# kujason/monopsr

Measured on AMD Instinct MI355X. Metric: instance-crops/sec (fwd+Chamfer), higher is better.
Workload: dtype f32; 1 GPU; BASELINE cfg3: batch=256/GPU synthetic 48x48 crops -> ResNet-101 trunk(block3, os4) + squash/map-decoder/xyz + heads fwd, + 1024-pt nn_distance Chamfer fwd/bwd; batch_per_gpu=256, global_batch=256, points=1024, streams_per_gpu=1

## Files before the change

### include/monopsr_hip.h

```cpp
#ifndef MONOPSR_HIP_H
#define MONOPSR_HIP_H

#include <stddef.h>
#include <stdint.h>

#ifdef __cplusplus
extern "C" {
#endif

typedef void *mpsr_stream_t;
typedef void *mpsr_event_t;

enum {
    MPSR_OK = 0,
    MPSR_ERR_INVALID_ARG = 1,
    MPSR_ERR_HIP = 2,
    MPSR_ERR_WORKSPACE = 3,
    MPSR_ERR_UNSUPPORTED = 4
};

const char *mpsr_last_error(void);
int mpsr_abi_version(void);
uint32_t mpsr_crc32c(uint32_t crc, const void *data, size_t n);


int mpsr_nn_distance_fwd(int b, int n, const float *xyz1, int m, const float *xyz2,
                         float *dist1, int *idx1, float *dist2, int *idx2, mpsr_stream_t stream);

int mpsr_nn_distance_bwd(int b, int n, const float *xyz1, int m, const float *xyz2,
                         const float *grad_dist1, const int *idx1, const float *grad_dist2, const int *idx2,
                         float *grad_xyz1, float *grad_xyz2, mpsr_stream_t stream);


enum { MPSR_EMD_DEVICE = 0, MPSR_EMD_HOST = 1 };

size_t mpsr_emd_temp_floats(int b, int n, int m, int semantics);
size_t mpsr_approx_match_temp_floats(int b, int n, int m);

int mpsr_approx_match(int b, int n, int m, const float *xyz1, const float *xyz2, float *match, float *temp,
                      size_t temp_floats, mpsr_stream_t stream);

int mpsr_approx_match_ex(int b, int n, int m, const float *xyz1, const float *xyz2, float *match, float *temp,
                         size_t temp_floats, int semantics, mpsr_stream_t stream);

size_t mpsr_emd_loss_temp_floats(int b, int n, int m, int semantics);
int mpsr_emd_loss(int b, int n, int m, const float *xyz1, const float *xyz2, float *cost, float *grad1, float *grad2,
                  float *temp, size_t temp_floats, int semantics, mpsr_stream_t stream);

int mpsr_match_cost(int b, int n, int m, const float *xyz1, const float *xyz2, const float *match, float *out,
                    mpsr_stream_t stream);

int mpsr_match_cost_grad(int b, int n, int m, const float *xyz1, const float *xyz2, const float *match,
                         float *grad1, float *grad2, mpsr_stream_t stream);


int mpsr_crop_and_resize(const float *image, int nimg, int H, int W, int C, const float *boxes,
                         const int *box_ind, int nb, int ch, int cw, float extrapolation_value, float *out,
                         mpsr_stream_t stream);

int mpsr_resize_bilinear(const float *in, int B, int H, int W, int C, int OH, int OW, int align_corners,
                         float *out, mpsr_stream_t stream);

int mpsr_max_pool(const float *in, int B, int H, int W, int C, int k, int s, int pad_same, float *out,
                  mpsr_stream_t stream);


size_t mpsr_conv2d_scratch_floats(int B, int H, int W, int N);
int mpsr_conv2d_plan(int B, int H, int W, int C, int N, int KH, int KW, int dilation, int *kind,
                     double *executed_flops);
int mpsr_conv2d_nhwc_f32(const float *x, int B, int H, int W, int C, const float *w, const float *bias,
                         const float *residual, float *y, int N, int KH, int KW, int dilation, int relu,
                         int split_k, float *ws, size_t ws_floats, mpsr_stream_t stream);

enum { MPSR_CALL_MATH_INHERIT = 0, MPSR_CALL_MATH_FP32 = 1, MPSR_CALL_MATH_BF16X3 = 2 };
enum { MPSR_CALL_WINOGRAD_INHERIT = 0, MPSR_CALL_WINOGRAD_AUTO = 1, MPSR_CALL_WINOGRAD_OFF = 2,
       MPSR_CALL_WINOGRAD_ACCURATE = 3  };
typedef struct mpsr_conv_opts {
    int32_t math;
    int32_t winograd_policy;
} mpsr_conv_opts;
int mpsr_conv2d_nhwc_f32_ex(const float *x, int B, int H, int W, int C, const float *w, const float *bias,
                            const float *residual, float *y, int N, int KH, int KW, int dilation, int relu,
                            int split_k, float *ws, size_t ws_floats, const mpsr_conv_opts *opts, mpsr_stream_t stream);

enum { MPSR_MATH_FP32 = 0, MPSR_MATH_BF16X3 = 1 };
int mpsr_set_conv_math(int mode);
int mpsr_get_conv_math(void);

enum { MPSR_WINOGRAD_AUTO = 0, MPSR_WINOGRAD_OFF = 1, MPSR_WINOGRAD_ACCURATE = 2 };
int mpsr_set_winograd_policy(int policy);
int mpsr_get_winograd_policy(void);

size_t mpsr_conv3x3_upsampled_scratch_floats(int B, int h, int w, int C, int N);
int mpsr_conv3x3_upsampled_f32(const float *x, int B, int h, int w, int C, int OH, int OW, int align_corners,
                               const float *weights, const float *bias, int relu, float *y, int N, float *ws,
                               size_t ws_floats, mpsr_stream_t stream);
int mpsr_conv3x3_upsampled_applies(int B, int h, int w, int C, int OH, int OW, int N, int align_corners);
size_t mpsr_conv3x3_upsampled_bwd_scratch_floats(int B, int h, int w, int C, int N);
int mpsr_conv3x3_upsampled_bwd_f32(const float *x, const float *dy, int B, int h, int w, int C, int OH, int OW,
                                   int align_corners, const float *weights, int N, float *dw, float *dx, float *ws,
                                   size_t ws_floats, mpsr_stream_t stream);

int mpsr_im2col_root(const float *x, int B, int H, int W, float *cols, int kpad, mpsr_stream_t stream);


int mpsr_conv2d_wgrad_f32(const float *x, const float *dy, int B, int H, int W, int C, int N, int KH, int KW,
                          int dilation, float *dw, float *db, mpsr_stream_t stream);
size_t mpsr_conv2d_wgrad_scratch_floats(int B, int H, int W, int C, int N, int KH, int KW, int dilation);
int mpsr_conv2d_wgrad_ws_f32(const float *x, const float *dy, int B, int H, int W, int C, int N, int KH, int KW,
                             int dilation, float *dw, float *db, float *ws, size_t ws_floats, mpsr_stream_t stream);
int mpsr_conv2d_wgrad_plan(int B, int H, int W, int C, int N, int KH, int KW, int dilation, size_t ws_floats, int *kind,
                           int *tiles, int *steps, int *nslices);

int mpsr_conv2d_dgrad_pack(const float *w, int N, int KH, int KW, int C, float *wd, mpsr_stream_t stream);

typedef struct mpsr_pack_job {
    const float *w;
    float *wd;
    int32_t N, Nd, T, C;
    int64_t chunk0;
} mpsr_pack_job;
size_t mpsr_dgrad_pack_table_bytes(const mpsr_pack_job *jobs, int n_jobs);
int mpsr_dgrad_pack_table_build(const mpsr_pack_job *jobs, int n_jobs, void *table_host, long long *n_chunks);
int mpsr_conv2d_dgrad_pack_batch(const void *table_dev, long long n_chunks, mpsr_stream_t stream);

int mpsr_act_bias_grad(const float *dy, const float *y, float *dx, float *db, long long M, int N,
                       mpsr_stream_t stream);

int mpsr_bias_grad(const float *dy, long long M, int N, float *db, mpsr_stream_t stream);

int mpsr_relu_grad(const float *dy, const float *y, float *dx, long long total, mpsr_stream_t stream);

int mpsr_conv2d_relu_masked_f32(const float *x, int B, int H, int W, int C, const float *w, const float *mask, float *y,
                                int N, int KH, int KW, int dilation, float *ws, size_t ws_floats, mpsr_stream_t stream);
long long mpsr_relu_bitmask_words(long long M, int N);
int mpsr_relu_bitmask(const float *y, long long M, int N, unsigned *bits, mpsr_stream_t stream);
int mpsr_conv1x1_masked_applies(long long M, int K, int N);
int mpsr_conv1x1_relu_bitmask_f32(const float *x, long long M, int K, const float *w, const float *bias,
                                  const float *residual, int relu, float *y, unsigned *bits, int N, mpsr_stream_t stream);
int mpsr_conv1x1_masked_f32(const float *x, long long M, int K, const float *w, const float *bias,
                            const float *residual, const unsigned *mask, float *y, int N, mpsr_stream_t stream);

int mpsr_max_pool_grad(const float *x, const float *dy, int B, int H, int W, int C, int k, int s, int pad_same,
                       float *dx, mpsr_stream_t stream);

int mpsr_resize_bilinear_grad(const float *dy, int B, int H, int W, int C, int OH, int OW, int align_corners,
                              float *dx, mpsr_stream_t stream);

int mpsr_adam_step(float *param, const float *grad, float *m, float *v, long long n, float lr, float beta1,
                   float beta2, float eps, int step, float grad_scale, mpsr_stream_t stream);
int mpsr_adam_step_lr_dev(float *param, const float *grad, float *m, float *v, long long n, const float *lr_t_dev,
                          float beta1, float beta2, float eps, float grad_scale, mpsr_stream_t stream);

int mpsr_crop_and_resize_grad(const float *grad_out, int nimg, int H, int W, int C, const float *boxes,
                              const int *box_ind, int nb, int ch, int cw, float *grad_image, mpsr_stream_t stream);

int mpsr_batch_norm_stats(const float *z, long long M, int C, double *sum, double *sumsq_shifted,
                          mpsr_stream_t stream);
int mpsr_batch_norm_finalize(const double *sum, const double *sumsq_shifted, const float *z_row0, long long M, int C,
                             float eps, float decay, float *moving_mean, float *moving_variance, float *mean,
                             float *inv_std, mpsr_stream_t stream);
int mpsr_batch_norm_grad_finalize(const double *sum_g, const double *sum_gz, double count, int C, float *dbeta,
                                  float *mean_g, float *mean_gz, mpsr_stream_t stream);
int mpsr_batch_norm_apply(const float *z, long long M, int C, const float *mean, const float *inv_std,
                          const float *beta, int relu, float *y, mpsr_stream_t stream);
int mpsr_batch_norm_grad_sums(const float *dy, const float *y, const float *z, long long M, int C, const float *mean,
                              const float *inv_std, double *sum_g, double *sum_gz, mpsr_stream_t stream);
int mpsr_batch_norm_grad(const float *dy, const float *y, const float *z, long long M, int C, const float *mean,
                         const float *inv_std, const float *mean_g, const float *mean_gz, float *dz,
                         mpsr_stream_t stream);

int mpsr_batch_norm_grad_sums_z(const float *dy, const float *z, long long M, int C, const float *mean,
                                const float *inv_std, const float *beta, double *sum_g, double *sum_gz,
                                mpsr_stream_t stream);
int mpsr_batch_norm_grad_z(const float *dy, const float *z, long long M, int C, const float *mean, const float *inv_std,
                           const float *beta, const float *mean_g, const float *mean_gz, float *dz, mpsr_stream_t stream);

int mpsr_clip_by_norm_segments(float *grads, const int *chunk_seg, const long long *chunk_begin,
                               const int *chunk_len, int n_chunks, float *sumsq, size_t sumsq_floats, int n_segments,
                               float clip_norm, mpsr_stream_t stream);

int mpsr_clip_adam_ema_step(float *param, const float *grad, float *m, float *v, float *shadow, const int *chunk_seg,
                            const long long *chunk_begin, const int *chunk_len, int n_chunks, float *sumsq,
                            size_t sumsq_floats, int n_segments, float clip_norm, float lr, float beta1, float beta2,
                            float eps, int step, float ema_decay, mpsr_stream_t stream);


int mpsr_xyz_map_local_to_global(const float *xyz_local, const float *view_angs, const float *centroids,
                                 float *xyz_global, int b, int p, mpsr_stream_t stream);

int mpsr_xyz_map_local_to_global_grad(const float *grad_global, const float *view_angs, float *grad_local,
                                      float *grad_centroids, int b, int p, mpsr_stream_t stream);

int mpsr_proj_err_norm(const float *xyz_global, const float *boxes_2d, const float *cam_p, const float *valid_mask,
                       float *proj_err_maps, float *proj_err_norm, int b, int h, int w, mpsr_stream_t stream);

int mpsr_proj_err_norm_grad(const float *grad_proj_err_norm, const float *xyz_global, const float *boxes_2d,
                            const float *cam_p, const float *valid_mask, float *grad_xyz_global, int b, int h, int w,
                            mpsr_stream_t stream);

int mpsr_proj_err_norm_cams(const float *xyz_global, const float *boxes_2d, const float *cam_p, int n_cams,
                            const int *cam_index, const float *valid_mask, float *proj_err_maps, float *proj_err_norm,
                            int b, int h, int w, mpsr_stream_t stream);
int mpsr_proj_err_norm_grad_cams(const float *grad_proj_err_norm, const float *xyz_global, const float *boxes_2d,
                                 const float *cam_p, int n_cams, const int *cam_index, const float *valid_mask,
                                 float *grad_xyz_global, int b, int h, int w, mpsr_stream_t stream);

int mpsr_depth_map_local_to_global(const float *depth_local, int depth_stride, const float *cen_z,
                                   const float *boxes_2d, const float *view_angs, const float *cam_p,
                                   float *depth_global, int b, int h, int w, int rotate_view, mpsr_stream_t stream);

int mpsr_depth_map_local_to_global_grad(const float *grad_global, const float *boxes_2d, const float *view_angs,
                                        const float *cam_p, float *grad_cen_z, int b, int h, int w, int rotate_view,
                                        mpsr_stream_t stream);

int mpsr_depth_map_local_to_global_cams(const float *depth_local, int depth_stride, const float *cen_z,
                                        const float *boxes_2d, const float *view_angs, const float *cam_p, int n_cams,
                                        const int *cam_index, float *depth_global, int b, int h, int w,
                                        int rotate_view, mpsr_stream_t stream);
int mpsr_depth_map_local_to_global_grad_cams(const float *grad_global, const float *boxes_2d, const float *view_angs,
                                             const float *cam_p, int n_cams, const int *cam_index, float *grad_cen_z,
                                             int b, int h, int w, int rotate_view, mpsr_stream_t stream);

int mpsr_huber_loss_sums(const float *pred, const float *target, const float *weights, int b, int p, int c,
                         float delta, float *sums, float *counts, mpsr_stream_t stream);

int mpsr_huber_loss_grad(const float *pred, const float *target, const float *weights, const float *scale, int b,
                         int p, int c, float delta, float *grad, mpsr_stream_t stream);

int mpsr_huber_loss_grad_scales(const float *pred, const float *target, const float *weights, const float *scale,
                                int b, int p, int c, float delta, float *grad, mpsr_stream_t stream);

int mpsr_format_boxes(const float *lwh, const float *view_angs, const float *alpha_bins, const float *alpha_regs,
                      const float *centroids, const float *boxes_2d, const float *scores, const int *class_idx,
                      const float *cam_p, int b, int num_alpha_bins, int img_h, int img_w, int centroid_middle,
                      int post_process_cen_x, float max_depth, float *box_3d, float *box_2d, mpsr_stream_t stream);


typedef struct mpsr_layer {
    int32_t cin, cout, kh, kw, dilation, relu;
    int64_t w_off;
    int64_t b_off;
} mpsr_layer;

typedef struct mpsr_net_opts {
    float *filter_cache;
    size_t filter_cache_floats;
    int32_t filter_cache_valid;
    mpsr_event_t ready_event;
    int32_t *filter_cache_tags;
    int32_t math;
    int32_t winograd_policy;
} mpsr_net_opts;

size_t mpsr_filter_cache_floats(const mpsr_layer *layers, int n_layers);

#define MPSR_TRUNK_LAYERS 94

size_t mpsr_trunk_workspace_bytes(int B, int H, int W);

int mpsr_trunk_fwd(const float *img, int B, int H, int W, const float *blob, const mpsr_layer *layers,
                   int n_layers, float *out, void *workspace, size_t workspace_bytes, mpsr_stream_t stream);
int mpsr_trunk_fwd_ex(const float *img, int B, int H, int W, const float *blob, const mpsr_layer *layers,
                      int n_layers, float *out, void *workspace, size_t workspace_bytes, const mpsr_net_opts *opts,
                      mpsr_stream_t stream);

#define MPSR_DECODER_LAYERS 7

size_t mpsr_decoder_workspace_bytes(int B, int fh, int fw, int mh, int mw);

int mpsr_squash_decoder_fwd(const float *crop_feat, const float *full_feat, int B, int fh, int fw, int mh, int mw,
                            const float *blob, const mpsr_layer *layers, int n_layers, float *feat_box3d,
                            float *feat_map, float *xyz_map, void *workspace, size_t workspace_bytes,
                            mpsr_stream_t stream);
int mpsr_squash_decoder_plan(int B, int fh, int fw, int mh, int mw, const mpsr_layer *layers, int n_layers, int *kinds,
                             double *executed_flops);
int mpsr_squash_decoder_fwd_ex(const float *crop_feat, const float *full_feat, int B, int fh, int fw, int mh, int mw,
                               const float *blob, const mpsr_layer *layers, int n_layers, float *feat_box3d,
                               float *feat_map, float *xyz_map, void *workspace, size_t workspace_bytes,
                               const mpsr_net_opts *opts, mpsr_stream_t stream);

#define MPSR_HEAD_LAYERS 7

typedef struct mpsr_head_consts {
    float image_h, image_w;
    float max_depth;
    float cen_y_norm;
    float cen_y_class_offset;
    int32_t num_classes;
    int32_t num_alpha_bins;
} mpsr_head_consts;

size_t mpsr_heads_workspace_bytes(int B, int feat_elems);

typedef struct mpsr_head_outputs {
    float *lwh, *lwh_offs, *alpha_bins, *alpha_regs, *prop_cen_z, *cen_y, *cen_y_offs, *cen_z, *cen_z_offs,
        *cen_x, *centroids;
} mpsr_head_outputs;

int mpsr_heads_fwd(const float *feat_box3d, int B, int feat_elems, const float *boxes_2d, const float *cam_p,
                   const float *view_angs, const int *class_idx, const float *mean_lwh, const float *cen_z_offset,
                   const mpsr_head_consts *consts, const float *blob, const mpsr_layer *layers, int n_layers,
                   const mpsr_head_outputs *outs, void *workspace, size_t workspace_bytes, mpsr_stream_t stream);
int mpsr_heads_fwd_cams(const float *feat_box3d, int B, int feat_elems, const float *boxes_2d, const float *cam_p,
                        int n_cams, const int *cam_index, const float *view_angs, const int *class_idx,
                        const float *mean_lwh, const float *cen_z_offset, const mpsr_head_consts *consts,
                        const float *blob, const mpsr_layer *layers, int n_layers, const mpsr_head_outputs *outs,
                        void *workspace, size_t workspace_bytes, mpsr_stream_t stream);


#define MPSR_KITTI_FIELDS 14
#define MPSR_KITTI_X1 0
#define MPSR_KITTI_Y1 1
#define MPSR_KITTI_X2 2
#define MPSR_KITTI_Y2 3
#define MPSR_KITTI_ALPHA 4
#define MPSR_KITTI_H 5
#define MPSR_KITTI_W 6
#define MPSR_KITTI_L 7
#define MPSR_KITTI_TX 8
#define MPSR_KITTI_TY 9
#define MPSR_KITTI_TZ 10
#define MPSR_KITTI_RY 11
#define MPSR_KITTI_SCORE 12
#define MPSR_KITTI_TRUNCATION 12
#define MPSR_KITTI_OCCLUSION 13
enum { MPSR_KITTI_CAR = 0, MPSR_KITTI_PEDESTRIAN = 1, MPSR_KITTI_CYCLIST = 2, MPSR_KITTI_VAN = 3,
       MPSR_KITTI_PERSON_SITTING = 4, MPSR_KITTI_DONTCARE = 5, MPSR_KITTI_OTHER = 6 };
#define MPSR_KITTI_CONFIGS 27
#define MPSR_KITTI_POINTS 41
#define MPSR_KITTI_MAX_FRAME_DETECTIONS 8192

typedef struct mpsr_kitti_batch {
    const double *det;
    const int *det_cls;
    const double *gt;
    const int *gt_cls;
    const int *det_off;
    const int *gt_off;
    const long long *pair_off;
    const int *det_off_host;
    const int *gt_off_host;
    const long long *pair_off_host;
    int n_det, n_gt, n_frames;
} mpsr_kitti_batch;

int mpsr_kitti_overlaps(const mpsr_kitti_batch *batch, double *overlaps, mpsr_stream_t stream);

int mpsr_kitti_match(const mpsr_kitti_batch *batch, const double *overlaps, const double *min_overlap,
                     double *tp_scores, int *n_care, mpsr_stream_t stream);

size_t mpsr_kitti_stats_workspace_bytes(int n_frames, int n_configs);

int mpsr_kitti_stats(const mpsr_kitti_batch *batch, const double *overlaps, const double *min_overlap,
                     const double *thresholds, const int *n_thresholds, int compute_aos, int *counts,
                     double *similarity, void *workspace, size_t workspace_bytes, mpsr_stream_t stream);


size_t mpsr_lidar_project_workspace_bytes(int n_frames, int h, int w);

int mpsr_lidar_project_depths(const float *points, const long long *frame_offsets, const long long *frame_offsets_host,
                              int n_frames, const double *velo_to_cam0, const double *p2, int h, int w,
                              double max_depth, float *out, void *workspace, size_t workspace_bytes,
                              mpsr_stream_t stream);

#define MPSR_DEPTH_MAX_KERNEL 15
enum { MPSR_DEPTH_BLUR_BILATERAL = 0, MPSR_DEPTH_BLUR_GAUSSIAN = 1 };
enum { MPSR_DEPTH_KERNEL_FAR = 0, MPSR_DEPTH_KERNEL_MED = 1, MPSR_DEPTH_KERNEL_NEAR = 2 };

typedef struct mpsr_depth_fill_opts {
    float max_depth;
    int extrapolate;
    int blur_type;
    int kernel_h[3];
    int kernel_w[3];
    unsigned char kernels[3][MPSR_DEPTH_MAX_KERNEL * MPSR_DEPTH_MAX_KERNEL];
} mpsr_depth_fill_opts;

size_t mpsr_depth_fill_workspace_bytes(int n_frames, int h, int w);

int mpsr_depth_fill_multiscale(const float *depths, int n_frames, int h, int w, const mpsr_depth_fill_opts *opts,
                               float *out, float *stages, void *workspace, size_t workspace_bytes,
                               mpsr_stream_t stream);


#define MPSR_INSTANCE_MAX_BOXES 255
#define MPSR_INSTANCE_BOX_STRIDE 20
enum { MPSR_CENTROID_BOTTOM = 0, MPSR_CENTROID_MIDDLE = 1 };

int mpsr_instance_images(const float *depth, int n_frames, int h, int w, const double *p2, const double *boxes,
                         const long long *box_offsets, const long long *box_offsets_host, unsigned char *out,
                         mpsr_stream_t stream);

int mpsr_instance_xyz_crops(const float *depth, const unsigned char *inst, const float *p2, int n_frames, int h, int w,
                            const int *frame_index, const int *instance_id, const float *boxes_2d,
                            const float *boxes_3d, const float *view_angs, const int *frame_index_host,
                            const int *instance_id_host, const float *boxes_2d_host, int n_boxes, int roi_h,
                            int roi_w, int centroid_type, int rotate_view, float *xyz_local, float *xyz_global,
                            float *valid, mpsr_stream_t stream);


enum { MPSR_JITTER_NONE = 0, MPSR_JITTER_OVERSAMPLE = 1, MPSR_JITTER_ALL = 2 };

int mpsr_sample_slots(const int *slot_frame, const int *slot_s, int n, const int *num_objs,
                      const long long *label_offset, const int *split_index, const int *frame_local,
                      const int *image_hw, const double *p00_p02, const double *label_boxes, int n_frames,
                      unsigned long long seed, int epoch, int jitter_mode, long long *label_row, int *oversample_index,
                      int *jitter_flag, double *boxes_xyxy, int *slot_hw, double *slot_p, int *slot_split_index,
                      int *slot_frame_local, mpsr_stream_t stream);

int mpsr_jitter_boxes_2d(const double *boxes_xyxy, const int *jitter_flag, const int *image_hw, const double *p00_p02,
                         const int *frame_index, const int *slot, int n, unsigned long long seed, int epoch,
                         double iou_threshold_min, int max_trials, int write_unjittered, double *out_xyxy,
                         float *out_boxes_2d, float *out_boxes_2d_norm, float *out_view_angs, int *out_trials,
                         mpsr_stream_t stream);

enum { MPSR_CROP_BAD_FRAME = 1, MPSR_CROP_BAD_ID = 2, MPSR_CROP_BAD_NOT_FINITE = 4, MPSR_CROP_BAD_BOX = 8 };
int mpsr_instance_xyz_crops_status(const float *depth, const unsigned char *inst, const float *p2, int n_frames, int h,
                                   int w, const int *frame_index, const int *instance_id, const float *boxes_2d,
                                   const float *boxes_3d, const float *view_angs, int n_boxes, int roi_h, int roi_w,
                                   int centroid_type, int rotate_view, float *xyz_local, float *xyz_global,
                                   float *valid, int *status, mpsr_stream_t stream);

enum { MPSR_IMAGE_NOISE_REFERENCE = 1, MPSR_IMAGE_NOISE_COMPOSED = 2 };
int mpsr_image_noise(const unsigned char *frames, int n_frames, int h, int w, const int *gather,
                     const int *frame_index, int nb, unsigned long long seed, int epoch, int mode, float *out,
                     int *stages, double *params, mpsr_stream_t stream);


enum { MPSR_MERGE_SCORE_DISTANCE = 0, MPSR_MERGE_SCORE_MAX = 1, MPSR_MERGE_SCORE_MIN = 2 };

int mpsr_merge_detections(const float *label_boxes, const float *label_z, const long long *label_off,
                          long long n_labels, const float *det_boxes, const double *det_scores,
                          const long long *det_off, long long n_dets, int n_frames, double min_iou, int score_type,
                          float *out_boxes, double *out_scores, int *out_match, mpsr_stream_t stream);

int mpsr_kitti_detection_rows(const float *box_3d, const float *box_2d, const int *frame, const double *p2,
                              const int *image_wh, int n, int n_frames, double score_threshold, int project,
                              double *rows, int *cls, int *keep, mpsr_stream_t stream);

enum { MPSR_NAN_RULE_ENTRY = 0, MPSR_NAN_RULE_FRAME = 1 };
#define MPSR_METRIC_STATS_MAX_COLS 32
int mpsr_metric_stats(const float *values, const int *frame, int n_rows, int n_cols, const int *column_metric,
                      int n_metrics, int n_frames, int nan_rule, int *frame_flags, double *stats,
                      mpsr_stream_t stream);

#define MPSR_TRAIN_LOG_MAX_TERMS 16
#define MPSR_TRAIN_LOG_STAT_COLS 5
typedef struct { const float *p[MPSR_TRAIN_LOG_MAX_TERMS]; } mpsr_train_log_terms;
int mpsr_train_log_append(mpsr_train_log_terms terms, int n_terms, const float *sumsq, int n_segments, float clip_norm,
                          float lr, long long step, float *rows, long long *steps, int n_rows, int n_cols, int row,
                          mpsr_stream_t stream);


size_t mpsr_scene_workspace_bytes(int n_frames, long long total_pixels, int n_boxes, int points_per_box);

int mpsr_scene_project(const float *xyz_global, const float *valid_mask, const int *box_frame,
                       const int *box_frame_host, const int *box_keep, const double *cam_p, const int *frame_hw,
                       const int *frame_hw_host, const long long *pixel_offset, const long long *pixel_offset_host,
                       int n_frames, int n_boxes, int points_per_box, void *workspace, size_t workspace_bytes,
                       mpsr_stream_t stream);

int mpsr_scene_resolve(const int *box_frame, const int *box_frame_host, int n_frames, long long total_pixels,
                       int n_boxes, int points_per_box, const void *workspace, size_t workspace_bytes, float *depth,
                       unsigned char *instance, mpsr_stream_t stream);

int mpsr_scene_compact(const float *xyz_global, const int *box_frame, const float *const *images,
                       const long long *pixel_offset, int n_frames, long long total_pixels, int n_boxes,
                       int points_per_box, int visible_only, void *workspace, size_t workspace_bytes, float *xyz,
                       float *rgb, int *box, int *pixel, long long *frame_offset, int *kept_per_box,
                       int *visible_per_box, mpsr_stream_t stream);

size_t mpsr_scene_score_scratch_bytes(int n_frames);
int mpsr_scene_score(const float *xyz_global, const int *box_frame, const int *box_frame_host, const int *box_gt_id,
                     const float *const *gt_depth, const unsigned char *const *gt_instance,
                     const long long *pixel_offset, int n_frames, long long total_pixels, int n_boxes,
                     int points_per_box, const void *workspace, size_t workspace_bytes, void *scratch,
                     size_t scratch_bytes, int *counts, double *sums, mpsr_stream_t stream);


size_t mpsr_scene_surface_workspace_bytes(int n_frames, long long total_pixels, int n_boxes, int map_h, int map_w);

int mpsr_scene_surface_render(const float *xyz_global, const float *valid_mask, const int *box_frame,
                              const int *box_frame_host, const int *box_keep, const double *cam_p, const int *frame_hw,
                              const int *frame_hw_host, const long long *pixel_offset,
                              const long long *pixel_offset_host, int n_frames, int n_boxes, int map_h, int map_w,
                              float max_edge_dz, int max_span_px, void *workspace, size_t workspace_bytes,
                              mpsr_stream_t stream);

int mpsr_scene_surface_resolve(const int *box_frame, const int *box_frame_host, int n_frames, long long total_pixels,
                               int n_boxes, int map_h, int map_w, const void *workspace, size_t workspace_bytes,
                               float *depth, unsigned char *instance, int *tri, mpsr_stream_t stream);

int mpsr_scene_surface_score(const int *box_frame, const int *box_frame_host, const int *box_gt_id,
                             const float *const *gt_depth, const unsigned char *const *gt_instance,
                             const int *frame_hw, const long long *pixel_offset, int n_frames, long long total_pixels,
                             int n_boxes, int map_h, int map_w, const void *workspace, size_t workspace_bytes,
                             void *scratch, size_t scratch_bytes, int *counts, double *sums, mpsr_stream_t stream);


int mpsr_proj_points(const float *local, const float *x, const float *boxes_2d, const float *cam_p, int n_cams,
                     const int *cam_index, const float *mask, float *uv, unsigned char *valid, double *err, int b,
                     int h, int w, int rotate_view, int cam0_shift, int round_box_2d, int use_pixel_centres,
                     mpsr_stream_t stream);

int mpsr_proj_fit(const float *local, const float *x0, const float *boxes_2d, const float *cam_p, int n_cams,
                  const int *cam_index, const float *mask, int b, int h, int w, int n_fit, int rotate_view,
                  int cam0_shift, int round_box_2d, int use_pixel_centres, double xatol, double fatol, int max_iter,
                  float *x, double *err, double *err0, int *iters, int *evals, int *status, mpsr_stream_t stream);

#ifdef __cplusplus
}
#endif
#endif
```

### monopsr_amd/_lib.py

```python
import ctypes
import os

_HERE = os.path.dirname(os.path.abspath(__file__))
LIB_PATH = os.environ.get("MPSR_LIB_PATH") or os.path.join(_HERE, "libmonopsr_hip.so")
ABI_VERSION = 13

_lib = None


class MpsrError(RuntimeError):
    """A libmonopsr_hip.so call returned a non-zero status."""


class InvalidArgumentError(MpsrError, ValueError):
    """Shape/argument check failed -- the analogue of the tf.errors.InvalidArgumentError the reference's
    OP_REQUIRES checks raise (tf_nndistance.cpp:51-58, tf_approxmatch.cpp:152-165)."""


c_f = ctypes.c_void_p
c_i = ctypes.c_int
c_sz = ctypes.c_size_t


class Layer(ctypes.Structure):
    _fields_ = [("cin", ctypes.c_int32), ("cout", ctypes.c_int32), ("kh", ctypes.c_int32), ("kw", ctypes.c_int32),
                ("dilation", ctypes.c_int32), ("relu", ctypes.c_int32), ("w_off", ctypes.c_int64),
                ("b_off", ctypes.c_int64)]


class HeadConsts(ctypes.Structure):
    _fields_ = [("image_h", ctypes.c_float), ("image_w", ctypes.c_float), ("max_depth", ctypes.c_float),
                ("cen_y_norm", ctypes.c_float), ("cen_y_class_offset", ctypes.c_float),
                ("num_classes", ctypes.c_int32), ("num_alpha_bins", ctypes.c_int32)]


class HeadOutputs(ctypes.Structure):
    _fields_ = [(k, ctypes.c_void_p) for k in
                ("lwh", "lwh_offs", "alpha_bins", "alpha_regs", "prop_cen_z", "cen_y", "cen_y_offs", "cen_z",
                 "cen_z_offs", "cen_x", "centroids")]


class NetOpts(ctypes.Structure):
    _fields_ = [("filter_cache", ctypes.c_void_p), ("filter_cache_floats", ctypes.c_size_t),
                ("filter_cache_valid", ctypes.c_int32), ("ready_event", ctypes.c_void_p),
                ("filter_cache_tags", ctypes.POINTER(ctypes.c_int32)), ("math", ctypes.c_int32),
                ("winograd_policy", ctypes.c_int32)]


class ConvOpts(ctypes.Structure):
    _fields_ = [("math", ctypes.c_int32), ("winograd_policy", ctypes.c_int32)]


class PackJob(ctypes.Structure):
    _fields_ = [("w", ctypes.c_void_p), ("wd", ctypes.c_void_p), ("N", ctypes.c_int32), ("Nd", ctypes.c_int32),
                ("T", ctypes.c_int32), ("C", ctypes.c_int32), ("chunk0", ctypes.c_int64)]


class KittiBatch(ctypes.Structure):
    _fields_ = [(k, ctypes.c_void_p) for k in
                ("det", "det_cls", "gt", "gt_cls", "det_off", "gt_off", "pair_off", "det_off_host", "gt_off_host",
                 "pair_off_host")] + [("n_det", ctypes.c_int32), ("n_gt", ctypes.c_int32), ("n_frames", ctypes.c_int32)]


class DepthFillOpts(ctypes.Structure):
    _fields_ = [("max_depth", ctypes.c_float), ("extrapolate", ctypes.c_int32), ("blur_type", ctypes.c_int32),
                ("kernel_h", ctypes.c_int32 * 3), ("kernel_w", ctypes.c_int32 * 3),
                ("kernels", (ctypes.c_uint8 * (15 * 15)) * 3)]


class TrainLogTerms(ctypes.Structure):
    _fields_ = [("p", ctypes.c_void_p * 16)]


CALL_MATH = {None: 0, "inherit": 0, "fp32": 1, "bf16x3": 2}
CALL_WINOGRAD = {None: 0, "inherit": 0, "auto": 1, "off": 2, "accurate": 3}


SIGNATURES = {
    "mpsr_last_error": (ctypes.c_char_p, []),
    "mpsr_abi_version": (c_i, []),
    "mpsr_set_conv_math": (c_i, [c_i]),
    "mpsr_get_conv_math": (c_i, []),
    "mpsr_set_winograd_policy": (c_i, [c_i]),
    "mpsr_get_winograd_policy": (c_i, []),
    "mpsr_crc32c": (ctypes.c_uint32, [ctypes.c_uint32, ctypes.c_void_p, c_sz]),
    "mpsr_nn_distance_fwd": (c_i, [c_i, c_i, c_f, c_i, c_f, c_f, c_f, c_f, c_f, c_f]),
    "mpsr_nn_distance_bwd": (c_i, [c_i, c_i, c_f, c_i, c_f, c_f, c_f, c_f, c_f, c_f, c_f, c_f]),
    "mpsr_approx_match_temp_floats": (c_sz, [c_i, c_i, c_i]),
    "mpsr_emd_temp_floats": (c_sz, [c_i, c_i, c_i, c_i]),
    "mpsr_emd_loss_temp_floats": (c_sz, [c_i, c_i, c_i, c_i]),
    "mpsr_approx_match": (c_i, [c_i, c_i, c_i, c_f, c_f, c_f, c_f, c_sz, c_f]),
    "mpsr_approx_match_ex": (c_i, [c_i, c_i, c_i, c_f, c_f, c_f, c_f, c_sz, c_i, c_f]),
    "mpsr_emd_loss": (c_i, [c_i, c_i, c_i, c_f, c_f, c_f, c_f, c_f, c_f, c_sz, c_i, c_f]),
    "mpsr_match_cost": (c_i, [c_i, c_i, c_i, c_f, c_f, c_f, c_f, c_f]),
    "mpsr_match_cost_grad": (c_i, [c_i, c_i, c_i, c_f, c_f, c_f, c_f, c_f, c_f]),
    "mpsr_crop_and_resize": (c_i, [c_f, c_i, c_i, c_i, c_i, c_f, c_f, c_i, c_i, c_i, ctypes.c_float, c_f, c_f]),
    "mpsr_resize_bilinear": (c_i, [c_f, c_i, c_i, c_i, c_i, c_i, c_i, c_i, c_f, c_f]),
    "mpsr_max_pool": (c_i, [c_f, c_i, c_i, c_i, c_i, c_i, c_i, c_i, c_f, c_f]),
    "mpsr_conv2d_nhwc_f32": (c_i, [c_f, c_i, c_i, c_i, c_i, c_f, c_f, c_f, c_f, c_i, c_i, c_i, c_i, c_i, c_i, c_f,
                                   c_sz, c_f]),
    "mpsr_conv2d_nhwc_f32_ex": (c_i, [c_f, c_i, c_i, c_i, c_i, c_f, c_f, c_f, c_f, c_i, c_i, c_i, c_i, c_i, c_i, c_f,
                                      c_sz, ctypes.POINTER(ConvOpts), c_f]),
    "mpsr_conv2d_scratch_floats": (c_sz, [c_i, c_i, c_i, c_i]),
    "mpsr_conv2d_plan": (c_i, [c_i] * 8 + [ctypes.POINTER(c_i), ctypes.POINTER(ctypes.c_double)]),
    "mpsr_im2col_root": (c_i, [c_f, c_i, c_i, c_i, c_f, c_i, c_f]),
    "mpsr_conv2d_wgrad_f32": (c_i, [c_f, c_f, c_i, c_i, c_i, c_i, c_i, c_i, c_i, c_i, c_f, c_f, c_f]),
    "mpsr_conv2d_wgrad_scratch_floats": (c_sz, [c_i] * 8),
    "mpsr_conv2d_wgrad_ws_f32": (c_i, [c_f, c_f, c_i, c_i, c_i, c_i, c_i, c_i, c_i, c_i, c_f, c_f, c_f, c_sz, c_f]),
    "mpsr_conv2d_wgrad_plan": (c_i, [c_i] * 8 + [c_sz] + [ctypes.POINTER(c_i)] * 4),
    "mpsr_conv2d_dgrad_pack": (c_i, [c_f, c_i, c_i, c_i, c_i, c_f, c_f]),
    "mpsr_dgrad_pack_table_bytes": (c_sz, [ctypes.POINTER(PackJob), c_i]),
    "mpsr_dgrad_pack_table_build": (c_i, [ctypes.POINTER(PackJob), c_i, ctypes.c_void_p,
                                          ctypes.POINTER(ctypes.c_longlong)]),
    "mpsr_conv2d_dgrad_pack_batch": (c_i, [c_f, ctypes.c_longlong, c_f]),
    "mpsr_act_bias_grad": (c_i, [c_f, c_f, c_f, c_f, ctypes.c_longlong, c_i, c_f]),
    "mpsr_bias_grad": (c_i, [c_f, ctypes.c_longlong, c_i, c_f, c_f]),
    "mpsr_relu_grad": (c_i, [c_f, c_f, c_f, ctypes.c_longlong, c_f]),
    "mpsr_conv2d_relu_masked_f32": (c_i, [c_f, c_i, c_i, c_i, c_i, c_f, c_f, c_f, c_i, c_i, c_i, c_i, c_f, c_sz, c_f]),
    "mpsr_relu_bitmask_words": (ctypes.c_longlong, [ctypes.c_longlong, c_i]),
    "mpsr_relu_bitmask": (c_i, [c_f, ctypes.c_longlong, c_i, c_f, c_f]),
    "mpsr_conv1x1_masked_applies": (c_i, [ctypes.c_longlong, c_i, c_i]),
    "mpsr_conv1x1_masked_f32": (c_i, [c_f, ctypes.c_longlong, c_i, c_f, c_f, c_f, c_f, c_f, c_i, c_f]),
    "mpsr_conv1x1_relu_bitmask_f32": (c_i, [c_f, ctypes.c_longlong, c_i, c_f, c_f, c_f, c_i, c_f, c_f, c_i, c_f]),
    "mpsr_max_pool_grad": (c_i, [c_f, c_f, c_i, c_i, c_i, c_i, c_i, c_i, c_i, c_f, c_f]),
    "mpsr_resize_bilinear_grad": (c_i, [c_f, c_i, c_i, c_i, c_i, c_i, c_i, c_i, c_f, c_f]),
    "mpsr_adam_step": (c_i, [c_f, c_f, c_f, c_f, ctypes.c_longlong, ctypes.c_float, ctypes.c_float, ctypes.c_float,
                             ctypes.c_float, c_i, ctypes.c_float, c_f]),
    "mpsr_adam_step_lr_dev": (c_i, [c_f, c_f, c_f, c_f, ctypes.c_longlong, c_f, ctypes.c_float, ctypes.c_float,
                                    ctypes.c_float, ctypes.c_float, c_f]),
    "mpsr_crop_and_resize_grad": (c_i, [c_f, c_i, c_i, c_i, c_i, c_f, c_f, c_i, c_i, c_i, c_f, c_f]),
    "mpsr_batch_norm_stats": (c_i, [c_f, ctypes.c_longlong, c_i, c_f, c_f, c_f]),
    "mpsr_batch_norm_finalize": (c_i, [c_f, c_f, c_f, ctypes.c_longlong, c_i, ctypes.c_float, ctypes.c_float, c_f, c_f,
                                       c_f, c_f, c_f]),
    "mpsr_batch_norm_grad_finalize": (c_i, [c_f, c_f, ctypes.c_double, c_i, c_f, c_f, c_f, c_f]),
    "mpsr_batch_norm_apply": (c_i, [c_f, ctypes.c_longlong, c_i, c_f, c_f, c_f, c_i, c_f, c_f]),
    "mpsr_batch_norm_grad_sums": (c_i, [c_f, c_f, c_f, ctypes.c_longlong, c_i, c_f, c_f, c_f, c_f, c_f]),
    "mpsr_batch_norm_grad_sums_z": (c_i, [c_f, c_f, ctypes.c_longlong, c_i, c_f, c_f, c_f, c_f, c_f, c_f]),
    "mpsr_batch_norm_grad_z": (c_i, [c_f, c_f, ctypes.c_longlong, c_i, c_f, c_f, c_f, c_f, c_f, c_f, c_f]),
    "mpsr_batch_norm_grad": (c_i, [c_f, c_f, c_f, ctypes.c_longlong, c_i, c_f, c_f, c_f, c_f, c_f, c_f]),
    "mpsr_clip_by_norm_segments": (c_i, [c_f, c_f, c_f, c_f, c_i, c_f, ctypes.c_size_t, c_i, ctypes.c_float, c_f]),
    "mpsr_clip_adam_ema_step": (c_i, [c_f, c_f, c_f, c_f, c_f, c_f, c_f, c_f, c_i, c_f, ctypes.c_size_t, c_i, ctypes.c_float,
                                      ctypes.c_float, ctypes.c_float, ctypes.c_float, ctypes.c_float, c_i, ctypes.c_float,
                                      c_f]),
    "mpsr_xyz_map_local_to_global": (c_i, [c_f, c_f, c_f, c_f, c_i, c_i, c_f]),
    "mpsr_xyz_map_local_to_global_grad": (c_i, [c_f, c_f, c_f, c_f, c_i, c_i, c_f]),
    "mpsr_proj_err_norm": (c_i, [c_f, c_f, c_f, c_f, c_f, c_f, c_i, c_i, c_i, c_f]),
    "mpsr_proj_err_norm_grad": (c_i, [c_f, c_f, c_f, c_f, c_f, c_f, c_i, c_i, c_i, c_f]),
    "mpsr_proj_err_norm_cams": (c_i, [c_f, c_f, c_f, c_i, c_f, c_f, c_f, c_f, c_i, c_i, c_i, c_f]),
    "mpsr_proj_err_norm_grad_cams": (c_i, [c_f, c_f, c_f, c_f, c_i, c_f, c_f, c_f, c_i, c_i, c_i, c_f]),
    "mpsr_depth_map_local_to_global": (c_i, [c_f, c_i, c_f, c_f, c_f, c_f, c_f, c_i, c_i, c_i, c_i, c_f]),
    "mpsr_depth_map_local_to_global_grad": (c_i, [c_f, c_f, c_f, c_f, c_f, c_i, c_i, c_i, c_i, c_f]),
    "mpsr_depth_map_local_to_global_cams": (c_i, [c_f, c_i, c_f, c_f, c_f, c_f, c_i, c_f, c_f, c_i, c_i, c_i, c_i, c_f]),
    "mpsr_depth_map_local_to_global_grad_cams": (c_i, [c_f, c_f, c_f, c_f, c_i, c_f, c_f, c_i, c_i, c_i, c_i, c_f]),
    "mpsr_huber_loss_sums": (c_i, [c_f, c_f, c_f, c_i, c_i, c_i, ctypes.c_float, c_f, c_f, c_f]),
    "mpsr_huber_loss_grad": (c_i, [c_f, c_f, c_f, c_f, c_i, c_i, c_i, ctypes.c_float, c_f, c_f]),
    "mpsr_huber_loss_grad_scales": (c_i, [c_f, c_f, c_f, c_f, c_i, c_i, c_i, ctypes.c_float, c_f, c_f]),
    "mpsr_format_boxes": (c_i, [c_f, c_f, c_f, c_f, c_f, c_f, c_f, c_f, c_f, c_i, c_i, c_i, c_i, c_i, c_i,
                                ctypes.c_float, c_f, c_f, c_f]),
    "mpsr_trunk_workspace_bytes": (c_sz, [c_i, c_i, c_i]),
    "mpsr_trunk_fwd": (c_i, [c_f, c_i, c_i, c_i, c_f, ctypes.POINTER(Layer), c_i, c_f, c_f, c_sz, c_f]),
    "mpsr_conv3x3_upsampled_scratch_floats": (c_sz, [c_i, c_i, c_i, c_i, c_i]),
    "mpsr_conv3x3_upsampled_f32": (c_i, [c_f, c_i, c_i, c_i, c_i, c_i, c_i, c_i, c_f, c_f, c_i, c_f, c_i, c_f, c_sz, c_f]),
    "mpsr_conv3x3_upsampled_applies": (c_i, [c_i, c_i, c_i, c_i, c_i, c_i, c_i, c_i]),
    "mpsr_conv3x3_upsampled_bwd_scratch_floats": (c_sz, [c_i, c_i, c_i, c_i, c_i]),
    "mpsr_conv3x3_upsampled_bwd_f32": (c_i, [c_f, c_f, c_i, c_i, c_i, c_i, c_i, c_i, c_i, c_f, c_i, c_f, c_f, c_f, c_sz,
                                            c_f]),
    "mpsr_filter_cache_floats": (c_sz, [ctypes.POINTER(Layer), c_i]),
    "mpsr_trunk_fwd_ex": (c_i, [c_f, c_i, c_i, c_i, c_f, ctypes.POINTER(Layer), c_i, c_f, c_f, c_sz,
                                ctypes.POINTER(NetOpts), c_f]),
    "mpsr_squash_decoder_fwd_ex": (c_i, [c_f, c_f, c_i, c_i, c_i, c_i, c_i, c_f, ctypes.POINTER(Layer), c_i, c_f, c_f,
                                         c_f, c_f, c_sz, ctypes.POINTER(NetOpts), c_f]),
    "mpsr_decoder_workspace_bytes": (c_sz, [c_i, c_i, c_i, c_i, c_i]),
    "mpsr_squash_decoder_plan": (c_i, [c_i, c_i, c_i, c_i, c_i, ctypes.POINTER(Layer), c_i, ctypes.POINTER(c_i),
                                       ctypes.POINTER(ctypes.c_double)]),
    "mpsr_squash_decoder_fwd": (c_i, [c_f, c_f, c_i, c_i, c_i, c_i, c_i, c_f, ctypes.POINTER(Layer), c_i, c_f, c_f,
                                      c_f, c_f, c_sz, c_f]),
    "mpsr_heads_workspace_bytes": (c_sz, [c_i, c_i]),
    "mpsr_heads_fwd": (c_i, [c_f, c_i, c_i, c_f, c_f, c_f, c_f, c_f, c_f, ctypes.POINTER(HeadConsts), c_f,
                             ctypes.POINTER(Layer), c_i, ctypes.POINTER(HeadOutputs), c_f, c_sz, c_f]),
    "mpsr_heads_fwd_cams": (c_i, [c_f, c_i, c_i, c_f, c_f, c_i, c_f, c_f, c_f, c_f, c_f, ctypes.POINTER(HeadConsts), c_f,
                                  ctypes.POINTER(Layer), c_i, ctypes.POINTER(HeadOutputs), c_f, c_sz, c_f]),
    "mpsr_kitti_overlaps": (c_i, [ctypes.POINTER(KittiBatch), c_f, c_f]),
    "mpsr_kitti_match": (c_i, [ctypes.POINTER(KittiBatch), c_f, ctypes.POINTER(ctypes.c_double), c_f, c_f, c_f]),
    "mpsr_kitti_stats_workspace_bytes": (c_sz, [c_i, c_i]),
    "mpsr_kitti_stats": (c_i, [ctypes.POINTER(KittiBatch), c_f, ctypes.POINTER(ctypes.c_double), c_f,
                               ctypes.POINTER(c_i), c_i, c_f, c_f, c_f, c_sz, c_f]),
    "mpsr_lidar_project_workspace_bytes": (c_sz, [c_i, c_i, c_i]),
    "mpsr_lidar_project_depths": (c_i, [c_f, c_f, ctypes.c_void_p, c_i, c_f, c_f, c_i, c_i, ctypes.c_double, c_f, c_f,
                                        c_sz, c_f]),
    "mpsr_depth_fill_workspace_bytes": (c_sz, [c_i, c_i, c_i]),
    "mpsr_depth_fill_multiscale": (c_i, [c_f, c_i, c_i, c_i, ctypes.POINTER(DepthFillOpts), c_f, c_f, c_f, c_sz, c_f]),
    "mpsr_instance_images": (c_i, [c_f, c_i, c_i, c_i, c_f, c_f, c_f, ctypes.c_void_p, c_f, c_f]),
    "mpsr_instance_xyz_crops": (c_i, [c_f, c_f, c_f, c_i, c_i, c_i, c_f, c_f, c_f, c_f, c_f, ctypes.c_void_p,
                                      ctypes.c_void_p, ctypes.c_void_p, c_i, c_i, c_i, c_i, c_i, c_f, c_f, c_f, c_f]),
    "mpsr_sample_slots": (c_i, [c_f, c_f, c_i, c_f, c_f, c_f, c_f, c_f, c_f, c_f, c_i, ctypes.c_uint64, c_i, c_i, c_f,
                                c_f, c_f, c_f, c_f, c_f, c_f, c_f, c_f]),
    "mpsr_jitter_boxes_2d": (c_i, [c_f, c_f, c_f, c_f, c_f, c_f, c_i, ctypes.c_uint64, c_i, ctypes.c_double, c_i, c_i,
                                   c_f, c_f, c_f, c_f, c_f, c_f]),
    "mpsr_image_noise": (c_i, [c_f, c_i, c_i, c_i, c_f, c_f, c_i, ctypes.c_uint64, c_i, c_i, c_f, c_f, c_f, c_f]),
    "mpsr_instance_xyz_crops_status": (c_i, [c_f, c_f, c_f, c_i, c_i, c_i, c_f, c_f, c_f, c_f, c_f, c_i, c_i, c_i, c_i,
                                             c_i, c_f, c_f, c_f, c_f, c_f]),
    "mpsr_merge_detections": (c_i, [c_f, c_f, c_f, ctypes.c_longlong, c_f, c_f, c_f, ctypes.c_longlong, c_i,
                                    ctypes.c_double, c_i, c_f, c_f, c_f, c_f]),
    "mpsr_kitti_detection_rows": (c_i, [c_f, c_f, c_f, c_f, c_f, c_i, c_i, ctypes.c_double, c_i, c_f, c_f, c_f, c_f]),
    "mpsr_metric_stats": (c_i, [c_f, c_f, c_i, c_i, ctypes.POINTER(c_i), c_i, c_i, c_i, c_f, c_f, c_f]),
    "mpsr_train_log_append": (c_i, [TrainLogTerms, c_i, c_f, c_i, ctypes.c_float, ctypes.c_float, ctypes.c_longlong, c_f,
                                    c_f, c_i, c_i, c_i, c_f]),
    "mpsr_scene_workspace_bytes": (c_sz, [c_i, ctypes.c_longlong, c_i, c_i]),
    "mpsr_scene_project": (c_i, [c_f, c_f, c_f, ctypes.c_void_p, c_f, c_f, c_f, ctypes.c_void_p, c_f, ctypes.c_void_p,
                                 c_i, c_i, c_i, c_f, c_sz, c_f]),
    "mpsr_scene_resolve": (c_i, [c_f, ctypes.c_void_p, c_i, ctypes.c_longlong, c_i, c_i, c_f, c_sz, c_f, c_f, c_f]),
    "mpsr_scene_compact": (c_i, [c_f, c_f, c_f, c_f, c_i, ctypes.c_longlong, c_i, c_i, c_i, c_f, c_sz, c_f, c_f, c_f,
                                 c_f, c_f, c_f, c_f, c_f]),
    "mpsr_scene_score_scratch_bytes": (c_sz, [c_i]),
    "mpsr_scene_score": (c_i, [c_f, c_f, ctypes.c_void_p, c_f, c_f, c_f, c_f, c_i, ctypes.c_longlong, c_i, c_i, c_f,
                               c_sz, c_f, c_sz, c_f, c_f, c_f]),
    "mpsr_scene_surface_workspace_bytes": (c_sz, [c_i, ctypes.c_longlong, c_i, c_i, c_i]),
    "mpsr_scene_surface_render": (c_i, [c_f, c_f, c_f, ctypes.c_void_p, c_f, c_f, c_f, ctypes.c_void_p, c_f,
                                        ctypes.c_void_p, c_i, c_i, c_i, c_i, ctypes.c_float, c_i, c_f, c_sz, c_f]),
    "mpsr_scene_surface_resolve": (c_i, [c_f, ctypes.c_void_p, c_i, ctypes.c_longlong, c_i, c_i, c_i, c_f, c_sz, c_f,
                                         c_f, c_f, c_f]),
    "mpsr_scene_surface_score": (c_i, [c_f, ctypes.c_void_p, c_f, c_f, c_f, c_f, c_f, c_i, ctypes.c_longlong, c_i, c_i,
                                       c_i, c_f, c_sz, c_f, c_sz, c_f, c_f, c_f]),
    "mpsr_proj_points": (c_i, [c_f, c_f, c_f, c_f, c_i, c_f, c_f, c_f, c_f, c_f, c_i, c_i, c_i, c_i, c_i, c_i, c_i,
                               c_f]),
    "mpsr_proj_fit": (c_i, [c_f, c_f, c_f, c_f, c_i, c_f, c_f, c_i, c_i, c_i, c_i, c_i, c_i, c_i, c_i, ctypes.c_double,
                            ctypes.c_double, c_i, c_f, c_f, c_f, c_f, c_f, c_f, c_f]),
}


def lib():
    global _lib
    if _lib is None:
        import torch
        if not os.path.exists(LIB_PATH):
            raise MpsrError(
                "libmonopsr_hip.so is not built (%s). Build it with `python -c 'import __graft_entry__ as g; "
                "g.build()'` or `make -C monopsr_amd/csrc`. There is no CPU fallback." % LIB_PATH)
        handle = ctypes.CDLL(LIB_PATH)
        missing = [name for name in SIGNATURES if not hasattr(handle, name)]
        if missing and not os.environ.get("MPSR_PARTIAL_LIB"):
            raise MpsrError("libmonopsr_hip.so lacks declared symbols %s; rebuild (make -C monopsr_amd/csrc)"
                            % missing)
        for name, (res, args) in SIGNATURES.items():
            if name in missing:
                continue
            fn = getattr(handle, name)
            fn.restype = res
            fn.argtypes = args
        got = handle.mpsr_abi_version()
        if got != ABI_VERSION:
            raise MpsrError("libmonopsr_hip.so ABI %d != expected %d; rebuild" % (got, ABI_VERSION))
        _lib = handle
    return _lib


MATH_MODES = {"fp32": 0, "bf16x3": 1}


def get_conv_math():
    return {v: k for k, v in MATH_MODES.items()}[lib().mpsr_get_conv_math()]


def set_conv_math(mode):
    names = {v: k for k, v in MATH_MODES.items()}
    prev = names[lib().mpsr_get_conv_math()]
    if mode not in MATH_MODES:
        raise InvalidArgumentError("unknown conv math mode %r (choose from %s)" % (mode, sorted(MATH_MODES)))
    check(lib().mpsr_set_conv_math(MATH_MODES[mode]))
    return prev


WINOGRAD_POLICIES = {"auto": 0, "off": 1, "accurate": 2}


def set_winograd_policy(policy):
    names = {v: k for k, v in WINOGRAD_POLICIES.items()}
    prev = names[lib().mpsr_get_winograd_policy()]
    if policy not in WINOGRAD_POLICIES:
        raise InvalidArgumentError("unknown Winograd policy %r (choose from %s)" % (policy, sorted(WINOGRAD_POLICIES)))
    check(lib().mpsr_set_winograd_policy(WINOGRAD_POLICIES[policy]))
    return prev


def check(status):
    if status == 0:
        return
    msg = lib().mpsr_last_error().decode("utf-8", "replace")
    if status == 1:
        raise InvalidArgumentError(msg)
    raise MpsrError("status %d: %s" % (status, msg))


def ptr(t):
    if t is None:
        return None
    if not t.is_cuda:
        raise MpsrError("expected a tensor on the GPU; monopsr_amd has no CPU path")
    if not t.is_contiguous():
        raise MpsrError("expected a contiguous tensor")
    return t.data_ptr()


def stream(device_index=None):
    import torch
    raw = getattr(torch._C, "_cuda_getCurrentRawStream", None)
    if raw is None:
        return torch.cuda.current_stream(device_index).cuda_stream
    return raw(torch._C._cuda_getDevice() if device_index is None else device_index)
```

### monopsr_amd/csrc/conv_mfma.hip

```cpp
#include <atomic>
#include <mutex>
#include <type_traits>

#include "common.h"

namespace {

using f32x16 = __attribute__((ext_vector_type(16))) float;
using f32x4 = __attribute__((ext_vector_type(4))) float;
using bf16x4 = __attribute__((ext_vector_type(4))) __bf16;
using bf16x8 = __attribute__((ext_vector_type(8))) __bf16;

constexpr int MATH_FP32 = 0, MATH_BF16X3 = 1;

constexpr int BK = 32;
constexpr int LDS_STRIDE = BK + 4;
constexpr int MAX_CLS = 9;

using mpsr::FastDiv;
using mpsr::fdiv;
using mpsr::make_fastdiv;

struct PixelClass {
    int y0, h, x0, w;
    int ky0, ky1, kx0, kx1;
    int tiles;
    int rows;
    FastDiv fd_ppi, fd_w;
};

struct ConvParams {
    const float *x;
    const float *w;
    const float *bias;
    const float *residual;
    float *y;
    float *ws;
    int M, H, W, C, N, KH, KW, dil, relu;
    int ksteps_total, ksteps_per_split, cblocks;
    int mtiles_xcd, ntiles, splits;
    FastDiv fd_ntiles, fd_mtiles;
    unsigned xbytes, wbytes;
    size_t ws_floats;
    int ncls;
    PixelClass cls[MAX_CLS];
};


template <bool PLAIN>
__device__ __forceinline__ int decode_row(const ConvParams &p, const PixelClass &pc, int row, int &yy, int &xx)
{
    if constexpr (PLAIN) {
        yy = xx = 0;
        return row < pc.rows ? row : -1;
    }
    if (row >= pc.rows) {
        yy = -(1 << 20);
        xx = 0;
        return -1;
    }
    const int img = fdiv(row, pc.fd_ppi), pp = row - img * (pc.h * pc.w);
    const int py = fdiv(pp, pc.fd_w);
    yy = pc.y0 + py;
    xx = pc.x0 + (pp - py * pc.w);
    return (img * p.H + yy) * p.W + xx;
}

template <bool PLAIN, int AV, int BV>
__device__ __forceinline__ void tile_rows(const ConvParams &p, const PixelClass &pc, int r0, int n0, int lrow,
                                          unsigned col, unsigned apast, int (&ay)[AV], int (&ax)[AV],
                                          unsigned (&abase)[AV], unsigned (&bbase)[BV])
{
#pragma unroll
    for (int j = 0; j < AV; ++j) {
        const int pix = decode_row<PLAIN>(p, pc, r0 + lrow + 32 * j, ay[j], ax[j]);
        abase[j] = pix < 0 ? apast : (unsigned)pix * (unsigned)p.C * 4u + col;
    }
    const int Ktot = p.KH * p.KW * p.C;
#pragma unroll
    for (int j = 0; j < BV; ++j) {
        const int n = n0 + lrow + 32 * j;
        bbase[j] = n < p.N ? (unsigned)n * (unsigned)Ktot * 4u + col : p.wbytes;
    }
}

struct KCursor {
    int cb, kx, ky;
    __device__ __forceinline__ void seek(const PixelClass &pc, int ks)
    {
        const int ntx = pc.kx1 - pc.kx0 + 1;
        const int ntaps = (pc.ky1 - pc.ky0 + 1) * ntx;
        cb = ks / ntaps;
        const int tap = ks - cb * ntaps;
        const int ty = tap / ntx;
        ky = pc.ky0 + ty;
        kx = pc.kx0 + (tap - ty * ntx);
    }
    __device__ __forceinline__ void advance(const PixelClass &pc)
    {
        if (++kx > pc.kx1) {
            kx = pc.kx0;
            if (++ky > pc.ky1) {
                ky = pc.ky0;
                ++cb;
            }
        }
    }
};

template <int AV, int BV>
__device__ __forceinline__ void load_tile_checked(const ConvParams &p, __amdgpu_buffer_rsrc_t rx,
                                                  __amdgpu_buffer_rsrc_t rw, const KCursor &st, int lcol, bool live,
                                                  const int (&ay)[AV], const int (&ax)[AV],
                                                  const unsigned (&abase)[AV], const unsigned (&bbase)[BV],
                                                  float4 (&ra)[AV], float4 (&rb)[BV])
{
    const int dy = (st.ky - (p.KH >> 1)) * p.dil, dx = (st.kx - (p.KW >> 1)) * p.dil;
    const int c = st.cb * BK + lcol;
    const bool cok = (c < p.C) & live;
    const int aoff = ((dy * p.W + dx) * p.C + c) * 4;
#pragma unroll
    for (int j = 0; j < AV; ++j) {
        const int yy = ay[j] + dy, xx = ax[j] + dx;
        const bool ok = cok & (yy >= 0) & (yy < p.H) & (xx >= 0) & (xx < p.W);
        const unsigned off = ok ? abase[j] + (unsigned)aoff : p.xbytes;
        ra[j] = __builtin_bit_cast(float4, __builtin_amdgcn_raw_buffer_load_b128(rx, off, 0, 0));
    }
    const unsigned boff = (unsigned)(((st.ky * p.KW + st.kx) * p.C + c) * 4);
#pragma unroll
    for (int j = 0; j < BV; ++j) {
        const unsigned off = cok ? bbase[j] + boff : p.wbytes;
        rb[j] = __builtin_bit_cast(float4, __builtin_amdgcn_raw_buffer_load_b128(rw, off, 0, 0));
    }
}

template <int MATH, int AV, int BV>
__device__ __forceinline__ void fill_lds(float *As, float *Bs, int lrow, int lcol, const float4 (&ra)[AV],
                                         const float4 (&rb)[BV])
{
    auto put = [&](float *row, const float4 &v4) {
        if constexpr (MATH == MATH_BF16X3) {
            const f32x4 v = {v4.x, v4.y, v4.z, v4.w};
            const bf16x4 hi = __builtin_convertvector(v, bf16x4);
            const bf16x4 lo = __builtin_convertvector(v - __builtin_convertvector(hi, f32x4), bf16x4);
            __bf16 *r = reinterpret_cast<__bf16 *>(row);
            *reinterpret_cast<bf16x4 *>(r + lcol) = hi;
            *reinterpret_cast<bf16x4 *>(r + BK + lcol) = lo;
        } else {
            *reinterpret_cast<float4 *>(row + lcol) = v4;
        }
    };
#pragma unroll
    for (int j = 0; j < AV; ++j) put(&As[(lrow + 32 * j) * LDS_STRIDE], ra[j]);
#pragma unroll
    for (int j = 0; j < BV; ++j) put(&Bs[(lrow + 32 * j) * LDS_STRIDE], rb[j]);
}

__device__ __forceinline__ int lds_fragment(int lane) { return (lane & 31) * LDS_STRIDE + (lane >> 5) * 4; }

template <int TM, int TN, int MATH>
__device__ __forceinline__ void mma_tile(f32x16 (&acc)[TM][TN], const float *Aw, const float *Bw)
{
    if constexpr (MATH == MATH_BF16X3) {
        const __bf16 *Ah = reinterpret_cast<const __bf16 *>(Aw), *Bh = reinterpret_cast<const __bf16 *>(Bw);
#pragma unroll
        for (int sl = 0; sl < BK / 16; ++sl) {
            bf16x8 ah[TM], al[TM], bh[TN], bl[TN];
#pragma unroll
            for (int i = 0; i < TM; ++i) {
                ah[i] = *reinterpret_cast<const bf16x8 *>(Ah + i * 32 * LDS_STRIDE * 2 + sl * 16);
                al[i] = *reinterpret_cast<const bf16x8 *>(Ah + i * 32 * LDS_STRIDE * 2 + BK + sl * 16);
            }
#pragma unroll
            for (int j = 0; j < TN; ++j) {
                bh[j] = *reinterpret_cast<const bf16x8 *>(Bh + j * 32 * LDS_STRIDE * 2 + sl * 16);
                bl[j] = *reinterpret_cast<const bf16x8 *>(Bh + j * 32 * LDS_STRIDE * 2 + BK + sl * 16);
            }
#pragma unroll
            for (int i = 0; i < TM; ++i)
#pragma unroll
                for (int j = 0; j < TN; ++j) {
                    acc[i][j] = __builtin_amdgcn_mfma_f32_32x32x16_bf16(al[i], bh[j], acc[i][j], 0, 0, 0);
                    acc[i][j] = __builtin_amdgcn_mfma_f32_32x32x16_bf16(ah[i], bl[j], acc[i][j], 0, 0, 0);
                    acc[i][j] = __builtin_amdgcn_mfma_f32_32x32x16_bf16(ah[i], bh[j], acc[i][j], 0, 0, 0);
                }
        }
    } else {
#pragma unroll
        for (int kb = 0; kb < BK / 8; ++kb) {
            float4 a[TM], b[TN];
#pragma unroll
            for (int i = 0; i < TM; ++i) a[i] = *reinterpret_cast<const float4 *>(Aw + i * 32 * LDS_STRIDE + kb * 8);
#pragma unroll
            for (int j = 0; j < TN; ++j) b[j] = *reinterpret_cast<const float4 *>(Bw + j * 32 * LDS_STRIDE + kb * 8);
#pragma unroll
            for (int i = 0; i < TM; ++i)
#pragma unroll
                for (int j = 0; j < TN; ++j) {
                    acc[i][j] = __builtin_amdgcn_mfma_f32_32x32x2f32(a[i].x, b[j].x, acc[i][j], 0, 0, 0);
                    acc[i][j] = __builtin_amdgcn_mfma_f32_32x32x2f32(a[i].y, b[j].y, acc[i][j], 0, 0, 0);
                    acc[i][j] = __builtin_amdgcn_mfma_f32_32x32x2f32(a[i].z, b[j].z, acc[i][j], 0, 0, 0);
                    acc[i][j] = __builtin_amdgcn_mfma_f32_32x32x2f32(a[i].w, b[j].w, acc[i][j], 0, 0, 0);
                }
        }
    }
}

template <int TM, int TN>
__device__ __forceinline__ void clear_acc(f32x16 (&acc)[TM][TN])
{
#pragma unroll
    for (int i = 0; i < TM; ++i)
#pragma unroll
        for (int j = 0; j < TN; ++j)
#pragma unroll
            for (int e = 0; e < 16; ++e) acc[i][j][e] = 0.f;
}

template <int TM, int TN>
__device__ __forceinline__ void settle_acc(f32x16 (&acc)[TM][TN])
{
#pragma unroll
    for (int i = 0; i < TM; ++i)
#pragma unroll
        for (int j = 0; j < TN; ++j) asm volatile("s_nop 15\n\ts_nop 7" : "+a"(acc[i][j]));
}

template <int TM, int TN, bool PLAIN, class TileFn>
__device__ __forceinline__ void store_output(const ConvParams &p, const PixelClass &pc, float *lds, int r0, int n0,
                                             int wm, int wn, int wave, int lane, bool fused, float *dst, TileFn tile)
{
    const int col = lane & 31, rsub = (lane >> 5) * 4;
    int dy_, dx_;
    if ((p.N & 3) == 0) {
        __syncthreads();
        float *ep = lds + wave * (32 * LDS_STRIDE);
        const int erow = lane >> 3, ecol = (lane & 7) * 4;
#pragma unroll
        for (int i = 0; i < TM; ++i) {
            int pix[4];
#pragma unroll
            for (int it = 0; it < 4; ++it)
                pix[it] = decode_row<PLAIN>(p, pc, r0 + (wm * TM + i) * 32 + erow + 8 * it, dy_, dx_);
#pragma unroll
            for (int j = 0; j < TN; ++j) {
                const int n = n0 + (wn * TN + j) * 32 + ecol;
                float4 bias = make_float4(0.f, 0.f, 0.f, 0.f);
                if (fused && p.bias && n < p.N) bias = *reinterpret_cast<const float4 *>(p.bias + n);
                const f32x16 tv = tile(i, j);
#pragma unroll
                for (int e = 0; e < 16; ++e) ep[((e & 3) + 8 * (e >> 2) + rsub) * LDS_STRIDE + col] = tv[e];
                __builtin_amdgcn_wave_barrier();
#pragma unroll
                for (int it = 0; it < 4; ++it) {
                    float4 v = *reinterpret_cast<const float4 *>(&ep[(erow + 8 * it) * LDS_STRIDE + ecol]);
                    if (pix[it] >= 0 && n < p.N) {
                        const size_t o = (size_t)pix[it] * p.N + n;
                        if (fused) {
                            v.x += bias.x; v.y += bias.y; v.z += bias.z; v.w += bias.w;
                            if (p.residual) {
                                const float4 rr = *reinterpret_cast<const float4 *>(p.residual + o);
                                v.x += rr.x; v.y += rr.y; v.z += rr.z; v.w += rr.w;
                            }
                            if (p.relu) {
                                v.x = fmaxf(v.x, 0.f); v.y = fmaxf(v.y, 0.f); v.z = fmaxf(v.z, 0.f); v.w = fmaxf(v.w, 0.f);
                            }
                        }
                        *reinterpret_cast<float4 *>(dst + o) = v;
                    }
                }
                __builtin_amdgcn_wave_barrier();
            }
        }
        return;
    }
#pragma unroll
    for (int i = 0; i < TM; ++i) {
#pragma unroll
        for (int j = 0; j < TN; ++j) {
            const int n = n0 + (wn * TN + j) * 32 + col;
            const f32x16 tv = tile(i, j);
            if (n >= p.N) continue;
#pragma unroll
            for (int e = 0; e < 16; ++e) {
                const int pix = decode_row<PLAIN>(p, pc, r0 + (wm * TM + i) * 32 + rsub + (e & 3) + 8 * (e >> 2), dy_, dx_);
                if (pix < 0) continue;
                const size_t o = (size_t)pix * p.N + n;
                float v = tv[e];
                if (fused) {
                    if (p.bias) v += p.bias[n];
                    if (p.residual) v += p.residual[o];
                    if (p.relu) v = fmaxf(v, 0.f);
                }
                dst[o] = v;
            }
        }
    }
}

template <int BM, int BN, int WM, int WN, int MATH = MATH_FP32, int DEPTH = 1, int KIND = 0>
__global__ __launch_bounds__(256) void conv_igemm_kernel(const ConvParams p)
{
    constexpr bool PLAIN = KIND == 1, CLS = KIND == 2;
    static_assert(WM * WN == 4, "4 waves per workgroup");
    constexpr int TM = BM / WM / 32, TN = BN / WN / 32;
    constexpr int AV = BM / 32, BV = BN / 32;
    __shared__ __attribute__((aligned(16))) float lds[(BM + BN) * LDS_STRIDE];
    float *As = lds, *Bs = lds + BM * LDS_STRIDE;

    const int xcd = blockIdx.x & 7, l = blockIdx.x >> 3;
    const int lq = fdiv(l, p.fd_ntiles);
    const int ni = l - lq * p.ntiles;
    const int si = fdiv(lq, p.fd_mtiles);
    int lm = lq - si * p.mtiles_xcd;
    const int n0 = ni * BN;
    int ci = -1;
    if constexpr (PLAIN) {
        if (xcd + 8 * lm < p.cls[0].tiles) ci = 0;
    } else {
        for (int c = 0; c < p.ncls; ++c) {
            const int cnt = p.cls[c].tiles > xcd ? (p.cls[c].tiles - xcd + 7) >> 3 : 0;
            if (lm < cnt) {
                ci = c;
                break;
            }
            lm -= cnt;
        }
    }
    if (ci < 0) return;
    const PixelClass pc = p.cls[ci];
    const int r0 = (xcd + 8 * lm) * BM;
    const int ksteps_cls = (pc.ky1 - pc.ky0 + 1) * (pc.kx1 - pc.kx0 + 1) * p.cblocks;
    const int ks_per = p.splits > 1 ? (ksteps_cls + p.splits - 1) / p.splits : ksteps_cls;
    const int ks_begin = si * ks_per;
    const int ks_end = min(ksteps_cls, ks_begin + ks_per);

    const int tid = threadIdx.x, lane = tid & 63, wave = tid >> 6;
    const int wm = wave / WN, wn = wave % WN;
    const int lrow = tid >> 3, lcol = (tid & 7) * 4;

    const __amdgpu_buffer_rsrc_t rx =
        __builtin_amdgcn_make_buffer_rsrc(const_cast<float *>(p.x), 0, (int)p.xbytes, 0x00020000);
    const __amdgpu_buffer_rsrc_t rw =
        __builtin_amdgcn_make_buffer_rsrc(const_cast<float *>(p.w), 0, (int)p.wbytes, 0x00020000);

    int ay[AV], ax[AV];
    unsigned abase[AV], bbase[BV];
    tile_rows<PLAIN>(p, pc, r0, n0, lrow, PLAIN || CLS ? (unsigned)lcol * 4u : 0u,
                     PLAIN ? p.xbytes : CLS ? p.xbytes + (unsigned)(p.dil * (p.W + 1) * p.C * 4) : 0u, ay, ax, abase,
                     bbase);

    KCursor st;
    if (PLAIN || ks_begin == 0) {
        st.cb = ks_begin;
        st.ky = pc.ky0;
        st.kx = pc.kx0;
    } else {
        st.seek(pc, ks_begin);
    }
    float4 ra[DEPTH][AV], rb[DEPTH][BV];
    auto load_tile = [&](auto set_c, bool live) {
        constexpr int set = decltype(set_c)::value;
        if constexpr (PLAIN) {
            const int soff = st.cb * (BK * 4);
            const __amdgpu_buffer_rsrc_t rxl =
                __builtin_amdgcn_make_buffer_rsrc(const_cast<float *>(p.x), 0, live ? (int)p.xbytes : 0, 0x00020000);
            const __amdgpu_buffer_rsrc_t rwl =
                __builtin_amdgcn_make_buffer_rsrc(const_cast<float *>(p.w), 0, live ? (int)p.wbytes : 0, 0x00020000);
#pragma unroll
            for (int j = 0; j < AV; ++j)
                ra[set][j] = __builtin_bit_cast(float4, __builtin_amdgcn_raw_buffer_load_b128(rxl, abase[j], soff, 0));
#pragma unroll
            for (int j = 0; j < BV; ++j)
                rb[set][j] = __builtin_bit_cast(float4, __builtin_amdgcn_raw_buffer_load_b128(rwl, bbase[j], soff, 0));
            ++st.cb;
        } else if constexpr (CLS) {
            const int dy = (st.ky - (p.KH >> 1)) * p.dil, dx = (st.kx - (p.KW >> 1)) * p.dil;
            const int bias = p.dil * (p.W + 1) * p.C * 4;
            const int soffa = ((dy * p.W + dx) * p.C + st.cb * BK) * 4 + bias;
            const int soffb = ((st.ky * p.KW + st.kx) * p.C + st.cb * BK) * 4;
            const __amdgpu_buffer_rsrc_t rxl = __builtin_amdgcn_make_buffer_rsrc(
                const_cast<char *>(reinterpret_cast<const char *>(p.x)) - bias, 0, live ? (int)p.xbytes + bias : 0,
                0x00020000);
            const __amdgpu_buffer_rsrc_t rwl =
                __builtin_amdgcn_make_buffer_rsrc(const_cast<float *>(p.w), 0, live ? (int)p.wbytes : 0, 0x00020000);
#pragma unroll
            for (int j = 0; j < AV; ++j)
                ra[set][j] = __builtin_bit_cast(float4, __builtin_amdgcn_raw_buffer_load_b128(rxl, abase[j], soffa, 0));
#pragma unroll
            for (int j = 0; j < BV; ++j)
                rb[set][j] = __builtin_bit_cast(float4, __builtin_amdgcn_raw_buffer_load_b128(rwl, bbase[j], soffb, 0));
            st.advance(pc);
        } else {
            load_tile_checked(p, rx, rw, st, lcol, live, ay, ax, abase, bbase, ra[set], rb[set]);
            st.advance(pc);
        }
    };
    using Set0 = std::integral_constant<int, 0>;
    using Set1 = std::integral_constant<int, DEPTH - 1>;
    auto store_tile = [&](auto set_c) {
        constexpr int set = decltype(set_c)::value;
        fill_lds<MATH>(As, Bs, lrow, lcol, ra[set], rb[set]);
    };

    f32x16 acc[TM][TN];
    clear_acc(acc);
    const float *Aw = As + (wm * TM * 32) * LDS_STRIDE + lds_fragment(lane);
    const float *Bw = Bs + (wn * TN * 32) * LDS_STRIDE + lds_fragment(lane);
    auto compute_tile = [&]() { mma_tile<TM, TN, MATH>(acc, Aw, Bw); };

    if (ks_begin < ks_end) {
        load_tile(Set0{}, true);
        store_tile(Set0{});
        __syncthreads();
        if constexpr (DEPTH == 1) {
            for (int ks = ks_begin; ks < ks_end - 1; ++ks) {
                load_tile(Set0{}, true);
                compute_tile();
                __syncthreads();
                store_tile(Set0{});
                __syncthreads();
            }
            compute_tile();
        } else {
            const int n = ks_end - ks_begin;
            load_tile(Set0{}, n > 1);
            int k = 0;
            for (; k + 2 < n; k += 2) {
                load_tile(Set1{}, true);
                compute_tile();
                __syncthreads();
                store_tile(Set0{});
                __syncthreads();
                load_tile(Set0{}, k + 3 < n);
                compute_tile();
                __syncthreads();
                store_tile(Set1{});
                __syncthreads();
            }
            compute_tile();
            if (n - k == 2) {
                __syncthreads();
                store_tile(Set0{});
                __syncthreads();
                compute_tile();
            }
        }
    }
    settle_acc(acc);

    const bool fused = p.splits == 1;
    store_output<TM, TN, PLAIN>(p, pc, lds, r0, n0, wm, wn, wave, lane, fused,
                                fused ? p.y : p.ws + (size_t)si * p.M * p.N,
                                [&](int i, int j) -> f32x16 { return acc[i][j]; });
}

__global__ __launch_bounds__(256) void splitk_reduce_kernel(const float *__restrict__ ws, int splits, long long MN,
                                                            int N, const float *__restrict__ bias,
                                                            const float *__restrict__ residual, int relu,
                                                            float *__restrict__ y)
{
    for (long long i = (long long)blockIdx.x * blockDim.x + threadIdx.x; i < MN;
         i += (long long)gridDim.x * blockDim.x) {
        float v = 0.f;
        for (int s = 0; s < splits; ++s) v += ws[(size_t)s * MN + i];
        if (bias) v += bias[i % N];
        if (residual) v += residual[i];
        if (relu) v = fmaxf(v, 0.f);
        y[i] = v;
    }
}

struct SkParams {
    int G;
    unsigned U;
    unsigned q, r;
    float *slabs;
    int *counters;
    unsigned ubase[MAX_CLS + 1];
    unsigned tbase[MAX_CLS + 1];
    int ks[MAX_CLS];
};

__device__ __forceinline__ unsigned sk_bound(const SkParams &s, unsigned v) { return v * s.q + min(v, s.r); }

__device__ __forceinline__ unsigned sk_owner(const SkParams &s, unsigned u)
{
    const unsigned thr = s.r * (s.q + 1);
    return u < thr ? u / (s.q + 1) : s.r + (u - thr) / s.q;
}

template <int BM, int BN, int WM, int WN, int MATH = MATH_FP32>
__global__ __launch_bounds__(256) void conv_sk_kernel(const ConvParams p, const SkParams sk)
{
    static_assert(WM * WN == 4, "4 waves per workgroup");
    constexpr int TM = BM / WM / 32, TN = BN / WN / 32;
    constexpr int AV = BM / 32, BV = BN / 32;
    __shared__ __attribute__((aligned(16))) float lds[(BM + BN) * LDS_STRIDE + 4];
    float *As = lds, *Bs = lds + BM * LDS_STRIDE;
    int *flag = reinterpret_cast<int *>(lds + (BM + BN) * LDS_STRIDE);

    const unsigned v = (blockIdx.x & 7) * ((unsigned)sk.G >> 3) + (blockIdx.x >> 3);
    const unsigned ustart = sk_bound(sk, v), uend = sk_bound(sk, v + 1);
    unsigned u = ustart;

    const __amdgpu_buffer_rsrc_t rx =
        __builtin_amdgcn_make_buffer_rsrc(const_cast<float *>(p.x), 0, (int)p.xbytes, 0x00020000);
    const __amdgpu_buffer_rsrc_t rw =
        __builtin_amdgcn_make_buffer_rsrc(const_cast<float *>(p.w), 0, (int)p.wbytes, 0x00020000);

    while (u < uend) {
        int tid = threadIdx.x;
        asm volatile("" : "+v"(tid));
        const int lane = tid & 63, wave = tid >> 6;
        const int wm = wave / WN, wn = wave % WN;
        const int lrow = tid >> 3, lcol = (tid & 7) * 4;
        int ci = 0;
        while (u >= sk.ubase[ci + 1]) ++ci;
        const PixelClass pc = p.cls[ci];
        const int ksc = sk.ks[ci];
        const unsigned local = u - sk.ubase[ci];
        const unsigned tic = local / (unsigned)ksc;
        const int ks_begin = (int)(local - tic * (unsigned)ksc);
        const int ks_end = min(ksc, ks_begin + (int)(uend - u));
        const int mt = (int)(tic / (unsigned)p.ntiles), ni = (int)(tic - (unsigned)mt * (unsigned)p.ntiles);
        const int r0 = mt * BM, n0 = ni * BN;

        int ay[AV], ax[AV];
        unsigned abase[AV], bbase[BV];
        tile_rows<false>(p, pc, r0, n0, lrow, 0u, 0u, ay, ax, abase, bbase);
        KCursor st;
        st.seek(pc, ks_begin);
        float4 ra[AV], rb[BV];
        auto load_tile = [&]() {
            load_tile_checked(p, rx, rw, st, lcol, true, ay, ax, abase, bbase, ra, rb);
            st.advance(pc);
        };
        auto store_tile = [&]() { fill_lds<MATH>(As, Bs, lrow, lcol, ra, rb); };
        f32x16 acc[TM][TN];
        clear_acc(acc);
        auto compute_tile = [&]() {
            mma_tile<TM, TN, MATH>(acc, As + (wm * TM * 32) * LDS_STRIDE + lds_fragment(lane),
                                   Bs + (wn * TN * 32) * LDS_STRIDE + lds_fragment(lane));
        };

        load_tile();
        store_tile();
        __syncthreads();
        for (int ks = ks_begin; ks < ks_end - 1; ++ks) {
            load_tile();
            compute_tile();
            __syncthreads();
            store_tile();
            __syncthreads();
        }
        compute_tile();
        settle_acc(acc);

        const unsigned seg_first = u;
        u += (unsigned)(ks_end - ks_begin);
        bool finish = true;
        int pieces = 1;
        unsigned t0 = 0, vfirst = 0;
        if (ks_begin != 0 || ks_end != ksc) {
            t0 = sk.ubase[ci] + tic * (unsigned)ksc;
            vfirst = sk_owner(sk, t0);
            pieces = (int)(sk_owner(sk, t0 + (unsigned)ksc - 1) - vfirst) + 1;
            int *cnt = sk.counters + (sk.tbase[ci] + tic);
            float *slab = sk.slabs + (size_t)(2 * v + (seg_first == ustart ? 0 : 1)) * (BM * BN);
#pragma unroll
            for (int i = 0; i < TM; ++i)
#pragma unroll
                for (int j = 0; j < TN; ++j)
#pragma unroll
                    for (int e4 = 0; e4 < 4; ++e4) {
                        const float4 val = make_float4(acc[i][j][4 * e4], acc[i][j][4 * e4 + 1], acc[i][j][4 * e4 + 2],
                                                       acc[i][j][4 * e4 + 3]);
                        *reinterpret_cast<float4 *>(slab + ((((wave * TM + i) * TN + j) * 4 + e4) * 64 + lane) * 4) = val;
                    }
            asm volatile("s_waitcnt vmcnt(0)" ::: "memory");
            __syncthreads();
            if (tid == 0) {
                __builtin_amdgcn_fence(__ATOMIC_RELEASE, "agent");
                asm volatile("s_waitcnt vmcnt(0)" ::: "memory");
                *flag = __hip_atomic_fetch_add(cnt, 1, __ATOMIC_RELAXED, __HIP_MEMORY_SCOPE_AGENT);
            }
            __syncthreads();
            finish = *flag == pieces - 1;
            if (finish) {
                if (tid == 0) {
                    __builtin_amdgcn_fence(__ATOMIC_ACQUIRE, "agent");
                    __hip_atomic_store(cnt, 0, __ATOMIC_RELAXED, __HIP_MEMORY_SCOPE_AGENT);
                }
                __syncthreads();
            }
        }
        auto tile_values = [&](int i, int j) -> f32x16 {
            if (pieces == 1) return acc[i][j];
            f32x16 t;
            for (int qq = 0; qq < pieces; ++qq) {
                const unsigned vq = vfirst + (unsigned)qq;
                const float *src = sk.slabs + (size_t)(2 * vq + (sk_bound(sk, vq) < t0 ? 1 : 0)) * (BM * BN) +
                                   (((wave * TM + i) * TN + j) * 4 * 64 + lane) * 4;
#pragma unroll
                for (int e4 = 0; e4 < 4; ++e4) {
                    const float4 val = *reinterpret_cast<const float4 *>(src + e4 * 256);
                    if (qq == 0) {
                        t[4 * e4] = val.x; t[4 * e4 + 1] = val.y; t[4 * e4 + 2] = val.z; t[4 * e4 + 3] = val.w;
                    } else {
                        t[4 * e4] += val.x; t[4 * e4 + 1] += val.y; t[4 * e4 + 2] += val.z; t[4 * e4 + 3] += val.w;
                    }
                }
            }
            return t;
        };
        if (finish) store_output<TM, TN, false>(p, pc, lds, r0, n0, wm, wn, wave, lane, true, p.y, tile_values);
        __syncthreads();
    }
}

void build_classes(ConvParams &p, int B, int BM, bool use_classes)
{
    struct Span {
        int o, len, k0, k1;
    };
    Span ys[3], xs[3];
    int ny = 0, nx = 0;
    const int d = p.dil, hk = p.KH >> 1, wk = p.KW >> 1;
    if (use_classes && p.KH == 3 && p.H >= 2 * d) {
        if (p.H - 2 * d > 0) ys[ny++] = {d, p.H - 2 * d, 0, 2};
        ys[ny++] = {0, d, hk, 2};
        ys[ny++] = {p.H - d, d, 0, hk};
    } else {
        ys[ny++] = {0, p.H, 0, p.KH - 1};
    }
    if (use_classes && p.KW == 3 && p.W >= 2 * d) {
        if (p.W - 2 * d > 0) xs[nx++] = {d, p.W - 2 * d, 0, 2};
        xs[nx++] = {0, d, wk, 2};
        xs[nx++] = {p.W - d, d, 0, wk};
    } else {
        xs[nx++] = {0, p.W, 0, p.KW - 1};
    }
    p.ncls = 0;
    for (int a = 0; a < ny; ++a)
        for (int b = 0; b < nx; ++b) {
            PixelClass &c = p.cls[p.ncls++];
            c.y0 = ys[a].o; c.h = ys[a].len; c.ky0 = ys[a].k0; c.ky1 = ys[a].k1;
            c.x0 = xs[b].o; c.w = xs[b].len; c.kx0 = xs[b].k0; c.kx1 = xs[b].k1;
            c.rows = B * c.h * c.w;
            c.fd_ppi = make_fastdiv(c.h * c.w);
            c.fd_w = make_fastdiv(c.w);
            c.tiles = mpsr::ceil_div(c.rows, BM);
        }
    auto taps = [](const PixelClass &c) { return (c.ky1 - c.ky0 + 1) * (c.kx1 - c.kx0 + 1); };
    for (int i = 0; i < p.ncls; ++i)
        for (int j = i + 1; j < p.ncls; ++j)
            if (taps(p.cls[j]) > taps(p.cls[i])) {
                const PixelClass tmp = p.cls[i];
                p.cls[i] = p.cls[j];
                p.cls[j] = tmp;
            }
    p.mtiles_xcd = 0;
    for (int i = 0; i < p.ncls; ++i) p.mtiles_xcd += mpsr::ceil_div(p.cls[i].tiles, 8);
}

inline void plan_tiles(ConvParams &p, int B, int BM, int BN, bool use_classes)
{
    build_classes(p, B, BM, use_classes);
    p.ntiles = mpsr::ceil_div(p.N, BN);
}

template <int BM_, int BN_, int WM_, int WN_>
struct TileShape {
    static constexpr int BM = BM_, BN = BN_, WM = WM_, WN = WN_;
};

template <class F>
int with_tile(int sel, F &&f)
{
    switch (sel) {
        case 0: return f(TileShape<128, 128, 2, 2>{});
        case 1: return f(TileShape<128, 64, 2, 2>{});
        case 2: return f(TileShape<64, 128, 2, 2>{});
        case 3: return f(TileShape<64, 64, 2, 2>{});
        case 5: return f(TileShape<96, 128, 1, 4>{});
        default: return f(TileShape<128, 32, 4, 1>{});
    }
}

std::atomic<int> g_plain_override{-1};

template <int BM, int BN, int WM, int WN, int MATH = MATH_FP32, int DEPTH = 1>
int launch(ConvParams &p, int B, bool use_classes, hipStream_t s)
{
    plan_tiles(p, B, BM, BN, use_classes);
    p.fd_ntiles = make_fastdiv(p.ntiles);
    p.fd_mtiles = make_fastdiv(p.mtiles_xcd);
    const long long blocks = 8LL * p.mtiles_xcd * p.ntiles * p.splits;
    if (blocks > 0x7fffffffLL) return mpsr::fail(MPSR_ERR_UNSUPPORTED, "conv2d: grid too large");
    const bool plain = p.KH == 1 && p.KW == 1 && p.C % BK == 0 && p.ncls == 1 && g_plain_override.load() != 0;
    const bool cls = use_classes && p.KH == 3 && p.KW == 3 && p.C % BK == 0 &&
                     p.H >= 2 * p.dil && p.W >= 2 * p.dil && g_plain_override.load() != 0 &&
                     (long long)p.xbytes + (long long)p.dil * (p.W + 1) * p.C * 4 < 0x7ffffff0LL;
    {
        if (plain) {
            hipLaunchKernelGGL((conv_igemm_kernel<BM, BN, WM, WN, MATH, DEPTH, 1>), dim3((unsigned)blocks), dim3(256),
                               0, s, p);
            MPSR_CHECK_LAUNCH("conv_igemm_kernel");
            return MPSR_OK;
        }
        if (cls) {
            hipLaunchKernelGGL((conv_igemm_kernel<BM, BN, WM, WN, MATH, DEPTH, 2>), dim3((unsigned)blocks), dim3(256),
                               0, s, p);
            MPSR_CHECK_LAUNCH("conv_igemm_kernel");
            return MPSR_OK;
        }
    }
    hipLaunchKernelGGL((conv_igemm_kernel<BM, BN, WM, WN, MATH, DEPTH>), dim3((unsigned)blocks), dim3(256), 0, s, p);
    MPSR_CHECK_LAUNCH("conv_igemm_kernel");
    return MPSR_OK;
}

struct SkSlots {
    std::once_flag once[16];
    int slots[16] = {0};
};

template <int BM, int BN, int WM, int WN, int MATH>
int sk_slots(int &out)
{
    static SkSlots cache;
    int dev = 0;
    MPSR_CHECK_HIP(hipGetDevice(&dev));
    if (dev < 0 || dev >= 16) dev = 0;
    hipError_t err = hipSuccess;
    std::call_once(cache.once[dev], [&]() {
        int per_cu = 0, cus = 0;
        err = hipOccupancyMaxActiveBlocksPerMultiprocessor(
            &per_cu, reinterpret_cast<const void *>(conv_sk_kernel<BM, BN, WM, WN, MATH>), 256, 0);
        if (err == hipSuccess) err = hipDeviceGetAttribute(&cus, hipDeviceAttributeMultiprocessorCount, dev);
        if (err == hipSuccess && per_cu > 0 && cus > 0) cache.slots[dev] = per_cu * cus;
    });
    if (err != hipSuccess) return mpsr::fail(MPSR_ERR_HIP, "stream-K occupancy query: %s", hipGetErrorString(err));
    out = cache.slots[dev] > 0 ? cache.slots[dev] : 256 * 4;
    return MPSR_OK;
}

std::atomic<int> g_tile_override{-1};
std::atomic<int> g_class_override{-1};
std::atomic<int> g_sched_override{-1};
std::atomic<int> g_sk_per_cu{0};
std::atomic<int> g_wino_policy{0};
std::atomic<int> g_wino_override{-1};
std::atomic<int> g_depth_override{-1};
std::atomic<int> g_math{MATH_FP32};
inline int cur_math() { return mpsr::t_call_math >= 0 ? mpsr::t_call_math : g_math.load(); }
inline int cur_wino_policy() { return mpsr::t_call_wino_policy >= 0 ? mpsr::t_call_wino_policy : g_wino_policy.load(); }
std::atomic<int> g_atrous_wino2{1};
std::atomic<int> g_atrous_wino2_min_pixels{12000};
std::atomic<int> g_wino3_halo{1};

inline size_t sk_scratch_floats(int G, int BM, int BN, long long tiles)
{
    return (size_t)G * 2 * BM * BN + (size_t)tiles;
}

template <int BM, int BN, int WM, int WN, int MATH = MATH_FP32>
int launch_sk(ConvParams &p, int B, bool use_classes, int mode, bool counters_clean, hipStream_t s, bool &done)
{
    done = false;
    plan_tiles(p, B, BM, BN, use_classes);
    p.splits = 1;
    SkParams sk;
    unsigned long long U = 0, T = 0;
    for (int c = 0; c < p.ncls; ++c) {
        const PixelClass &pc = p.cls[c];
        sk.ks[c] = (pc.ky1 - pc.ky0 + 1) * (pc.kx1 - pc.kx0 + 1) * p.cblocks;
        sk.ubase[c] = (unsigned)U;
        sk.tbase[c] = (unsigned)T;
        const unsigned long long tiles = (unsigned long long)pc.tiles * p.ntiles;
        T += tiles;
        U += tiles * sk.ks[c];
    }
    for (int c = p.ncls; c <= MAX_CLS; ++c) {
        sk.ubase[c] = (unsigned)U;
        sk.tbase[c] = (unsigned)T;
        if (c < MAX_CLS) sk.ks[c] = 1;
    }
    if (U == 0 || U > 0x7fffffffULL || T > 0x7fffffffULL) return MPSR_OK;
    int slots = 0;
    if (int rc = sk_slots<BM, BN, WM, WN, MATH>(slots)) return rc;
    const int per_cu = g_sk_per_cu.load();
    if (per_cu > 0) {
        int dev = 0, cus = 256;
        MPSR_CHECK_HIP(hipGetDevice(&dev));
        MPSR_CHECK_HIP(hipDeviceGetAttribute(&cus, hipDeviceAttributeMultiprocessorCount, dev));
        slots = per_cu * cus;
    } else if (per_cu < 0) {
        slots = -per_cu;
    }
    long long G = slots;
    if (G > (long long)(U / 4)) G = (long long)(U / 4);
    G = G / 8 * 8;
    if (G < 8) G = 8;
    while (G > 8 && sk_scratch_floats((int)G, BM, BN, (long long)T) > (p.ws ? p.ws_floats : 0)) G -= 8;
    if (!p.ws || sk_scratch_floats((int)G, BM, BN, (long long)T) > p.ws_floats) return MPSR_OK;
    sk.G = (int)G;
    sk.U = (unsigned)U;
    sk.q = (unsigned)(U / G);
    sk.r = (unsigned)(U % G);
    sk.slabs = p.ws;
    sk.counters = reinterpret_cast<int *>(p.ws + (size_t)G * 2 * BM * BN);
    if (!counters_clean) MPSR_CHECK_HIP(hipMemsetAsync(sk.counters, 0, sizeof(int) * (size_t)T, s));
    hipLaunchKernelGGL((conv_sk_kernel<BM, BN, WM, WN, MATH>), dim3((unsigned)G), dim3(256), 0, s, p, sk);
    MPSR_CHECK_LAUNCH("conv_sk_kernel");
    done = true;
    return MPSR_OK;
}

}

namespace mpsr {

bool conv2d_takes_fc_rows(int H, int W, long long M, int C, int N, int KH, int KW, int split_k)
{
    const int pw = pointwise_override();
    return H == 1 && W == 1 && KH == 1 && KW == 1 && split_k <= 1 && pw != 0 && cur_math() == MATH_FP32 &&
           g_tile_override.load() < 0 && g_sched_override.load() < 0 && fc_rows_applies(M, C, N);
}

bool conv2d_takes_pointwise(long long M, int C, int N, int KH, int KW, int split_k)
{
    const int pw = pointwise_override();
    if (KH != 1 || KW != 1 || split_k > 1 || pw == 0 || cur_math() != MATH_FP32 || g_tile_override.load() >= 0 ||
        !pointwise_applies(M, C, N))
        return false;
    if (pw > 0) return true;
    if (g_sched_override.load() >= 0 || g_class_override.load() >= 0) return false;
    const long long tiles = ((M + 95) / 96) * ((N + 127) / 128);
    return split_k == 0 && N % 128 == 0 && tiles >= 512;
}

size_t conv_auto_split_floats() { return (size_t)1536 * 64 * 64; }
size_t conv_scratch_floats(long long M, int N)
{
    const size_t slabs = (size_t)1024 * 2 * 96 * 128;
    const size_t counters = (size_t)((M + 63) / 64 + 9) * (size_t)((N + 31) / 32);
    return slabs + counters;
}

int g_auto_split_target = 768;
constexpr int g_auto_split_enough = 768;
constexpr int g_auto_split_min_ksteps = 4;

int auto_split_k(int M, int N, int ksteps, const float *ws, size_t ws_floats)
{
    if (!ws) return 1;
    const long long tiles = (long long)ceil_div(M, 64) * ceil_div(N, 64);
    if (tiles >= g_auto_split_enough || tiles >= g_auto_split_target || N <= 32) return 1;
    long long s = (g_auto_split_target + tiles - 1) / tiles;
    if (s > 8) s = 8;
    if (s > ksteps / g_auto_split_min_ksteps) s = ksteps / g_auto_split_min_ksteps;
    while (s > 1 && (size_t)s * M * N > ws_floats) --s;
    return s < 1 ? 1 : (int)s;
}

static int winograd_mode()
{
    const int wino = g_wino_override.load();
    return (wino < 0 && cur_wino_policy() == MPSR_WINOGRAD_OFF) ? 0 : wino;
}
static bool accurate_only() { return g_wino_override.load() < 0 && cur_wino_policy() == MPSR_WINOGRAD_ACCURATE; }

bool conv2d_takes_winograd4(int B, int H, int W, int C, int N, const float *ws, size_t ws_floats)
{
    const long long M64 = (long long)B * H * W;
    const int wino = winograd_mode();
    if (accurate_only()) return false;
    return ws && (wino < 0 || wino == 2) && g_tile_override.load() < 0 && M64 >= 65536 && C >= 64 && N >= 64 &&
           winograd4_applies(H, W, C, N) && ws_floats >= winograd4_scratch_floats(C, N) && M64 * C * 4 < 0x7f000000LL;
}

bool conv2d_takes_winograd3(int B, int H, int W, int C, int N, int KH, int KW, int dilation, int split_k, const float *ws,
                            size_t ws_floats)
{
    const int wino = winograd_mode();
    const long long M64 = (long long)B * H * W;
    const bool can3 = KH == 3 && KW == 3 && split_k == 0 && ws && cur_math() == MATH_FP32 &&
                      winograd3_applies(H, W, C, dilation) && ws_floats >= winograd3_scratch_floats(C, N) &&
                      M64 * C * 4 < 0x7f000000LL;
    const int th = can3 ? H / (3 * dilation) : 1;
    const long long min_tiles = (can3 && th == 1 && winograd3_form(B, H, W, C, N, dilation) == 2) ? 1 : 1024;
    const int th_max = !g_wino3_halo.load() ? 1 : dilation > 1 ? 2 : conv2d_takes_winograd4(B, H, W, C, N, ws, ws_floats) ? 4 : 16;
    const bool want3 = wino == 3 || (wino < 0 && g_tile_override.load() < 0 && g_class_override.load() < 0 &&
                                     th <= th_max && (dilation > 1 || th > 1) &&
                                     (long long)B * dilation * dilation * th * th >= min_tiles && C >= 64 && N >= 64);
    if (accurate_only() && !(th == 1 && winograd3_form(B, H, W, C, N, dilation) == 2)) return false;
    return can3 && want3;
}

int conv2d_winograd_choice(int B, int H, int W, int C, int N, int KH, int KW, int dilation, bool residual, int split_k,
                           const float *ws, size_t ws_floats)
{
    const long long M64 = (long long)B * H * W;
    int wino = winograd_mode();
    const bool base = KH == 3 && KW == 3 && dilation == 1 && !residual && split_k <= 1 && ws;
    const bool atrous2 = KH == 3 && KW == 3 && dilation > 1 && !residual && split_k <= 1 && ws &&
                         winograd_applies_dilated(H, W, C, N, dilation) && M64 * C * 4 < 0x7f000000LL;
    const bool can2 = (base || atrous2) && cur_math() == MATH_FP32 && winograd_applies_dilated(H, W, C, N, dilation) &&
                      ws_floats >= winograd_scratch_floats(C, N);
    const bool can4 = base && winograd4_applies(H, W, C, N) && ws_floats >= winograd4_scratch_floats(C, N) &&
                      M64 * C * 4 < 0x7f000000LL;
    const long long atrous2_min = C >= 256 ? std::min(6000, g_atrous_wino2_min_pixels.load()) : g_atrous_wino2_min_pixels.load();
    if (wino < 0) wino = split_k != 0 ? 0 : (base && conv2d_takes_winograd4(B, H, W, C, N, ws, ws_floats)) ? 2
                         : (base && M64 >= 65536 && C >= 64 && N >= 64 && g_tile_override.load() < 0) ? 1
                         : (atrous2 && g_atrous_wino2.load() && M64 >= atrous2_min && C >= 64 && N >= 64 &&
                            g_tile_override.load() < 0 && g_class_override.load() < 0) ? 1 : 0;
    if (wino == 2 && can4) return 2;
    if ((wino == 1 || wino == 2) && can2) return 1;
    return 0;
}

int conv2d(const float *x, int B, int H, int W, int C, const float *w, const float *bias, const float *residual,
           float *y, int N, int KH, int KW, int dilation, int relu, int split_k, float *ws, size_t ws_floats,
           hipStream_t stream)
{
    MPSR_REQUIRE(B >= 0 && H > 0 && W > 0 && C > 0 && N > 0, "conv2d: bad shape (B=%d H=%d W=%d C=%d N=%d)", B, H, W,
                 C, N);
    MPSR_REQUIRE(KH >= 1 && KW >= 1 && (KH & 1) && (KW & 1) && dilation >= 1,
                 "conv2d: kernel %dx%d (odd sizes only) dilation %d", KH, KW, dilation);
    MPSR_REQUIRE(C % 4 == 0, "conv2d: C=%d must be a multiple of 4 (pad the channels)", C);
    if (B == 0) return MPSR_OK;
    MPSR_REQUIRE(x && w && y, "conv2d: null pointer");
    MPSR_REQUIRE(((uintptr_t)x & 15) == 0 && ((uintptr_t)w & 15) == 0, "conv2d: x and w must be 16-byte aligned");
    const long long M64 = (long long)B * H * W;
    MPSR_REQUIRE(M64 * C * 4 < 0xfffffff0LL && (long long)N * KH * KW * C * 4 < 0xfffffff0LL && M64 < 0x7fffffffLL,
                 "conv2d: tensor exceeds the 4 GiB addressable by one launch; split the batch");
    if (KH == 3 && KW == 3 && dilation == 1 && N <= 4 && C % 32 == 0 && !residual && split_k <= 1 &&
        g_tile_override.load() < 0 && ((uintptr_t)w & 3) == 0)
        return conv3x3_narrow(x, B, H, W, C, w, bias, relu, y, N, stream, 0);
    if (!residual && split_k <= 1 && g_tile_override.load() < 0 && cur_math() == MATH_FP32 &&
        thin_input_conv_applies(B, H, W, C, N, KH, KW, dilation))
        return thin_input_conv(x, B, H, W, w, bias, relu, y, N, stream);
    if (!residual && conv2d_takes_winograd3(B, H, W, C, N, KH, KW, dilation, split_k, ws, ws_floats))
        return conv3x3_winograd3(x, B, H, W, C, w, bias, relu, y, N, dilation, ws, ws_floats, stream);
    {
        const int wc = conv2d_winograd_choice(B, H, W, C, N, KH, KW, dilation, residual != nullptr, split_k, ws, ws_floats);
        if (wc == 2) return conv3x3_winograd4(x, B, H, W, C, w, bias, relu, y, N, ws, ws_floats, stream, 0, 0, nullptr, 0);
        if (wc == 1) return conv3x3_winograd(x, B, H, W, C, w, bias, relu, y, N, ws, ws_floats, stream, dilation);
    }
    if (conv2d_takes_pointwise(M64, C, N, KH, KW, split_k))
        return conv1x1_pointwise(x, M64, C, w, bias, residual, relu, y, N, stream);
    if (conv2d_takes_fc_rows(H, W, M64, C, N, KH, KW, split_k))
        return fc_rows(x, M64, C, w, bias, residual, relu, y, N, stream);
    if (H == 1 && W == 1 && KH == 1 && KW == 1 && !residual && split_k == 0 && pointwise_override() != 0 &&
        cur_math() == MATH_FP32 && g_tile_override.load() < 0 && g_sched_override.load() < 0 &&
        fc_rows_split_applies(M64, C, N, bias, y, ws, ws_floats))
        return fc_rows_split(x, M64, C, w, bias, relu, y, N, ws, stream);
    ConvParams p;
    p.x = x; p.w = w; p.bias = bias; p.residual = residual; p.y = y; p.ws = ws; p.ws_floats = ws ? ws_floats : 0;
    p.M = (int)M64; p.H = H; p.W = W; p.C = C; p.N = N; p.KH = KH; p.KW = KW; p.dil = dilation; p.relu = relu;
    p.xbytes = (unsigned)(M64 * C * 4);
    p.wbytes = (unsigned)((long long)N * KH * KW * C * 4);
    p.cblocks = ceil_div(C, BK);
    p.ksteps_total = KH * KW * p.cblocks;
    bool use_classes = KH == 3 && KW == 3 && dilation > 1;
    const int class_override = g_class_override.load(), tile_override = g_tile_override.load();
    const int math = cur_math();
    if (class_override == 0) use_classes = false;
    if (class_override == 1) use_classes = KH == 3 && KW == 3;
    int sel = tile_override;
    if (sel < 0) {
        if (N <= 32) sel = 4;
        else if (p.M >= 131072) sel = N <= 64 ? 1 : 0;
        else if (KH == 1 && KW == 1 && C >= 512 && N >= 256 && N % 128 == 0 && p.M >= 24576 && math == MATH_FP32) sel = 5;
        else sel = 3;
        if (math == MATH_BF16X3) sel = N <= 32 ? 4 : (p.M < 16384 ? 3 : ((N <= 64 || p.M < 131072) ? 1 : 0));
    }
    int sched = g_sched_override.load();
    if (sched < 0) sched = (split_k == 0 && ws && p.M <= 2048 && p.ksteps_total >= 128) ? 1 : 0;
    if (sched == 1 && split_k <= 1 && ws) {
        bool done = false;
        const int rc = with_tile(sel, [&](auto t) {
            using T = decltype(t);
            return math == MATH_BF16X3
                       ? launch_sk<T::BM, T::BN, T::WM, T::WN, MATH_BF16X3>(p, B, use_classes, sched, false, stream, done)
                       : launch_sk<T::BM, T::BN, T::WM, T::WN, MATH_FP32>(p, B, use_classes, sched, false, stream, done);
        });
        if (rc) return rc;
        if (done) return MPSR_OK;
    }
    if (split_k == 0) split_k = auto_split_k(p.M, N, p.ksteps_total, ws, ws_floats);
    if (split_k < 1) split_k = 1;
    if (split_k > p.ksteps_total) split_k = p.ksteps_total;
    p.ksteps_per_split = ceil_div(p.ksteps_total, split_k);
    p.splits = ceil_div(p.ksteps_total, p.ksteps_per_split);
    if (p.splits > 1) {
        if (!ws || ws_floats < (size_t)p.splits * p.M * N)
            return fail(MPSR_ERR_WORKSPACE, "conv2d: split_k=%d needs %zu workspace floats, got %zu", p.splits,
                        (size_t)p.splits * p.M * N, ws_floats);
    }
    int depth = g_depth_override.load();
    const bool plain64 = sel == 3 && KH == 1 && KW == 1 && C % BK == 0 && p.ksteps_total >= 8 && math == MATH_FP32;
    if (depth < 0) depth = ((sel == 3 && use_classes) || (sel == 5 && N <= 256) || plain64) ? 2 : 1;
    const int rc = with_tile(sel, [&](auto t) {
        using T = decltype(t);
        return math == MATH_BF16X3 ? launch<T::BM, T::BN, T::WM, T::WN, MATH_BF16X3>(p, B, use_classes, stream)
               : depth == 2        ? launch<T::BM, T::BN, T::WM, T::WN, MATH_FP32, 2>(p, B, use_classes, stream)
                                   : launch<T::BM, T::BN, T::WM, T::WN, MATH_FP32, 1>(p, B, use_classes, stream);
    });
    if (rc) return rc;
    if (p.splits > 1) {
        const long long MN = (long long)p.M * N;
        const int grid = (int)((MN + 255) / 256 < 65536 ? (MN + 255) / 256 : 65536);
        hipLaunchKernelGGL(splitk_reduce_kernel, dim3(grid), dim3(256), 0, stream, ws, p.splits, MN, N, bias, residual,
                           relu, y);
        MPSR_CHECK_LAUNCH("splitk_reduce_kernel");
    }
    return MPSR_OK;
}

}

extern "C" void mpsr_debug_set_auto_split_target(int workgroups) { mpsr::g_auto_split_target = workgroups; }
extern "C" void mpsr_debug_set_conv_tile(int sel) { g_tile_override = sel; }
extern "C" void mpsr_debug_set_conv_classes(int mode) { g_class_override = mode; }
extern "C" void mpsr_debug_set_conv_depth(int depth) { g_depth_override = depth; }
extern "C" void mpsr_debug_set_conv_plain(int mode) { g_plain_override = mode; }
extern "C" void mpsr_debug_set_conv_winograd(int mode) { g_wino_override = mode; }
extern "C" int mpsr_set_winograd_policy(int policy)
{
    MPSR_REQUIRE(policy == MPSR_WINOGRAD_AUTO || policy == MPSR_WINOGRAD_OFF || policy == MPSR_WINOGRAD_ACCURATE,
                 "set_winograd_policy: unknown policy %d", policy);
    g_wino_policy = policy;
    return MPSR_OK;
}
extern "C" int mpsr_get_winograd_policy(void) { return g_wino_policy; }
extern "C" void mpsr_debug_set_conv_sched(int mode, int per_cu)
{
    g_sched_override = mode;
    g_sk_per_cu = per_cu;
}

extern "C" int mpsr_set_conv_math(int mode)
{
    MPSR_REQUIRE(mode == MATH_FP32 || mode == MATH_BF16X3, "set_conv_math: unknown mode %d", mode);
    g_math = mode;
    return MPSR_OK;
}
extern "C" int mpsr_get_conv_math(void) { return g_math; }
extern "C" void mpsr_debug_set_wino3_halo(int on) { g_wino3_halo = on; }
extern "C" void mpsr_debug_set_atrous_wino2(int on, int min_pixels)
{
    g_atrous_wino2 = on;
    if (min_pixels > 0) g_atrous_wino2_min_pixels = min_pixels;
}

extern "C" int mpsr_conv2d_plan(int B, int H, int W, int C, int N, int KH, int KW, int dilation, int *kind,
                                double *executed_flops)
{
    MPSR_REQUIRE(B > 0 && H > 0 && W > 0 && C > 0 && N > 0 && kind && executed_flops, "conv2d_plan: bad arguments");
    const double M = (double)B * H * W;
    if (mpsr::conv2d_takes_winograd3(B, H, W, C, N, KH, KW, dilation, 0, reinterpret_cast<const float *>(16), ~(size_t)0)) {
        *kind = 4;
        *executed_flops = mpsr::winograd3_executed_flops(B, H, C, N, dilation);
        return MPSR_OK;
    }
    const int wc = mpsr::conv2d_winograd_choice(B, H, W, C, N, KH, KW, dilation, false, 0,
                                                reinterpret_cast<const float *>(16), ~(size_t)0);
    if (wc == 2) {
        *kind = 3;
        *executed_flops = 2.0 * (double)B * (H / 4) * (W / 4) * 36.0 * C * N;
        return MPSR_OK;
    }
    if (wc == 1) {
        *kind = 1;
        *executed_flops = 2.0 * (double)B * (H / 2) * (W / 2) * 16.0 * C * N;
        return MPSR_OK;
    }
    if (KH == 3 && KW == 3 && dilation == 1 && N <= 4 && C % 32 == 0) {
        *kind = 2;
        *executed_flops = 2.0 * M * 9.0 * C * N;
        return MPSR_OK;
    }
    if (mpsr::thin_input_conv_applies(B, H, W, C, N, KH, KW, dilation)) {
        *kind = 2;
        *executed_flops = 2.0 * M * 9.0 * C * N;
        return MPSR_OK;
    }
    if (mpsr::conv2d_takes_pointwise((long long)B * H * W, C, N, KH, KW, 0)) {
        *kind = 5;
        *executed_flops = 2.0 * M * C * N;
        return MPSR_OK;
    }
    if (mpsr::conv2d_takes_fc_rows(H, W, (long long)B * H * W, C, N, KH, KW, 0)) {
        *kind = 6;
        *executed_flops = 2.0 * M * C * N;
        return MPSR_OK;
    }
    *kind = 0;
    double taps = (double)KH * KW * H * W;
    if (KH == 3 && KW == 3 && dilation > 1 && H >= 2 * dilation && W >= 2 * dilation) {
        const double ty = 3.0 * H - 2.0 * dilation, tx = 3.0 * W - 2.0 * dilation;
        taps = ty * tx;
    }
    *executed_flops = 2.0 * (double)B * taps * C * N;
    return MPSR_OK;
}

extern "C" size_t mpsr_conv2d_scratch_floats(int B, int H, int W, int N)
{
    if (B <= 0 || H <= 0 || W <= 0 || N <= 0) return 0;
    size_t n = mpsr::conv_scratch_floats((long long)B * H * W, N);
    if (mpsr::g_wino4_split.load() != 0 && (long long)B * H * W >= 65536 && N % 128 == 0 && H % 4 == 0 && W % 4 == 0)
        n += mpsr::winograd4_split_floats(B, H, W, N) + 64;
    return n;
}

extern "C" int mpsr_conv2d_nhwc_f32(const float *x, int B, int H, int W, int C, const float *w, const float *bias,
                                    const float *residual, float *y, int N, int KH, int KW, int dilation, int relu,
                                    int split_k, float *ws, size_t ws_floats, mpsr_stream_t stream)
{
    return mpsr::conv2d(x, B, H, W, C, w, bias, residual, y, N, KH, KW, dilation, relu, split_k, ws, ws_floats,
                        mpsr::as_stream(stream));
}

extern "C" int mpsr_conv2d_nhwc_f32_ex(const float *x, int B, int H, int W, int C, const float *w, const float *bias,
                                       const float *residual, float *y, int N, int KH, int KW, int dilation, int relu,
                                       int split_k, float *ws, size_t ws_floats, const mpsr_conv_opts *opts,
                                       mpsr_stream_t stream)
{
    if (opts) {
        MPSR_REQUIRE(opts->math >= 0 && opts->math <= MPSR_CALL_MATH_BF16X3, "conv2d: unknown opts.math %d", opts->math);
        MPSR_REQUIRE(opts->winograd_policy >= 0 && opts->winograd_policy <= MPSR_CALL_WINOGRAD_ACCURATE,
                     "conv2d: unknown opts.winograd_policy %d", opts->winograd_policy);
    }
    mpsr::CallOptsGuard guard(opts ? opts->math : 0, opts ? opts->winograd_policy : 0);
    return mpsr::conv2d(x, B, H, W, C, w, bias, residual, y, N, KH, KW, dilation, relu, split_k, ws, ws_floats,
                        mpsr::as_stream(stream));
}

extern "C" int mpsr_conv2d_relu_masked_f32(const float *x, int B, int H, int W, int C, const float *w, const float *mask,
                                           float *y, int N, int KH, int KW, int dilation, float *ws, size_t ws_floats,
                                           mpsr_stream_t stream)
{
    MPSR_REQUIRE(mask, "conv2d_relu_masked: null mask");
    hipStream_t s = mpsr::as_stream(stream);
    if (B > 0 && x && w && y && mpsr::conv2d_takes_winograd3(B, H, W, C, N, KH, KW, dilation, 0, ws, ws_floats))
        return mpsr::conv3x3_winograd3(x, B, H, W, C, w, nullptr, 0, y, N, dilation, ws, ws_floats, s, mask);
    if (int rc = mpsr::conv2d(x, B, H, W, C, w, nullptr, nullptr, y, N, KH, KW, dilation, 0, 0, ws, ws_floats, s)) return rc;
    return mpsr_relu_grad(y, mask, y, (long long)B * H * W * N, stream);
}
```

### monopsr_amd/csrc/internal.h

```cpp
#pragma once
#include <hip/hip_runtime.h>

#include <atomic>
#include <cstddef>

#include "monopsr_hip.h"

namespace mpsr {

char *error_buffer();
extern thread_local int t_call_math;
extern thread_local int t_call_wino_policy;

int conv2d(const float *x, int B, int H, int W, int C, const float *w, const float *bias, const float *residual,
           float *y, int N, int KH, int KW, int dilation, int relu, int split_k, float *ws, size_t ws_floats,
           hipStream_t stream);
size_t conv_scratch_floats(long long M, int N);
bool conv2d_takes_winograd4(int B, int H, int W, int C, int N, const float *ws, size_t ws_floats);
bool conv2d_takes_winograd3(int B, int H, int W, int C, int N, int KH, int KW, int dilation, int split_k, const float *ws,
                            size_t ws_floats);
bool conv2d_takes_pointwise(long long M, int C, int N, int KH, int KW, int split_k);
int conv2d_winograd_choice(int B, int H, int W, int C, int N, int KH, int KW, int dilation, bool residual, int split_k,
                           const float *ws, size_t ws_floats);

int conv3x3_narrow(const float *x, int B, int H, int W, int C, const float *w, const float *bias, int relu, float *y,
                   int N, hipStream_t s, int in_c8);
bool conv3x3_narrow_takes_mfma(const float *x, int B, int H, int W, int C, int N, const float *w);
int resize_bilinear_c8(const float *in, int B, int H, int W, int C, int OH, int OW, int align_corners, float *out,
                       hipStream_t s);

size_t winograd_scratch_floats(int C, int N);
bool winograd_applies(int H, int W, int C, int N);
bool winograd_applies_dilated(int H, int W, int C, int N, int dilation);
int conv3x3_winograd(const float *x, int B, int H, int W, int C, const float *w, const float *bias, int relu, float *y,
                     int N, float *ws, size_t ws_floats, hipStream_t s, int dilation);
extern std::atomic<int> g_wino_waves;

size_t winograd4_scratch_floats(int C, int N);
bool winograd4_applies(int H, int W, int C, int N);
int conv3x3_winograd4(const float *x, int B, int H, int W, int C, const float *w, const float *bias, int relu,
                      float *y, int N, float *ws, size_t ws_floats, hipStream_t s, int in_c8, int out_c8, float *part,
                      size_t part_floats);
size_t winograd4_split_floats(int B, int H, int W, int N);
extern std::atomic<int> g_wino4_split;

size_t winograd3_scratch_floats(int C, int N);
bool winograd3_applies(int H, int W, int C, int dilation);
double winograd3_executed_flops(int B, int H, int C, int N, int dilation);
int winograd3_form(int B, int H, int W, int C, int N, int dilation);
int winograd3_filter_form(int B, int H, int W, int C, int N, int dilation);
int conv3x3_winograd3(const float *x, int B, int H, int W, int C, const float *w, const float *bias, int relu,
                      float *y, int N, int dilation, float *ws, size_t ws_floats, hipStream_t s,
                      const float *mask = nullptr);
struct FilterTailJob {
    const float *w = nullptr;
    float *u = nullptr;
    int N = 0, C = 0;
    int form = 0;
};
extern thread_local FilterTailJob g_filter_tail_job;
extern thread_local FilterTailJob g_filter_tail_done;
struct FilterCacheSlot {
    const float *w = nullptr;
    float *u = nullptr;
    size_t floats = 0;
    bool ready = false;
    int *tag = nullptr;
    bool holds(int kind)
    {
        const bool ok = ready && (!tag || *tag == kind);
        if (tag) *tag = kind;
        return ok;
    }
};
enum { FILTER_FORM_WINO4 = 1, FILTER_FORM_WINO3 = 2, FILTER_FORM_UPCONV = 3, FILTER_FORM_WINO3Z = 4, FILTER_FORM_WINO2 = 5 };
extern thread_local FilterCacheSlot g_filter_cache_slot;

bool winograd3w_applies(int B, int H, int W, int C, int N, int dilation);
long long winograd3w_workgroups(int B, int N, int dilation);
int launch_winograd3w(const float *x, int B, int H, int W, int C, const float *u, const float *bias, int relu, float *y,
                      int N, int dilation, hipStream_t s, const float *mask);

int launch_winograd3z(const float *x, int B, int H, int W, int C, const float *u, const float *bias, int relu, float *y,
                      int N, int dilation, hipStream_t s, const float *mask, float *part, size_t part_floats);
int launch_winograd3z_filter(const float *w, int N, int C, float *u, hipStream_t s);
int winograd_slices(long long blocks, int want_blocks, int cblocks, int min_steps, size_t part_floats, size_t y_floats);
int winograd_finish_slices(const float *part, const float *bias, float *y, size_t y_floats, int nslices, int N, int relu,
                           hipStream_t s);

struct WgradSlices {
    int tiles, steps, nslices;
};
WgradSlices wgrad_tile_slices(int tiles, int blocks, int workgroups, int kt);

bool winograd3_wgrad_applies(int B, int H, int W, int C, int N, int KH, int KW, int dilation);
WgradSlices winograd3_wgrad_slices(int B, int dilation, int C, int N);
int conv3x3_wgrad_winograd3(const float *x, const float *dy, int B, int H, int W, int C, int N, int dilation, float *dw,
                            float *db, hipStream_t s);

bool pointwise_applies(long long M, int K, int N);
bool pointwise_masked_applies(long long M, int K, int N);
int pointwise_override();
int conv1x1_pointwise(const float *x, long long M, int K, const float *w, const float *bias, const float *residual,
                      int relu, float *y, int N, hipStream_t s);
int conv1x1_pointwise_masked(const float *x, long long M, int K, const float *w, const float *bias, const float *residual,
                             const unsigned *mask, float *y, int N, hipStream_t s);
int conv1x1_pointwise_emit(const float *x, long long M, int K, const float *w, const float *bias, const float *residual,
                           int relu, float *y, unsigned *bits, int N, hipStream_t s);
bool fc_rows_applies(long long M, int K, int N);
bool fc_rows_split_applies(long long M, int K, int N, const float *bias, const float *y, const float *ws, size_t ws_floats);
int fc_rows_split(const float *x, long long M, int K, const float *w, const float *bias, int relu, float *y, int N,
                  float *ws, hipStream_t s);
int fc_rows(const float *x, long long M, int K, const float *w, const float *bias, const float *residual, int relu,
            float *y, int N, hipStream_t s);

int conv2d_wgrad_direct_plan(int B, int H, int W, int C, int N, int KH, int KW, int dilation, bool dy_aligned, int *kind);

bool thin_input_conv_applies(int B, int H, int W, int C, int N, int KH, int KW, int dilation);
int thin_input_conv(const float *x, int B, int H, int W, const float *w, const float *bias, int relu, float *y, int N,
                    hipStream_t s);
bool thin_wgrad_applies(int B, int H, int W, int C, int N, int KH, int KW, int dilation);
int thin_wgrad(const float *x, const float *dy, int B, int H, int W, int C, float *dw, float *db, hipStream_t s);

bool upconv_applies(int B, int h, int w, int C, int OH, int OW, int N, int align_corners);
size_t upconv_z_floats(long long Msrc, int N);
size_t upconv_weight_floats(int C, int N);
int conv3x3_upsampled(const float *x, int B, int h, int w, int C, int OH, int OW, int align_corners, const float *g,
                      const float *bias, int relu, float *y, int N, int out_c8, float *z, size_t z_floats, float *ws,
                      size_t ws_floats, hipStream_t s);

}
```

### monopsr_amd/csrc/network.hip

```cpp
#include <atomic>
#include <vector>

#include "common.h"

static std::atomic<int> g_decoder_c8{1};
extern "C" void mpsr_debug_set_decoder_c8(int on) { g_decoder_c8 = on; }
static std::atomic<int> g_decoder_upconv{1};
extern "C" void mpsr_debug_set_decoder_upconv(int on) { g_decoder_upconv = on; }

namespace {

struct Arena {
    char *base;
    size_t size, used = 0;
    bool ok = true;
    Arena(void *p, size_t n) : base(static_cast<char *>(p)), size(n) {}
    float *floats(size_t n)
    {
        const size_t bytes = mpsr::align_up(n * sizeof(float), 256);
        if (used + bytes > size) {
            ok = false;
            return nullptr;
        }
        float *r = reinterpret_cast<float *>(base + used);
        used += bytes;
        return r;
    }
};

inline size_t fbytes(size_t n) { return mpsr::align_up(n * sizeof(float), 256); }

int run_layer(const float *blob, const mpsr_layer &L, const float *x, int B, int H, int W, const float *residual,
              float *y, int split_k, float *ws, size_t ws_floats, hipStream_t s)
{
    return mpsr::conv2d(x, B, H, W, L.cin, blob + L.w_off, L.b_off >= 0 ? blob + L.b_off : nullptr, residual, y, L.cout,
                        L.kh, L.kw, L.dilation, L.relu, split_k, ws, ws_floats, s);
}

constexpr int kTrunkUnits[3] = {3, 4, 23};

inline size_t cache_floats_of(const mpsr_layer &L)
{
    if (L.kh != 3 || L.kw != 3) return 0;
    return mpsr::align_up((size_t)(L.dilation > 1 ? 25 : 36) * (size_t)L.cout * (size_t)L.cin, 64);
}

struct FilterCache {
    float *base = nullptr;
    size_t floats = 0, used = 0;
    bool valid = false;
    int *tags = nullptr;
    explicit FilterCache(const mpsr_net_opts *o)
    {
        if (o && o->filter_cache && o->filter_cache_floats) {
            base = o->filter_cache;
            floats = o->filter_cache_floats;
            valid = o->filter_cache_valid != 0;
            tags = o->filter_cache_tags;
        }
    }
    float *take(const mpsr_layer &L)
    {
        const size_t need = cache_floats_of(L);
        if (!base || need == 0) return nullptr;
        float *r = used + need <= floats ? base + used : nullptr;
        used += need;
        return r;
    }
    void offer(const float *w, float *slice, const mpsr_layer &L, int layer_index) const
    {
        mpsr::g_filter_cache_slot = mpsr::FilterCacheSlot();
        if (slice) {
            mpsr::g_filter_cache_slot.w = w;
            mpsr::g_filter_cache_slot.u = slice;
            mpsr::g_filter_cache_slot.floats = cache_floats_of(L);
            mpsr::g_filter_cache_slot.ready = valid;
            mpsr::g_filter_cache_slot.tag = tags ? tags + layer_index : nullptr;
        }
    }
};

struct TrunkDims {
    int OH, OW, PH, PW;
};
inline TrunkDims trunk_dims(int H, int W)
{
    TrunkDims d;
    d.OH = (H + 6 - 7) / 2 + 1;
    d.OW = (W + 6 - 7) / 2 + 1;
    d.PH = (d.OH + 1) / 2;
    d.PW = (d.OW + 1) / 2;
    return d;
}

}


extern "C" size_t mpsr_trunk_workspace_bytes(int B, int H, int W)
{
    if (B <= 0 || H <= 0 || W <= 0) return 0;
    const TrunkDims d = trunk_dims(H, W);
    const size_t Mr = (size_t)B * d.OH * d.OW, Mp = (size_t)B * d.PH * d.PW;
    return fbytes(Mr * 160) + fbytes(Mr * 64) + fbytes(Mp * 64) + 3 * fbytes(Mp * 1024) + 2 * fbytes(Mp * 256) +
           fbytes(mpsr::conv_scratch_floats((long long)(Mr > Mp ? Mr : Mp), 1024));
}

extern "C" size_t mpsr_filter_cache_floats(const mpsr_layer *layers, int n_layers)
{
    size_t n = 0;
    if (layers)
        for (int i = 0; i < n_layers; ++i) n += cache_floats_of(layers[i]);
    return n;
}

extern "C" int mpsr_trunk_fwd(const float *img, int B, int H, int W, const float *blob, const mpsr_layer *layers,
                              int n_layers, float *out, void *workspace, size_t workspace_bytes, mpsr_stream_t stream)
{
    return mpsr_trunk_fwd_ex(img, B, H, W, blob, layers, n_layers, out, workspace, workspace_bytes, nullptr, stream);
}

extern "C" int mpsr_trunk_fwd_ex(const float *img, int B, int H, int W, const float *blob, const mpsr_layer *layers,
                                 int n_layers, float *out, void *workspace, size_t workspace_bytes,
                                 const mpsr_net_opts *opts, mpsr_stream_t stream)
{
    MPSR_REQUIRE(B >= 0 && H >= 7 && W >= 7, "trunk_fwd: bad input shape (B=%d H=%d W=%d)", B, H, W);
    if (opts) {
        MPSR_REQUIRE(opts->math >= 0 && opts->math <= MPSR_CALL_MATH_BF16X3, "%s: unknown opts.math %d", "trunk_fwd", opts->math);
        MPSR_REQUIRE(opts->winograd_policy >= 0 && opts->winograd_policy <= MPSR_CALL_WINOGRAD_ACCURATE,
                     "%s: unknown opts.winograd_policy %d", "trunk_fwd", opts->winograd_policy);
    }
    mpsr::CallOptsGuard call_opts(opts ? opts->math : 0, opts ? opts->winograd_policy : 0);
    MPSR_REQUIRE(n_layers == MPSR_TRUNK_LAYERS, "trunk_fwd: expected %d layer records, got %d", MPSR_TRUNK_LAYERS,
                 n_layers);
    if (B == 0) return MPSR_OK;
    MPSR_REQUIRE(img && blob && layers && out && workspace, "trunk_fwd: null pointer");
    hipStream_t s = mpsr::as_stream(stream);
    const TrunkDims d = trunk_dims(H, W);
    const size_t Mr = (size_t)B * d.OH * d.OW, Mp = (size_t)B * d.PH * d.PW;
    const mpsr_layer &root = layers[0];
    MPSR_REQUIRE(root.kh == 1 && root.kw == 1 && root.cin >= 147 && root.cin % 32 == 0,
                 "trunk_fwd: layer 0 must be the root as a 1x1 layer over im2col columns (cin=%d)", root.cin);
    int cmax = 0, bmax = 0;
    for (int i = 1; i < n_layers; ++i) {
        if (layers[i].kh == 3 && layers[i].cout > bmax) bmax = layers[i].cout;
        if (layers[i].cout > cmax) cmax = layers[i].cout;
    }
    Arena ar(workspace, workspace_bytes);
    float *cols = ar.floats(Mr * root.cin);
    float *rootout = ar.floats(Mr * root.cout);
    float *pooled = ar.floats(Mp * root.cout);
    float *ping = ar.floats(Mp * cmax), *pong = ar.floats(Mp * cmax), *scut = ar.floats(Mp * cmax);
    float *t1 = ar.floats(Mp * bmax), *t2 = ar.floats(Mp * bmax);
    const size_t skn = mpsr::conv_scratch_floats((long long)(Mr > Mp ? Mr : Mp), cmax > 1024 ? cmax : 1024);
    float *sk = ar.floats(skn);
    if (!ar.ok)
        return mpsr::fail(MPSR_ERR_WORKSPACE, "trunk_fwd: workspace %zu bytes too small (see mpsr_trunk_workspace_bytes)",
                          workspace_bytes);

    int rc;
    struct TailJobGuard {
        ~TailJobGuard()
        {
            mpsr::g_filter_tail_job = mpsr::FilterTailJob();
            mpsr::g_filter_tail_done = mpsr::FilterTailJob();
            mpsr::g_filter_cache_slot = mpsr::FilterCacheSlot();
        }
    } tail_job_guard;
    FilterCache cache(opts);
    if ((rc = mpsr_im2col_root(img, B, H, W, cols, root.cin, stream))) return rc;
    if ((rc = run_layer(blob, root, cols, B, d.OH, d.OW, nullptr, rootout, 0, sk, skn, s))) return rc;
    if ((rc = mpsr_max_pool(rootout, B, d.OH, d.OW, root.cout, 3, 2, 1, pooled, stream))) return rc;

    const float *cur = pooled;
    int cur_c = root.cout;
    int li = 1;
    for (int blk = 0; blk < 3; ++blk) {
        for (int u = 0; u < kTrunkUnits[blk]; ++u) {
            const bool last = (blk == 2 && u == kTrunkUnits[blk] - 1);
            const float *residual = cur;
            if (u == 0) {
                const mpsr_layer &S = layers[li++];
                MPSR_REQUIRE(S.kh == 1 && S.cin == cur_c && !S.relu, "trunk_fwd: record %d is not a shortcut", li - 1);
                if ((rc = run_layer(blob, S, cur, B, d.PH, d.PW, nullptr, scut, 0, sk, skn, s))) return rc;
                residual = scut;
            }
            const mpsr_layer &c1 = layers[li], &c2 = layers[li + 1], &c3 = layers[li + 2];
            li += 3;
            MPSR_REQUIRE(c1.kh == 1 && c1.cin == cur_c && c2.kh == 3 && c2.cin == c1.cout && c3.kh == 1 &&
                             c3.cin == c2.cout && (u == 0 || c3.cout == cur_c),
                         "trunk_fwd: records %d..%d do not form a bottleneck unit", li - 3, li - 1);
            float *dst = last ? out : (cur == ping ? pong : ping);
            float *uslice = cache.take(c2);
            const int c2i = (int)(&c2 - layers);
            const int fform = mpsr::winograd3_filter_form(B, d.PH, d.PW, c2.cin, c2.cout, c2.dilation);
            const bool cached_u = uslice && cache.valid && (!cache.tags || cache.tags[c2i] == fform);
            if (!cached_u &&
                mpsr::conv2d_takes_pointwise((long long)B * d.PH * d.PW, c1.cin, c1.cout, 1, 1, 0) &&
                mpsr::conv2d_takes_winograd3(B, d.PH, d.PW, c2.cin, c2.cout, c2.kh, c2.kw, c2.dilation, 0, sk, skn)) {
                mpsr::g_filter_tail_job.w = blob + c2.w_off;
                mpsr::g_filter_tail_job.u = uslice ? uslice : sk;
                mpsr::g_filter_tail_job.N = c2.cout;
                mpsr::g_filter_tail_job.C = c2.cin;
                mpsr::g_filter_tail_job.form = fform == mpsr::FILTER_FORM_WINO3Z ? 1 : 0;
            }
            if ((rc = run_layer(blob, c1, cur, B, d.PH, d.PW, nullptr, t1, 0, sk, skn, s))) return rc;
            mpsr::g_filter_tail_job = mpsr::FilterTailJob();
            cache.offer(blob + c2.w_off, uslice, c2, c2i);
            rc = run_layer(blob, c2, t1, B, d.PH, d.PW, nullptr, t2, 0, sk, skn, s);
            mpsr::g_filter_cache_slot = mpsr::FilterCacheSlot();
            if (rc) return rc;
            if ((rc = run_layer(blob, c3, t2, B, d.PH, d.PW, residual, dst, 0, sk, skn, s))) return rc;
            cur = dst;
            cur_c = c3.cout;
        }
    }
    return MPSR_OK;
}


namespace {
struct DecoderChoice {
    bool c8, up1, up2, xyz_c8;
};
DecoderChoice decoder_choice(int B, int fh, int fw, int mh, int mw, const mpsr_layer *L, const float *blob, bool feat_map,
                             bool xyz_map, const float *sk, size_t skn)
{
    const int hh = mh / 2, hw = mw / 2;
    const int csq = L[1].cout, c2 = L[2].cout, c3 = L[4].cout;
    DecoderChoice ch;
    ch.xyz_c8 = !feat_map && xyz_map && L[6].kh == 3 && L[6].kw == 3 && L[6].dilation == 1 &&
                mpsr::conv3x3_narrow_takes_mfma(nullptr, B, mh, mw, L[6].cin, L[6].cout, blob ? blob + L[6].w_off : nullptr);
    const bool k3 = L[2].kh == 3 && L[3].kh == 3 && L[4].kh == 3 && L[5].kh == 3 && L[2].kw == 3 && L[3].kw == 3 &&
                    L[4].kw == 3 && L[5].kw == 3 && L[2].dilation == 1 && L[3].dilation == 1 && L[4].dilation == 1 &&
                    L[5].dilation == 1;
    const bool upok = g_decoder_upconv.load() != 0 && k3 && mpsr_get_conv_math() == MPSR_MATH_FP32;
    ch.up1 = upok && mpsr::upconv_applies(B, fh, fw, csq, hh, hw, c2, 1) && skn >= mpsr::upconv_weight_floats(csq, c2);
    ch.up2 = upok && mpsr::upconv_applies(B, hh, hw, c2, mh, mw, c3, 1) && skn >= mpsr::upconv_weight_floats(c2, c3);
    ch.c8 = g_decoder_c8.load() != 0 && csq % 8 == 0 && c2 % 8 == 0 && c3 % 8 == 0 && k3 &&
            (ch.up1 || mpsr::conv2d_takes_winograd4(B, hh, hw, L[2].cin, L[2].cout, sk, skn)) &&
            mpsr::conv2d_takes_winograd4(B, hh, hw, L[3].cin, L[3].cout, sk, skn) &&
            (ch.up2 || mpsr::conv2d_takes_winograd4(B, mh, mw, L[4].cin, L[4].cout, sk, skn)) &&
            mpsr::conv2d_takes_winograd4(B, mh, mw, L[5].cin, L[5].cout, sk, skn);
    if (!ch.c8) ch.xyz_c8 = false;
    return ch;
}
}

extern "C" int mpsr_squash_decoder_plan(int B, int fh, int fw, int mh, int mw, const mpsr_layer *L, int n_layers,
                                        int *kinds, double *executed_flops)
{
    MPSR_REQUIRE(B > 0 && fh >= 2 && fw >= 2 && mh >= 2 && mw >= 2 && L && n_layers == MPSR_DECODER_LAYERS && kinds &&
                     executed_flops,
                 "squash_decoder_plan: bad arguments");
    const int hh = mh / 2, hw = mw / 2;
    const size_t Mm = (size_t)B * mh * mw;
    int cwide = L[1].cout;
    for (int i = 2; i < n_layers; ++i) cwide = L[i].cout > cwide ? L[i].cout : cwide;
    const size_t skn = mpsr::conv_scratch_floats((long long)Mm, cwide > 512 ? cwide : 512);
    const DecoderChoice ch = decoder_choice(B, fh, fw, mh, mw, L, nullptr, false, true, reinterpret_cast<const float *>(256), skn);
    const int hs[7] = {fh, fh, hh, hh, mh, mh, mh}, ws[7] = {fw, fw, hw, hw, mw, mw, mw};
    for (int i = 0; i < 7; ++i) {
        int rc;
        if ((i == 2 && ch.up1) || (i == 4 && ch.up2)) {
            const int sh = i == 2 ? fh : hh, sw = i == 2 ? fw : hw;
            kinds[i] = 7;
            executed_flops[i] = 2.0 * (double)B * sh * sw * (double)L[i].cin * 9.0 * (double)L[i].cout;
        } else if (ch.c8 && (i == 2 || i == 3 || i == 4 || i == 5)) {
            kinds[i] = 3;
            executed_flops[i] = 2.0 * (double)B * (hs[i] / 4) * (ws[i] / 4) * 36.0 * (double)L[i].cin * (double)L[i].cout;
        } else if ((rc = mpsr_conv2d_plan(B, hs[i], ws[i], L[i].cin, L[i].cout, L[i].kh, L[i].kw, L[i].dilation, &kinds[i],
                                          &executed_flops[i])))
            return rc;
    }
    return MPSR_OK;
}

extern "C" size_t mpsr_decoder_workspace_bytes(int B, int fh, int fw, int mh, int mw)
{
    if (B <= 0) return 0;
    const size_t Mf = (size_t)B * fh * fw, Mh = (size_t)B * (mh / 2) * (mw / 2), Mm = (size_t)B * mh * mw;
    const size_t parth = mpsr::winograd4_split_floats(B, mh / 2, mw / 2, 256), partm = mpsr::winograd4_split_floats(B, mh, mw, 128);
    const size_t part = mpsr::g_wino4_split.load() != 0 ? fbytes((parth > partm ? parth : partm) + 64) : 0;
    const size_t r1 = Mh * 512 > Mf * 9 * 256 ? Mh * 512 : Mf * 9 * 256, r2 = Mm * 256 > Mh * 9 * 128 ? Mm * 256 : Mh * 9 * 128;
    return 2 * fbytes(Mf * 512) + fbytes(r1) + 2 * fbytes(Mh * 256) + fbytes(r2) + 2 * fbytes(Mm * 128) +
           fbytes(mpsr::conv_scratch_floats((long long)Mm, 512)) + part;
}

extern "C" int mpsr_squash_decoder_fwd(const float *crop_feat, const float *full_feat, int B, int fh, int fw, int mh,
                                       int mw, const float *blob, const mpsr_layer *L, int n_layers,
                                       float *feat_box3d, float *feat_map, float *xyz_map, void *workspace,
                                       size_t workspace_bytes, mpsr_stream_t stream)
{
    return mpsr_squash_decoder_fwd_ex(crop_feat, full_feat, B, fh, fw, mh, mw, blob, L, n_layers, feat_box3d, feat_map,
                                      xyz_map, workspace, workspace_bytes, nullptr, stream);
}

extern "C" int mpsr_squash_decoder_fwd_ex(const float *crop_feat, const float *full_feat, int B, int fh, int fw, int mh,
                                          int mw, const float *blob, const mpsr_layer *L, int n_layers,
                                          float *feat_box3d, float *feat_map, float *xyz_map, void *workspace,
                                          size_t workspace_bytes, const mpsr_net_opts *opts, mpsr_stream_t stream)
{
    MPSR_REQUIRE(B >= 0 && fh >= 2 && fw >= 2 && mh >= 2 && mw >= 2 && mh % 2 == 0 && mw % 2 == 0,
                 "squash_decoder_fwd: bad shape");
    if (opts) {
        MPSR_REQUIRE(opts->math >= 0 && opts->math <= MPSR_CALL_MATH_BF16X3, "%s: unknown opts.math %d", "squash_decoder_fwd", opts->math);
        MPSR_REQUIRE(opts->winograd_policy >= 0 && opts->winograd_policy <= MPSR_CALL_WINOGRAD_ACCURATE,
                     "%s: unknown opts.winograd_policy %d", "squash_decoder_fwd", opts->winograd_policy);
    }
    mpsr::CallOptsGuard call_opts(opts ? opts->math : 0, opts ? opts->winograd_policy : 0);
    MPSR_REQUIRE(n_layers == MPSR_DECODER_LAYERS, "squash_decoder_fwd: expected %d layer records, got %d",
                 MPSR_DECODER_LAYERS, n_layers);
    if (B == 0) return MPSR_OK;
    MPSR_REQUIRE(crop_feat && full_feat && blob && L && feat_box3d && workspace,
                 "squash_decoder_fwd: null pointer");
    hipStream_t s = mpsr::as_stream(stream);
    const int hh = mh / 2, hw = mw / 2;
    const size_t Mf = (size_t)B * fh * fw, Mh = (size_t)B * hh * hw, Mm = (size_t)B * mh * mw;
    const int csq = L[1].cout, c2 = L[2].cout, c3 = L[4].cout;
    MPSR_REQUIRE(L[0].cout == csq && L[2].cin == csq && L[3].cin == c2 && L[4].cin == c2 && L[5].cin == c3 &&
                     L[6].cin == c3,
                 "squash_decoder_fwd: layer records are not squash_a, squash_b, conv2_1, conv2_2, conv3_1, conv3_2, xyz");
    Arena ar(workspace, workspace_bytes);
    float *part = ar.floats(Mf * csq), *sq = ar.floats(Mf * csq);
    const size_t r1n = Mh * csq > Mf * 9 * (size_t)c2 ? Mh * csq : Mf * 9 * (size_t)c2;
    const size_t r2n = Mm * c2 > Mh * 9 * (size_t)c3 ? Mm * c2 : Mh * 9 * (size_t)c3;
    float *r1 = ar.floats(r1n), *a = ar.floats(Mh * c2), *b = ar.floats(Mh * c2);
    float *r2 = ar.floats(r2n), *c = ar.floats(Mm * c3);
    float *fm = feat_map ? feat_map : ar.floats(Mm * c3);
    int cwide = csq;
    for (int i = 2; i < n_layers; ++i) cwide = L[i].cout > cwide ? L[i].cout : cwide;
    const size_t skn = mpsr::conv_scratch_floats((long long)Mm, cwide > 512 ? cwide : 512);
    float *sk = ar.floats(skn);
    size_t partn = 0;
    float *partb = nullptr;
    if (ar.ok && mpsr::g_wino4_split.load() != 0 && c2 % 128 == 0 && c3 % 128 == 0 && hh % 4 == 0 && hw % 4 == 0 && mh % 4 == 0 && mw % 4 == 0) {
        const size_t a1 = mpsr::winograd4_split_floats(B, hh, hw, c2), a2 = mpsr::winograd4_split_floats(B, mh, mw, c3);
        partn = (a1 > a2 ? a1 : a2) + 64;
        partb = ar.floats(partn);
        if (!ar.ok) {
            ar.ok = true;
            partb = nullptr;
            partn = 0;
        }
    }
    if (!ar.ok)
        return mpsr::fail(MPSR_ERR_WORKSPACE, "squash_decoder_fwd: workspace %zu bytes too small", workspace_bytes);
    int rc;
    if ((rc = run_layer(blob, L[0], crop_feat, B, fh, fw, nullptr, part, 0, sk, skn, s))) return rc;
    if ((rc = run_layer(blob, L[1], full_feat, B, fh, fw, part, sq, 0, sk, skn, s))) return rc;
    if ((rc = mpsr_max_pool(sq, B, fh, fw, csq, 2, 2, 0, feat_box3d, stream))) return rc;
    if (opts && opts->ready_event) MPSR_CHECK_HIP(hipEventRecord(reinterpret_cast<hipEvent_t>(opts->ready_event), s));
    struct SlotGuard {
        ~SlotGuard() { mpsr::g_filter_cache_slot = mpsr::FilterCacheSlot(); }
    } slot_guard;
    FilterCache cache(opts);
    const DecoderChoice ch = decoder_choice(B, fh, fw, mh, mw, L, blob, feat_map != nullptr, xyz_map != nullptr, sk, skn);
    const bool xyz_c8 = ch.xyz_c8, up1 = ch.up1, up2 = ch.up2, c8 = ch.c8;
    if (c8) {
        auto wino = [&](const mpsr_layer &Lr, const float *x, int H, int W, float *y, int in_c8, int out_c8) {
            cache.offer(blob + Lr.w_off, cache.take(Lr), Lr, (int)(&Lr - L));
            return mpsr::conv3x3_winograd4(x, B, H, W, Lr.cin, blob + Lr.w_off, Lr.b_off >= 0 ? blob + Lr.b_off : nullptr,
                                           Lr.relu, y, Lr.cout, sk, skn, s, in_c8, out_c8, partb, partn);
        };
        auto upconv = [&](const mpsr_layer &Lr, const float *x, int h, int w, int H, int W, float *y, float *z, size_t zn) {
            cache.offer(blob + Lr.w_off, cache.take(Lr), Lr, (int)(&Lr - L));
            return mpsr::conv3x3_upsampled(x, B, h, w, Lr.cin, H, W, 1, blob + Lr.w_off,
                                           Lr.b_off >= 0 ? blob + Lr.b_off : nullptr, Lr.relu, y, Lr.cout, 1, z, zn, sk,
                                           skn, s);
        };
        if (up1) {
            if ((rc = upconv(L[2], sq, fh, fw, hh, hw, a, r1, r1n))) return rc;
        } else {
            if ((rc = mpsr::resize_bilinear_c8(sq, B, fh, fw, csq, hh, hw, 1, r1, s))) return rc;
            if ((rc = wino(L[2], r1, hh, hw, a, 1, 1))) return rc;
        }
        if ((rc = wino(L[3], a, hh, hw, b, 1, 0))) return rc;
        if (up2) {
            if ((rc = upconv(L[4], b, hh, hw, mh, mw, c, r2, r2n))) return rc;
        } else {
            if ((rc = mpsr::resize_bilinear_c8(b, B, hh, hw, c2, mh, mw, 1, r2, s))) return rc;
            if ((rc = wino(L[4], r2, mh, mw, c, 1, 1))) return rc;
        }
        if ((rc = wino(L[5], c, mh, mw, fm, 1, xyz_c8 ? 1 : 0))) return rc;
        if (xyz_map) {
            if (xyz_c8)
                rc = mpsr::conv3x3_narrow(fm, B, mh, mw, L[6].cin, blob + L[6].w_off,
                                          L[6].b_off >= 0 ? blob + L[6].b_off : nullptr, L[6].relu, xyz_map, L[6].cout, s, 1);
            else
                rc = run_layer(blob, L[6], fm, B, mh, mw, nullptr, xyz_map, 1, nullptr, 0, s);
            if (rc) return rc;
        }
        return MPSR_OK;
    }
    auto cached = [&](const mpsr_layer &Lr, const float *x, int H, int W, float *y) {
        cache.offer(blob + Lr.w_off, cache.take(Lr), Lr, (int)(&Lr - L));
        return run_layer(blob, Lr, x, B, H, W, nullptr, y, 0, sk, skn, s);
    };
    auto upconv_nhwc = [&](const mpsr_layer &Lr, const float *x, int h, int w, int H, int W, float *y, float *z, size_t zn) {
        cache.offer(blob + Lr.w_off, cache.take(Lr), Lr, (int)(&Lr - L));
        return mpsr::conv3x3_upsampled(x, B, h, w, Lr.cin, H, W, 1, blob + Lr.w_off,
                                       Lr.b_off >= 0 ? blob + Lr.b_off : nullptr, Lr.relu, y, Lr.cout, 0, z, zn, sk, skn, s);
    };
    if (up1) {
        if ((rc = upconv_nhwc(L[2], sq, fh, fw, hh, hw, a, r1, r1n))) return rc;
    } else {
        if ((rc = mpsr_resize_bilinear(sq, B, fh, fw, csq, hh, hw, 1, r1, stream))) return rc;
        if ((rc = cached(L[2], r1, hh, hw, a))) return rc;
    }
    if ((rc = cached(L[3], a, hh, hw, b))) return rc;
    if (up2) {
        if ((rc = upconv_nhwc(L[4], b, hh, hw, mh, mw, c, r2, r2n))) return rc;
    } else {
        if ((rc = mpsr_resize_bilinear(b, B, hh, hw, c2, mh, mw, 1, r2, stream))) return rc;
        if ((rc = cached(L[4], r2, mh, mw, c))) return rc;
    }
    if ((rc = cached(L[5], c, mh, mw, fm))) return rc;
    if (xyz_map && (rc = run_layer(blob, L[6], fm, B, mh, mw, nullptr, xyz_map, 1, nullptr, 0, s))) return rc;
    return MPSR_OK;
}


namespace {

struct HeadIn {
    const float *boxes, *cam_p, *view, *mean_lwh, *z_off;
    const int *cls;
    const int *cam_idx;
    int n_cams;
    mpsr_head_consts k;
};
__device__ const float kBadCam[12] = {__builtin_nanf(""), __builtin_nanf(""), __builtin_nanf(""), __builtin_nanf(""),
                                      __builtin_nanf(""), __builtin_nanf(""), __builtin_nanf(""), __builtin_nanf(""),
                                      __builtin_nanf(""), __builtin_nanf(""), __builtin_nanf(""), __builtin_nanf("")};
__device__ __forceinline__ const float *cam_of(const HeadIn &in, int b)
{
    if (!in.cam_idx) return in.cam_p;
    const int i = in.cam_idx[b];
    return (i >= 0 && i < in.n_cams) ? in.cam_p + 12 * i : kBadCam;
}

__device__ __forceinline__ float common_feature(const HeadIn &in, int b, int j)
{
    const float *bx = in.boxes + 4 * b;
    const float *cam = cam_of(in, b);
    const float cu = cam[2], cv = cam[6];
    if (j < 4) {
        const float centre = (j & 1) ? cu : cv;
        const float half = ((j & 1) ? in.k.image_w : in.k.image_h) / 2.0f;
        return (bx[j] - centre) / half;
    }
    if (j == 4) return (bx[2] - bx[0]) / in.k.image_h;
    if (j == 5) return in.view[b];
    return (in.cls[b] == j - 6) ? 1.0f : 0.0f;
}

__constant__ float kCamNorm[12] = {1000.f, 1.f, 1000.f, 100.f, 1.f, 1000.f, 1000.f, 1.f, 1.f, 1.f, 1.f, 1.f};

__global__ __launch_bounds__(256) void head_concat_prop_kernel(HeadIn in, const float *__restrict__ imgfc,
                                                               int imgfc_stride, int nfc, int kpad, int B,
                                                               float *__restrict__ out)
{
    const int i = blockIdx.x * blockDim.x + threadIdx.x;
    if (i >= B * kpad) return;
    const int b = i / kpad, col = i - b * kpad;
    const int ncommon = 6 + in.k.num_classes;
    float v = 0.f;
    if (col < nfc) v = imgfc[(size_t)b * imgfc_stride + col];
    else if (col < nfc + ncommon) v = common_feature(in, b, col - nfc);
    else if (col < nfc + ncommon + 12) v = cam_of(in, b)[col - nfc - ncommon] / kCamNorm[col - nfc - ncommon];
    out[i] = v;
}

__global__ __launch_bounds__(256) void head_prop_outputs_kernel(HeadIn in, const float *__restrict__ pout, int B,
                                                                mpsr_head_outputs o, float *__restrict__ prop)
{
    const int b = blockIdx.x * blockDim.x + threadIdx.x;
    if (b >= B) return;
    const int nb = in.k.num_alpha_bins, stride = 3 + 2 * nb;
    const float *p = pout + (size_t)b * stride;
    float lwh[3];
    for (int j = 0; j < 3; ++j) {
        lwh[j] = in.mean_lwh[3 * b + j] + p[j];
        if (o.lwh) o.lwh[3 * b + j] = lwh[j];
        if (o.lwh_offs) o.lwh_offs[3 * b + j] = p[j];
    }
    for (int j = 0; j < nb; ++j) {
        if (o.alpha_bins) o.alpha_bins[(size_t)b * nb + j] = p[3 + j];
        if (o.alpha_regs) o.alpha_regs[(size_t)b * nb + j] = p[3 + nb + j];
    }
    const float *bx = in.boxes + 4 * b;
    const float focal = cam_of(in, b)[0], cv = cam_of(in, b)[6];
    const float z = focal * lwh[2] / (bx[2] - bx[0]) + in.z_off[b];
    const float centre_v = (bx[2] + bx[0]) / 2.0f - cv;
    const float y = centre_v * (z / focal) - in.k.cen_y_class_offset;
    if (o.prop_cen_z) o.prop_cen_z[b] = z;
    prop[2 * b] = y;
    prop[2 * b + 1] = z;
}

__global__ __launch_bounds__(256) void head_concat_reg_kernel(HeadIn in, const float *__restrict__ imgfc,
                                                              int imgfc_stride, int nfc, int kpad, int B,
                                                              const float *__restrict__ pout,
                                                              const float *__restrict__ prop, float *__restrict__ out)
{
    const int i = blockIdx.x * blockDim.x + threadIdx.x;
    if (i >= B * kpad) return;
    const int b = i / kpad, col = i - b * kpad;
    const int ncommon = 6 + in.k.num_classes, nout = 3 + 2 * in.k.num_alpha_bins;
    float v = 0.f;
    if (col < nfc) v = imgfc[(size_t)b * imgfc_stride + nfc + col];
    else if (col < nfc + ncommon) v = common_feature(in, b, col - nfc);
    else if (col < nfc + ncommon + nout) v = pout[(size_t)b * nout + (col - nfc - ncommon)];
    else if (col == nfc + ncommon + nout) v = prop[2 * b] / in.k.cen_y_norm;
    else if (col == nfc + ncommon + nout + 1) v = prop[2 * b + 1] / in.k.max_depth;
    out[i] = v;
}

__global__ __launch_bounds__(256) void head_final_kernel(HeadIn in, const float *__restrict__ rout,
                                                         const float *__restrict__ prop, int B, mpsr_head_outputs o)
{
    const int b = blockIdx.x * blockDim.x + threadIdx.x;
    if (b >= B) return;
    const float yo = rout[2 * b], zo = rout[2 * b + 1];
    const float y = prop[2 * b] + yo, z = prop[2 * b + 1] + zo;
    const float x = z * tanf(in.view[b]) + (-cam_of(in, b)[3] / cam_of(in, b)[0]);
    if (o.cen_y) o.cen_y[b] = y;
    if (o.cen_y_offs) o.cen_y_offs[b] = yo;
    if (o.cen_z) o.cen_z[b] = z;
    if (o.cen_z_offs) o.cen_z_offs[b] = zo;
    if (o.cen_x) o.cen_x[b] = x;
    if (o.centroids) {
        o.centroids[3 * b] = x;
        o.centroids[3 * b + 1] = y;
        o.centroids[3 * b + 2] = z;
    }
}

}

extern "C" size_t mpsr_heads_workspace_bytes(int B, int feat_elems)
{
    if (B <= 0 || feat_elems <= 0) return 0;
    const size_t b = (size_t)B;
    return fbytes(b * 2048) + fbytes(mpsr::conv_scratch_floats(B, 2048)) + 2 * fbytes(b * 1152) + 4 * fbytes(b * 1024) +
           fbytes(b * 64) + fbytes(b * 2) + fbytes(b * 2);
}

extern "C" int mpsr_heads_fwd(const float *feat_box3d, int B, int feat_elems, const float *boxes_2d,
                              const float *cam_p, const float *view_angs, const int *class_idx, const float *mean_lwh,
                              const float *cen_z_offset, const mpsr_head_consts *consts, const float *blob,
                              const mpsr_layer *L, int n_layers, const mpsr_head_outputs *outs, void *workspace,
                              size_t workspace_bytes, mpsr_stream_t stream)
{
    return mpsr_heads_fwd_cams(feat_box3d, B, feat_elems, boxes_2d, cam_p, 1, nullptr, view_angs, class_idx, mean_lwh,
                               cen_z_offset, consts, blob, L, n_layers, outs, workspace, workspace_bytes, stream);
}

extern "C" int mpsr_heads_fwd_cams(const float *feat_box3d, int B, int feat_elems, const float *boxes_2d,
                                   const float *cam_p, int n_cams, const int *cam_index, const float *view_angs,
                                   const int *class_idx, const float *mean_lwh, const float *cen_z_offset,
                                   const mpsr_head_consts *consts, const float *blob, const mpsr_layer *L, int n_layers,
                                   const mpsr_head_outputs *outs, void *workspace, size_t workspace_bytes,
                                   mpsr_stream_t stream)
{
    MPSR_REQUIRE(n_cams >= 1, "heads_fwd: n_cams = %d", n_cams);
    MPSR_REQUIRE(B >= 0 && feat_elems > 0 && feat_elems % 4 == 0, "heads_fwd: bad shape (B=%d feat=%d)", B, feat_elems);
    MPSR_REQUIRE(n_layers == MPSR_HEAD_LAYERS, "heads_fwd: expected %d layer records, got %d", MPSR_HEAD_LAYERS,
                 n_layers);
    if (B == 0) return MPSR_OK;
    MPSR_REQUIRE(feat_box3d && boxes_2d && cam_p && view_angs && class_idx && mean_lwh && cen_z_offset && consts &&
                     blob && L && outs && workspace,
                 "heads_fwd: null pointer");
    const int nfc = L[0].cout / 2;
    const int nb = consts->num_alpha_bins, nc = consts->num_classes;
    const int prop_in = nfc + 6 + nc + 12, reg_in = nfc + 6 + nc + 3 + 2 * nb + 2;
    MPSR_REQUIRE(L[0].cin == feat_elems && L[1].cin >= prop_in && L[1].cin % 4 == 0 && L[3].cout == 3 + 2 * nb &&
                     L[4].cin >= reg_in && L[4].cin % 4 == 0 && L[6].cout == 2 && L[1].cin <= 1152 && L[4].cin <= 1152 &&
                     L[1].cout <= 1024 && L[2].cout <= 1024 && L[4].cout <= 1024 && L[5].cout <= 1024 && nfc <= 1024 &&
                     3 + 2 * nb <= 64,
                 "heads_fwd: layer records do not match the head graph");
    hipStream_t s = mpsr::as_stream(stream);
    Arena ar(workspace, workspace_bytes);
    const size_t b = (size_t)B;
    float *imgfc = ar.floats(b * L[0].cout);
    const size_t skn = mpsr::conv_scratch_floats(B, L[0].cout > 2048 ? L[0].cout : 2048);
    float *skws = ar.floats(skn);
    float *cat_p = ar.floats(b * L[1].cin), *cat_r = ar.floats(b * L[4].cin);
    float *h1 = ar.floats(b * L[1].cout), *h2 = ar.floats(b * L[2].cout);
    float *g1 = ar.floats(b * L[4].cout), *g2 = ar.floats(b * L[5].cout);
    float *pout = ar.floats(b * L[3].cout), *rout = ar.floats(b * 2), *prop = ar.floats(b * 2);
    if (!ar.ok) return mpsr::fail(MPSR_ERR_WORKSPACE, "heads_fwd: workspace %zu bytes too small", workspace_bytes);

    HeadIn in;
    in.boxes = boxes_2d; in.cam_p = cam_p; in.view = view_angs; in.mean_lwh = mean_lwh; in.z_off = cen_z_offset;
    in.cls = class_idx; in.cam_idx = cam_index; in.n_cams = n_cams; in.k = *consts;
    int rc;
    if ((rc = run_layer(blob, L[0], feat_box3d, B, 1, 1, nullptr, imgfc, 0, skws, skn, s))) return rc;
    {
        const int total = B * L[1].cin;
        hipLaunchKernelGGL(head_concat_prop_kernel, dim3(mpsr::ceil_div(total, 256)), dim3(256), 0, s, in, imgfc,
                           L[0].cout, nfc, L[1].cin, B, cat_p);
        MPSR_CHECK_LAUNCH("head_concat_prop_kernel");
    }
    if ((rc = run_layer(blob, L[1], cat_p, B, 1, 1, nullptr, h1, 1, nullptr, 0, s))) return rc;
    if ((rc = run_layer(blob, L[2], h1, B, 1, 1, nullptr, h2, 1, nullptr, 0, s))) return rc;
    if ((rc = run_layer(blob, L[3], h2, B, 1, 1, nullptr, pout, 1, nullptr, 0, s))) return rc;
    hipLaunchKernelGGL(head_prop_outputs_kernel, dim3(mpsr::ceil_div(B, 256)), dim3(256), 0, s, in, pout, B, *outs, prop);
    MPSR_CHECK_LAUNCH("head_prop_outputs_kernel");
    {
        const int total = B * L[4].cin;
        hipLaunchKernelGGL(head_concat_reg_kernel, dim3(mpsr::ceil_div(total, 256)), dim3(256), 0, s, in, imgfc,
                           L[0].cout, nfc, L[4].cin, B, pout, prop, cat_r);
        MPSR_CHECK_LAUNCH("head_concat_reg_kernel");
    }
    if ((rc = run_layer(blob, L[4], cat_r, B, 1, 1, nullptr, g1, 1, nullptr, 0, s))) return rc;
    if ((rc = run_layer(blob, L[5], g1, B, 1, 1, nullptr, g2, 1, nullptr, 0, s))) return rc;
    if ((rc = run_layer(blob, L[6], g2, B, 1, 1, nullptr, rout, 1, nullptr, 0, s))) return rc;
    hipLaunchKernelGGL(head_final_kernel, dim3(mpsr::ceil_div(B, 256)), dim3(256), 0, s, in, rout, prop, B, *outs);
    MPSR_CHECK_LAUNCH("head_final_kernel");
    return MPSR_OK;
}
```

### monopsr_amd/csrc/winograd3.hip

```cpp
#include <atomic>
#include <type_traits>

#include "common.h"
#include "wino3_filter.h"
#include "wino3_transforms.h"

namespace {

using f32x16 = __attribute__((ext_vector_type(16))) float;

namespace f3 {
constexpr int MT = 32, NT = 64, KC = 8, NP = 25;
constexpr int APOS = MT * KC;
constexpr int ABUF = NP * APOS;
constexpr int MEXF = NP * 16 * NT;
constexpr int LDSF = MEXF > 2 * ABUF ? MEXF : 2 * ABUF;
constexpr unsigned OOB = 0x80000000u;
}

struct Wino3Params {
    const float *x, *u, *bias;
    float *y;
    int B, H, W, C, N, dil, T;
    int th;
    int cblocks, nblocks, mblocks, relu;
    unsigned xbytes, ubytes;
    const float *mask;
};

__global__ __launch_bounds__(256) void wino3_filter_kernel(const float *__restrict__ w, int N, int C, float *__restrict__ u)
{
    const long long i = (long long)blockIdx.x * 256 + threadIdx.x;
    if (i < (long long)N * C) mpsr::wino3_filter_one(w, N, C, u, i);
}

using mpsr::w3t::bt5;
using mpsr::w3t::at3;

template <int V>
using IC3 = std::integral_constant<int, V>;

template <int NPOS, int DG, bool HALO>
__device__ __forceinline__ void wino3_body(const Wino3Params &p, const int n0, const int t0, float *lds)
{
    using namespace f3;
    constexpr int NU = NPOS == 7 ? 3 : 2;
    const int tid = threadIdx.x, lane = tid & 63;
    const int wave = __builtin_amdgcn_readfirstlane(tid >> 6);
    const int pg = wave >> 1, nh = wave & 1;
    const int gpos = 6 * pg;
    const int nsteps = p.cblocks;
    const int d = p.dil;

    const int lt = 8 * (wave & 3) + (lane >> 3), ch = lane & 7;
    const int th = HALO ? p.th : 1, tpi = d * d * th * th;
    unsigned abase;
    unsigned voffc[3][3];
    const unsigned shift = HALO ? (unsigned)(d * p.W + d) * (unsigned)p.C * 4u : 0u;
    char *xback = const_cast<char *>(reinterpret_cast<const char *>(p.x)) - shift;
    {
        const int t = t0 + lt;
        const int img = t / tpi, rem = t - img * tpi;
        const int sub = rem / (th * th), tt = rem - sub * th * th;
        const int a = sub / d, b = sub - a * d, ty = tt / th, tx = tt - ty * th;
        abase = t < p.T ? (unsigned)(((img * p.H + a + 3 * d * ty) * p.W + b + 3 * d * tx) * p.C + ch) * 4u : OOB;
        const bool rowc[3] = {ty > 0, true, ty < th - 1}, colc[3] = {tx > 0, true, tx < th - 1};
#pragma unroll
        for (int u = 0; u < 3; ++u)
#pragma unroll
            for (int v = 0; v < 3; ++v) voffc[u][v] = (t < p.T && rowc[u] && colc[v]) ? abase : OOB;
    }
    float pa[25];
    auto load_patch1 = [&](int step, int L) __attribute__((always_inline)) {
        const bool live = step < nsteps;
        if constexpr (HALO) {
            const int s_ = L / 5, r_ = L % 5;
            const __amdgpu_buffer_rsrc_t rr =
                __builtin_amdgcn_make_buffer_rsrc(xback, 0, live ? (int)(p.xbytes + shift) : 0, 0x00020000);
            const unsigned so = (unsigned)((d * r_ * p.W + d * s_) * p.C + (live ? step : 0) * KC) * 4u;
            pa[5 * r_ + s_] = __builtin_bit_cast(
                float, __builtin_amdgcn_raw_buffer_load_b32(rr, voffc[r_ == 0 ? 0 : r_ == 4 ? 2 : 1][s_ == 0 ? 0 : s_ == 4 ? 2 : 1],
                                                            so, 0));
        } else {
            const int j = L / 3, i = L % 3;
            const __amdgpu_buffer_rsrc_t rr =
                __builtin_amdgcn_make_buffer_rsrc(const_cast<float *>(p.x), 0, live ? (int)p.xbytes : 0, 0x00020000);
            const unsigned so = (unsigned)((d * i * p.W + d * j) * p.C + (live ? step : 0) * KC) * 4u;
            pa[5 * (i + 1) + (j + 1)] = __builtin_bit_cast(float, __builtin_amdgcn_raw_buffer_load_b32(rr, abase, so, 0));
        }
    };
    auto vertical = [&](int j) __attribute__((always_inline)) {
        float t0_, t1_, t2_, t3_, t4_;
        if constexpr (HALO) {
            bt5(pa[5 + j], pa[10 + j], pa[15 + j], t0_, t1_, t2_, t3_, t4_);
            pa[j] = fmaf(2.f, pa[j], t0_);
            pa[5 + j] = t1_;
            pa[10 + j] = t2_;
            pa[15 + j] = t3_;
            pa[20 + j] = pa[20 + j] + t4_;
            return;
        }
        bt5(pa[5 + j + 1], pa[10 + j + 1], pa[15 + j + 1], t0_, t1_, t2_, t3_, t4_);
        pa[j + 1] = t0_;
        pa[5 + j + 1] = t1_;
        pa[10 + j + 1] = t2_;
        pa[15 + j + 1] = t3_;
        pa[20 + j + 1] = t4_;
    };
    auto horizontal = [&](int r) __attribute__((always_inline)) {
        float t0_, t1_, t2_, t3_, t4_;
        bt5(pa[5 * r + 1], pa[5 * r + 2], pa[5 * r + 3], t0_, t1_, t2_, t3_, t4_);
        if constexpr (HALO) {
            t0_ = fmaf(2.f, pa[5 * r], t0_);
            t4_ = pa[5 * r + 4] + t4_;
        }
        pa[5 * r] = t0_;
        pa[5 * r + 1] = t1_;
        pa[5 * r + 2] = t2_;
        pa[5 * r + 3] = t3_;
        pa[5 * r + 4] = t4_;
    };
    float *awr = lds + lt * 8 + 4 * ((ch >> 2) ^ ((lt >> 3) & 1)) + (ch & 3);
    auto store_a = [&](int buf, int pos) __attribute__((always_inline)) {
        awr[buf * ABUF + pos * APOS] = pa[pos];
    };

    const unsigned bvoff = n0 + 32 * nh + (lane & 31) < p.N
                               ? (unsigned)((n0 + 32 * nh + (lane & 31)) * KC + 4 * (lane >> 5)) * 4u : OOB;
    const unsigned bpstride = (unsigned)p.N * KC * 4u;
    float4 fb[NU][3];
    auto load_b1 = [&](int step, int q, int set, int j) __attribute__((always_inline)) {
        const bool live = step < nsteps;
        const __amdgpu_buffer_rsrc_t rr =
            __builtin_amdgcn_make_buffer_rsrc(const_cast<float *>(p.u), 0, live ? (int)p.ubytes : 0, 0x00020000);
        const unsigned so = ((unsigned)(live ? step : 0) * (unsigned)NP + (unsigned)(gpos + q)) * bpstride;
        fb[set][j] = __builtin_bit_cast(float4, __builtin_amdgcn_raw_buffer_load_b128(rr, bvoff, so, 0));
    };
    const float *ard = lds + gpos * APOS + (lane & 31) * 8 + 4 * ((lane >> 5) ^ (((lane & 31) >> 3) & 1));
    float4 fa[3];

    f32x16 acc[NPOS];
#pragma unroll
    for (int q = 0; q < NPOS; ++q)
#pragma unroll
        for (int e = 0; e < 16; ++e) acc[q][e] = 0.f;

    auto kstep = [&](int s, auto buf_c, auto &&duty) __attribute__((always_inline)) {
        constexpr int buf = decltype(buf_c)::value;
#pragma unroll
        for (int u = 0; u < NU; ++u) {
            const int np = u < 2 ? 3 : 1;
#pragma unroll
            for (int j = 0; j < 3; ++j)
                if (j < np) fa[j] = *reinterpret_cast<const float4 *>(ard + buf * ABUF + (3 * u + j) * APOS);
            __builtin_amdgcn_sched_barrier(0);
#pragma unroll
            for (int k = 0; k < 4; ++k)
#pragma unroll
                for (int j = 0; j < 3; ++j) {
                    if (j >= np) continue;
                    const int m = 12 * u + np * k + j;
                    const float av = k == 0 ? fa[j].x : k == 1 ? fa[j].y : k == 2 ? fa[j].z : fa[j].w;
                    const float bv = k == 0 ? fb[u][j].x : k == 1 ? fb[u][j].y : k == 2 ? fb[u][j].z : fb[u][j].w;
                    acc[3 * u + j] = __builtin_amdgcn_mfma_f32_32x32x2f32(av, bv, acc[3 * u + j], 0, 0, 0);
                    if (k == 0) {
                        const int un = (u + 1) % NU, npn = un < 2 ? 3 : 1;
                        if (j < npn) load_b1(u + 1 < NU ? s : s + 1, 3 * un + j, un, j);
                        if (np == 1 && npn == 3) {
                            load_b1(u + 1 < NU ? s : s + 1, 3 * un + 1, un, 1);
                            load_b1(u + 1 < NU ? s : s + 1, 3 * un + 2, un, 2);
                        }
                    }
                    if (m < 24) duty(m);
                    __builtin_amdgcn_sched_barrier(0);
                }
        }
    };
    auto request = [&](int step) __attribute__((always_inline)) {
        return [&, step](int slot) __attribute__((always_inline)) {
            if constexpr (HALO) {
                load_patch1(step, slot);
                if (slot == 23) load_patch1(step, 24);
            } else {
                if (slot >= 3 && slot < 12) load_patch1(step, slot - 3);
            }
        };
    };
    auto transform = [&](auto buf_c) __attribute__((always_inline)) {
        return [&](int slot) __attribute__((always_inline)) {
            constexpr int buf = decltype(buf_c)::value;
            if constexpr (HALO) {
                if (slot < 5) vertical(slot);
                else if (slot < 15 && ((slot - 5) & 1) == 0) horizontal((slot - 5) >> 1);
                if (slot >= 6 && slot < 16) {
                    const int r = (slot - 6) >> 1;
                    if (((slot - 6) & 1) == 0) {
                        store_a(buf, 5 * r);
                        store_a(buf, 5 * r + 1);
                        store_a(buf, 5 * r + 2);
                    } else {
                        store_a(buf, 5 * r + 3);
                        store_a(buf, 5 * r + 4);
                    }
                }
                return;
            }
            if (slot < 3) vertical(slot);
            else if (slot < 13 && ((slot - 3) & 1) == 0) horizontal((slot - 3) >> 1);
            if (slot >= 4 && slot < 14) {
                const int r = (slot - 4) >> 1;
                if (((slot - 4) & 1) == 0) {
                    store_a(buf, 5 * r);
                    store_a(buf, 5 * r + 1);
                    store_a(buf, 5 * r + 2);
                } else {
                    store_a(buf, 5 * r + 3);
                    store_a(buf, 5 * r + 4);
                }
            }
        };
    };

#pragma unroll
    for (int j = 0; j < 3; ++j) load_b1(0, j, 0, j);
#pragma unroll
    for (int i = 0; i < (HALO ? 25 : 9); ++i) load_patch1(DG, i);
    if (DG == 0) {
#pragma unroll
        for (int j = 0; j < (HALO ? 5 : 3); ++j) vertical(j);
#pragma unroll
        for (int r = 0; r < 5; ++r) horizontal(r);
#pragma unroll
        for (int i = 0; i < 25; ++i) store_a(0, i);
    }
    __syncthreads();

    if (DG == 0) {
        for (int s = 0; s < nsteps; s += 2) {
            kstep(s, IC3<0>{}, request(s + 2));
            __syncthreads();
            kstep(s + 1, IC3<1>{}, transform(IC3<0>{}));
            __syncthreads();
        }
    } else {
        for (int s = 0; s < nsteps; s += 2) {
            kstep(s, IC3<0>{}, transform(IC3<1>{}));
            __syncthreads();
            kstep(s + 1, IC3<1>{}, request(s + 3));
            __syncthreads();
        }
    }
    int tid2 = tid;
    if constexpr (NPOS == 7)
        asm volatile("s_nop 15\n\ts_nop 7"
                     : "+v"(acc[0]), "+v"(acc[1]), "+v"(acc[2]), "+v"(acc[3]), "+v"(acc[4]), "+v"(acc[5]), "+v"(acc[6]),
                       "+v"(tid2));
    else
        asm volatile("s_nop 15\n\ts_nop 7"
                     : "+v"(acc[0]), "+v"(acc[1]), "+v"(acc[2]), "+v"(acc[3]), "+v"(acc[4]), "+v"(acc[5]), "+v"(tid2));

    const int lane2 = tid2 & 63;
    float *mwr = lds + gpos * (16 * NT) + (4 * (lane2 >> 5)) * NT + 32 * nh + (lane2 & 31);
    const float *mrd = lds + (tid2 >> 5) * NT + (tid2 & 31);
    float bias2[2];
#pragma unroll
    for (int h = 0; h < 2; ++h) {
        const int n = n0 + (tid2 & 31) + 32 * h;
        bias2[h] = (p.bias && n < p.N) ? p.bias[n] : 0.f;
    }
#pragma unroll
    for (int round = 0; round < 2; ++round) {
        if (round) __syncthreads();
#pragma unroll
        for (int q = 0; q < NPOS; ++q)
#pragma unroll
            for (int e8 = 0; e8 < 8; ++e8) {
                const int trow = (e8 & 3) + 8 * (e8 >> 2);
                mwr[q * (16 * NT) + trow * NT] = acc[q][8 * round + e8];
            }
        const int tt = t0 + 16 * round + (tid2 >> 5);
        const int img = tt / tpi, rem = tt - img * tpi;
        const int sub = rem / (th * th), tq = rem - sub * th * th;
        const int a = sub / d + 3 * d * (tq / th), b = sub % d + 3 * d * (tq % th);
        float mk[2][9];
        if (p.mask) {
#pragma unroll
            for (int h = 0; h < 2; ++h) {
                const int n = n0 + (tid2 & 31) + 32 * h;
                const bool ok = tt < p.T && n < p.N;
                const float *mo = p.mask + ((size_t)(img * p.H + a) * p.W + b) * p.N + n;
#pragma unroll
                for (int j = 0; j < 3; ++j)
#pragma unroll
                    for (int i = 0; i < 3; ++i) mk[h][3 * j + i] = ok ? mo[((size_t)(d * i) * p.W + d * j) * p.N] : 0.f;
            }
        }
        __syncthreads();
#pragma unroll
        for (int h = 0; h < 2; ++h) {
            float z[5][3];
#pragma unroll
            for (int u = 0; u < 5; ++u) {
                float m[5];
#pragma unroll
                for (int v = 0; v < 5; ++v) m[v] = mrd[(5 * u + v) * (16 * NT) + 32 * h];
                at3(m[0], m[1], m[2], m[3], m[4], z[u][0], z[u][1], z[u][2]);
            }
            const int n = n0 + (tid2 & 31) + 32 * h;
            const bool ok = tt < p.T && n < p.N;
            float *o = p.y + ((size_t)(img * p.H + a) * p.W + b) * p.N + n;
#pragma unroll
            for (int j = 0; j < 3; ++j) {
                float yv[3];
                at3(z[0][j], z[1][j], z[2][j], z[3][j], z[4][j], yv[0], yv[1], yv[2]);
#pragma unroll
                for (int i = 0; i < 3; ++i) {
                    float v = yv[i] + bias2[h];
                    if (p.relu) v = fmaxf(v, 0.f);
                    if (p.mask) v = mk[h][3 * j + i] > 0.f ? v : 0.f;
                    if (ok) o[((size_t)(d * i) * p.W + d * j) * p.N] = v;
                }
            }
        }
    }
}

__global__ __launch_bounds__(512) __attribute__((amdgpu_waves_per_eu(2, 2))) void wino3_conv_kernel(const Wino3Params p)
{
    extern __shared__ __attribute__((aligned(16))) float lds[];
    const int xcd = blockIdx.x & 7, l_ = blockIdx.x >> 3;
    const int nb = l_ % p.nblocks;
    const int mb = (l_ / p.nblocks) * 8 + xcd;
    if (mb >= p.mblocks) return;
    const int n0 = nb * f3::NT, t0 = mb * f3::MT;
    const int wave = __builtin_amdgcn_readfirstlane(threadIdx.x >> 6);
    if (wave < 4) wino3_body<6, 0, false>(p, n0, t0, lds);
    else if (wave < 6) wino3_body<6, 1, false>(p, n0, t0, lds);
    else wino3_body<7, 1, false>(p, n0, t0, lds);
}

__global__ __launch_bounds__(512) __attribute__((amdgpu_waves_per_eu(2, 2))) void wino3h_conv_kernel(const Wino3Params p)
{
    extern __shared__ __attribute__((aligned(16))) float lds[];
    const int xcd = blockIdx.x & 7, l_ = blockIdx.x >> 3;
    const int nb = l_ % p.nblocks;
    const int mb = (l_ / p.nblocks) * 8 + xcd;
    if (mb >= p.mblocks) return;
    const int n0 = nb * f3::NT, t0 = mb * f3::MT;
    const int wave = __builtin_amdgcn_readfirstlane(threadIdx.x >> 6);
    if (wave < 4) wino3_body<6, 0, true>(p, n0, t0, lds);
    else if (wave < 6) wino3_body<6, 1, true>(p, n0, t0, lds);
    else wino3_body<7, 1, true>(p, n0, t0, lds);
}

}

namespace mpsr {

std::atomic<int> g_wino3_form{-1};

int winograd3_form(int B, int H, int W, int C, int N, int dilation)
{
    const int th = H / (3 * dilation);
    if (th != 1 || !winograd3w_applies(B, H, W, C, N, dilation)) return 0;
    const int form = g_wino3_form.load();
    return (form >= 0 && form <= 2) ? form : 2;
}
int winograd3_filter_form(int B, int H, int W, int C, int N, int dilation)
{
    return winograd3_form(B, H, W, C, N, dilation) == 2 ? FILTER_FORM_WINO3Z : FILTER_FORM_WINO3;
}

thread_local FilterTailJob g_filter_tail_job;
thread_local FilterTailJob g_filter_tail_done;
thread_local FilterCacheSlot g_filter_cache_slot;

size_t winograd3_scratch_floats(int C, int N) { return (size_t)f3::NP * N * C; }

bool winograd3_applies(int H, int W, int C, int dilation)
{
    return dilation >= 1 && H == W && H % (3 * dilation) == 0 && H / (3 * dilation) <= 16 && C % 16 == 0 && C >= 16;
}

long long winograd3_tiles(int B, int H, int dilation)
{
    const int th = H / (3 * dilation);
    return (long long)B * dilation * dilation * th * th;
}
double winograd3_executed_flops(int B, int H, int C, int N, int dilation)
{
    const double products = winograd3_form(B, H, H, C, N, dilation) == 2 ? 16.0 : 25.0;
    return 2.0 * (double)winograd3_tiles(B, H, dilation) * products * C * N;
}

int conv3x3_winograd3(const float *x, int B, int H, int W, int C, const float *w, const float *bias, int relu,
                      float *y, int N, int dilation, float *ws, size_t ws_floats, hipStream_t s, const float *mask)
{
    using namespace f3;
    MPSR_REQUIRE(winograd3_applies(H, W, C, dilation),
                 "conv3x3_winograd3: needs H = W = a multiple of 3 * dilation and C %% 16 == 0");
    if (ws_floats < winograd3_scratch_floats(C, N) || !ws)
        return fail(MPSR_ERR_WORKSPACE, "conv3x3_winograd3: scratch holds %zu floats, needs %zu", ws_floats,
                    winograd3_scratch_floats(C, N));
    const long long xbytes = (long long)B * H * W * C * 4;
    MPSR_REQUIRE(xbytes < 0x7ff00000LL && winograd3_scratch_floats(C, N) * 4 < 0x7ff00000ULL,
                 "conv3x3_winograd3: tensor exceeds the 2 GiB this kernel's offsets address; split the batch");
    const int th = H / (3 * dilation);
    const void *kern = th > 1 ? reinterpret_cast<const void *>(wino3h_conv_kernel) : reinterpret_cast<const void *>(wino3_conv_kernel);
    MPSR_CHECK_HIP(hipFuncSetAttribute(kern, hipFuncAttributeMaxDynamicSharedMemorySize, (int)(LDSF * sizeof(float))));
    const int form = winograd3_form(B, H, W, C, N, dilation);
    const int fform = form == 2 ? FILTER_FORM_WINO3Z : FILTER_FORM_WINO3;
    float *u = ws;
    bool ready = false;
    if (g_filter_cache_slot.w == w && g_filter_cache_slot.u && g_filter_cache_slot.floats >= winograd3_scratch_floats(C, N)) {
        u = g_filter_cache_slot.u;
        ready = g_filter_cache_slot.holds(fform);
    }
    g_filter_cache_slot = FilterCacheSlot();
    ready = ready || (g_filter_tail_done.w == w && g_filter_tail_done.u == u && g_filter_tail_done.N == N &&
                      g_filter_tail_done.C == C && g_filter_tail_done.form == (form == 2 ? 1 : 0));
    g_filter_tail_done = FilterTailJob();
    if (!ready) {
        if (form == 2) {
            if (int rc = launch_winograd3z_filter(w, N, C, u, s)) return rc;
        } else {
            const long long total = (long long)N * C;
            hipLaunchKernelGGL(wino3_filter_kernel, dim3((unsigned)((total + 255) / 256)), dim3(256), 0, s, w, N, C, u);
            MPSR_CHECK_LAUNCH("wino3_filter_kernel");
        }
    }
    if (form == 2) {
        float *part = ws;
        size_t part_floats = ws_floats;
        if (u == ws) {
            const size_t off = align_up(winograd3_scratch_floats(C, N), 64);
            part = ws + off;
            part_floats = ws_floats > off ? ws_floats - off : 0;
        }
        return launch_winograd3z(x, B, H, W, C, u, bias, relu, y, N, dilation, s, mask, part, part_floats);
    }
    if (form == 1) return launch_winograd3w(x, B, H, W, C, u, bias, relu, y, N, dilation, s, mask);
    Wino3Params p;
    p.x = x; p.u = u; p.bias = bias; p.y = y; p.mask = mask;
    p.B = B; p.H = H; p.W = W; p.C = C; p.N = N; p.dil = dilation;
    p.th = th;
    p.T = (int)winograd3_tiles(B, H, dilation);
    p.cblocks = C / KC;
    p.nblocks = ceil_div(N, NT);
    p.mblocks = ceil_div(p.T, MT);
    p.relu = relu;
    p.xbytes = (unsigned)xbytes;
    p.ubytes = (unsigned)(winograd3_scratch_floats(C, N) * 4);
    const long long blocks = 8LL * ceil_div(p.mblocks, 8) * p.nblocks;
    if (blocks > 0x7fffffffLL) return fail(MPSR_ERR_UNSUPPORTED, "conv3x3_winograd3: grid too large");
    if (th > 1) hipLaunchKernelGGL(wino3h_conv_kernel, dim3((unsigned)blocks), dim3(512), LDSF * sizeof(float), s, p);
    else hipLaunchKernelGGL(wino3_conv_kernel, dim3((unsigned)blocks), dim3(512), LDSF * sizeof(float), s, p);
    MPSR_CHECK_LAUNCH("wino3_conv_kernel");
    return MPSR_OK;
}

}

extern "C" void mpsr_debug_set_wino3_form(int form) { mpsr::g_wino3_form = form; }
```

Baseline: 19880 crops/s.

## Fuse root im2col into implicit-GEMM and add narrow-N Winograd3 variant

Adds a ROOT kind to the implicit-GEMM conv kernel that gathers 7x7 stride-2 patches straight from the 3-channel image with per-row validity bitmasks. This removes the separate im2col pass and its large column buffer from the trunk's first layer. Separately, the Winograd F(3x3) kernel gains a 32-wide N-tile variant with 256 threads and double-buffered patch loads. It is picked when the grid would otherwise have fewer workgroups than CUs, to fill the device on small problems. The fused root gather does scalar 4-byte loads with index arithmetic per element, which may be slower than the vectorized loads from a materialized cols buffer.

```diff
diff --git a/include/monopsr_hip.h b/include/monopsr_hip.h
--- a/include/monopsr_hip.h
+++ b/include/monopsr_hip.h
@@ -102,6 +102,8 @@
                                    size_t ws_floats, mpsr_stream_t stream);
 
 int mpsr_im2col_root(const float *x, int B, int H, int W, float *cols, int kpad, mpsr_stream_t stream);
+int mpsr_root_conv_fwd(const float *img, int B, int H, int W, const float *w, int kpad, const float *bias, int relu,
+                       float *y, int cout, mpsr_stream_t stream);
 
 
 int mpsr_conv2d_wgrad_f32(const float *x, const float *dy, int B, int H, int W, int C, int N, int KH, int KW,
diff --git a/monopsr_amd/_lib.py b/monopsr_amd/_lib.py
--- a/monopsr_amd/_lib.py
+++ b/monopsr_amd/_lib.py
@@ -104,6 +104,7 @@
     "mpsr_conv2d_scratch_floats": (c_sz, [c_i, c_i, c_i, c_i]),
     "mpsr_conv2d_plan": (c_i, [c_i] * 8 + [ctypes.POINTER(c_i), ctypes.POINTER(ctypes.c_double)]),
     "mpsr_im2col_root": (c_i, [c_f, c_i, c_i, c_i, c_f, c_i, c_f]),
+    "mpsr_root_conv_fwd": (c_i, [c_f, c_i, c_i, c_i, c_f, c_i, c_f, c_i, c_f, c_i, c_f]),
     "mpsr_conv2d_wgrad_f32": (c_i, [c_f, c_f, c_i, c_i, c_i, c_i, c_i, c_i, c_i, c_i, c_f, c_f, c_f]),
     "mpsr_conv2d_wgrad_scratch_floats": (c_sz, [c_i] * 8),
     "mpsr_conv2d_wgrad_ws_f32": (c_i, [c_f, c_f, c_i, c_i, c_i, c_i, c_i, c_i, c_i, c_i, c_f, c_f, c_f, c_sz, c_f]),
diff --git a/monopsr_amd/csrc/conv_mfma.hip b/monopsr_amd/csrc/conv_mfma.hip
--- a/monopsr_amd/csrc/conv_mfma.hip
+++ b/monopsr_amd/csrc/conv_mfma.hip
@@ -37,6 +37,7 @@
     float *y;
     float *ws;
     int M, H, W, C, N, KH, KW, dil, relu;
+    int IH, IW;
     int ksteps_total, ksteps_per_split, cblocks;
     int mtiles_xcd, ntiles, splits;
     FastDiv fd_ntiles, fd_mtiles;
@@ -66,15 +67,31 @@
     return (img * p.H + yy) * p.W + xx;
 }
 
-template <bool PLAIN, int AV, int BV>
+template <int KIND, int AV, int BV>
 __device__ __forceinline__ void tile_rows(const ConvParams &p, const PixelClass &pc, int r0, int n0, int lrow,
                                           unsigned col, unsigned apast, int (&ay)[AV], int (&ax)[AV],
                                           unsigned (&abase)[AV], unsigned (&bbase)[BV])
 {
 #pragma unroll
     for (int j = 0; j < AV; ++j) {
-        const int pix = decode_row<PLAIN>(p, pc, r0 + lrow + 32 * j, ay[j], ax[j]);
-        abase[j] = pix < 0 ? apast : (unsigned)pix * (unsigned)p.C * 4u + col;
+        if constexpr (KIND == 3) {
+            int oy, ox;
+            const int pix = decode_row<false>(p, pc, r0 + lrow + 32 * j, oy, ox);
+            const int img = fdiv(max(pix, 0), pc.fd_ppi);
+            const int y0 = 2 * oy - 3, x0 = 2 * ox - 3;
+            int my = 0, mx = 0;
+#pragma unroll
+            for (int t = 0; t < 7; ++t) {
+                my |= (int)((unsigned)(y0 + t) < (unsigned)p.IH) << t;
+                mx |= (int)((unsigned)(x0 + t) < (unsigned)p.IW) << t;
+            }
+            ay[j] = pix < 0 ? 0 : my;
+            ax[j] = pix < 0 ? 0 : mx;
+            abase[j] = (unsigned)(((img * p.IH + y0) * p.IW + x0) * 3) * 4u;
+        } else {
+            const int pix = decode_row<KIND == 1>(p, pc, r0 + lrow + 32 * j, ay[j], ax[j]);
+            abase[j] = pix < 0 ? apast : (unsigned)pix * (unsigned)p.C * 4u + col;
+        }
     }
     const int Ktot = p.KH * p.KW * p.C;
 #pragma unroll
@@ -301,7 +318,8 @@
 template <int BM, int BN, int WM, int WN, int MATH = MATH_FP32, int DEPTH = 1, int KIND = 0>
 __global__ __launch_bounds__(256) void conv_igemm_kernel(const ConvParams p)
 {
-    constexpr bool PLAIN = KIND == 1, CLS = KIND == 2;
+    constexpr bool PLAIN = KIND == 1, CLS = KIND == 2, ROOT = KIND == 3;
+    constexpr bool ROWS = PLAIN || ROOT;
     static_assert(WM * WN == 4, "4 waves per workgroup");
     constexpr int TM = BM / WM / 32, TN = BN / WN / 32;
     constexpr int AV = BM / 32, BV = BN / 32;
@@ -315,7 +333,7 @@
     int lm = lq - si * p.mtiles_xcd;
     const int n0 = ni * BN;
     int ci = -1;
-    if constexpr (PLAIN) {
+    if constexpr (ROWS) {
         if (xcd + 8 * lm < p.cls[0].tiles) ci = 0;
     } else {
         for (int c = 0; c < p.ncls; ++c) {
@@ -346,12 +364,12 @@
 
     int ay[AV], ax[AV];
     unsigned abase[AV], bbase[BV];
-    tile_rows<PLAIN>(p, pc, r0, n0, lrow, PLAIN || CLS ? (unsigned)lcol * 4u : 0u,
+    tile_rows<KIND>(p, pc, r0, n0, lrow, ROWS || CLS ? (unsigned)lcol * 4u : 0u,
                      PLAIN ? p.xbytes : CLS ? p.xbytes + (unsigned)(p.dil * (p.W + 1) * p.C * 4) : 0u, ay, ax, abase,
                      bbase);
 
     KCursor st;
-    if (PLAIN || ks_begin == 0) {
+    if (ROWS || ks_begin == 0) {
         st.cb = ks_begin;
         st.ky = pc.ky0;
         st.kx = pc.kx0;
@@ -370,6 +388,37 @@
 #pragma unroll
             for (int j = 0; j < AV; ++j)
                 ra[set][j] = __builtin_bit_cast(float4, __builtin_amdgcn_raw_buffer_load_b128(rxl, abase[j], soff, 0));
+#pragma unroll
+            for (int j = 0; j < BV; ++j)
+                rb[set][j] = __builtin_bit_cast(float4, __builtin_amdgcn_raw_buffer_load_b128(rwl, bbase[j], soff, 0));
+            ++st.cb;
+        } else if constexpr (ROOT) {
+            const int soff = st.cb * (BK * 4);
+            const __amdgpu_buffer_rsrc_t rxl =
+                __builtin_amdgcn_make_buffer_rsrc(const_cast<float *>(p.x), 0, live ? (int)p.xbytes : 0, 0x00020000);
+            const __amdgpu_buffer_rsrc_t rwl =
+                __builtin_amdgcn_make_buffer_rsrc(const_cast<float *>(p.w), 0, live ? (int)p.wbytes : 0, 0x00020000);
+            int sy[4], sx[4];
+            unsigned dk[4];
+#pragma unroll
+            for (int e = 0; e < 4; ++e) {
+                const unsigned k = (unsigned)(st.cb * BK + lcol + e);
+                const unsigned ky = k / 21u, r = k - 21u * ky;
+                sy[e] = k < 147u ? (int)ky : 31;
+                sx[e] = (int)(r / 3u);
+                dk[e] = (ky * (unsigned)(3 * p.IW) + r) * 4u;
+            }
+#pragma unroll
+            for (int j = 0; j < AV; ++j) {
+                float v[4];
+#pragma unroll
+                for (int e = 0; e < 4; ++e) {
+                    const bool ok = (((unsigned)ay[j] >> sy[e]) & ((unsigned)ax[j] >> sx[e]) & 1u) != 0u;
+                    v[e] = __builtin_bit_cast(
+                        float, __builtin_amdgcn_raw_buffer_load_b32(rxl, ok ? abase[j] + dk[e] : p.xbytes, 0, 0));
+                }
+                ra[set][j] = make_float4(v[0], v[1], v[2], v[3]);
+            }
 #pragma unroll
             for (int j = 0; j < BV; ++j)
                 rb[set][j] = __builtin_bit_cast(float4, __builtin_amdgcn_raw_buffer_load_b128(rwl, bbase[j], soff, 0));
@@ -450,9 +499,9 @@
     settle_acc(acc);
 
     const bool fused = p.splits == 1;
-    store_output<TM, TN, PLAIN>(p, pc, lds, r0, n0, wm, wn, wave, lane, fused,
-                                fused ? p.y : p.ws + (size_t)si * p.M * p.N,
-                                [&](int i, int j) -> f32x16 { return acc[i][j]; });
+    store_output<TM, TN, ROWS>(p, pc, lds, r0, n0, wm, wn, wave, lane, fused,
+                               fused ? p.y : p.ws + (size_t)si * p.M * p.N,
+                               [&](int i, int j) -> f32x16 { return acc[i][j]; });
 }
 
 __global__ __launch_bounds__(256) void splitk_reduce_kernel(const float *__restrict__ ws, int splits, long long MN,
@@ -528,7 +577,7 @@
 
         int ay[AV], ax[AV];
         unsigned abase[AV], bbase[BV];
-        tile_rows<false>(p, pc, r0, n0, lrow, 0u, 0u, ay, ax, abase, bbase);
+        tile_rows<0>(p, pc, r0, n0, lrow, 0u, 0u, ay, ax, abase, bbase);
         KCursor st;
         st.seek(pc, ks_begin);
         float4 ra[AV], rb[BV];
@@ -703,6 +752,12 @@
                      p.H >= 2 * p.dil && p.W >= 2 * p.dil && g_plain_override.load() != 0 &&
                      (long long)p.xbytes + (long long)p.dil * (p.W + 1) * p.C * 4 < 0x7ffffff0LL;
     {
+        if (p.IH > 0) {
+            hipLaunchKernelGGL((conv_igemm_kernel<BM, BN, WM, WN, MATH, DEPTH, 3>), dim3((unsigned)blocks), dim3(256),
+                               0, s, p);
+            MPSR_CHECK_LAUNCH("conv_igemm_kernel");
+            return MPSR_OK;
+        }
         if (plain) {
             hipLaunchKernelGGL((conv_igemm_kernel<BM, BN, WM, WN, MATH, DEPTH, 1>), dim3((unsigned)blocks), dim3(256),
                                0, s, p);
@@ -920,6 +975,10 @@
     if ((wino == 1 || wino == 2) && can2) return 1;
     return 0;
 }
+
+static int conv2d_gemm(const float *x, int B, int H, int W, int C, const float *w, const float *bias, const float *residual,
+                float *y, int N, int KH, int KW, int dilation, int relu, int split_k, float *ws, size_t ws_floats,
+                hipStream_t stream, int IH, int IW);
 
 int conv2d(const float *x, int B, int H, int W, int C, const float *w, const float *bias, const float *residual,
            float *y, int N, int KH, int KW, int dilation, int relu, int split_k, float *ws, size_t ws_floats,
@@ -957,10 +1016,19 @@
         cur_math() == MATH_FP32 && g_tile_override.load() < 0 && g_sched_override.load() < 0 &&
         fc_rows_split_applies(M64, C, N, bias, y, ws, ws_floats))
         return fc_rows_split(x, M64, C, w, bias, relu, y, N, ws, stream);
+    return conv2d_gemm(x, B, H, W, C, w, bias, residual, y, N, KH, KW, dilation, relu, split_k, ws, ws_floats, stream, 0, 0);
+}
+
+static int conv2d_gemm(const float *x, int B, int H, int W, int C, const float *w, const float *bias, const float *residual,
+                float *y, int N, int KH, int KW, int dilation, int relu, int split_k, float *ws, size_t ws_floats,
+                hipStream_t stream, int IH, int IW)
+{
+    const long long M64 = (long long)B * H * W;
     ConvParams p;
     p.x = x; p.w = w; p.bias = bias; p.residual = residual; p.y = y; p.ws = ws; p.ws_floats = ws ? ws_floats : 0;
     p.M = (int)M64; p.H = H; p.W = W; p.C = C; p.N = N; p.KH = KH; p.KW = KW; p.dil = dilation; p.relu = relu;
-    p.xbytes = (unsigned)(M64 * C * 4);
+    p.IH = IH; p.IW = IW;
+    p.xbytes = IH > 0 ? (unsigned)((long long)B * IH * IW * 3 * 4) : (unsigned)(M64 * C * 4);
     p.wbytes = (unsigned)((long long)N * KH * KW * C * 4);
     p.cblocks = ceil_div(C, BK);
     p.ksteps_total = KH * KW * p.cblocks;
@@ -979,7 +1047,7 @@
     }
     int sched = g_sched_override.load();
     if (sched < 0) sched = (split_k == 0 && ws && p.M <= 2048 && p.ksteps_total >= 128) ? 1 : 0;
-    if (sched == 1 && split_k <= 1 && ws) {
+    if (sched == 1 && split_k <= 1 && ws && IH == 0) {
         bool done = false;
         const int rc = with_tile(sel, [&](auto t) {
             using T = decltype(t);
@@ -1020,6 +1088,29 @@
     return MPSR_OK;
 }
 
+int root_conv(const float *img, int B, int H, int W, const float *w, int kpad, const float *bias, int relu, float *y,
+              int cout, float *ws, size_t ws_floats, hipStream_t stream)
+{
+    MPSR_REQUIRE(B >= 0 && H >= 7 && W >= 7 && cout > 0, "root_conv: bad shape (B=%d H=%d W=%d cout=%d)", B, H, W, cout);
+    MPSR_REQUIRE(kpad >= 147 && kpad % 32 == 0, "root_conv: kpad=%d must be a multiple of 32 and >= 147", kpad);
+    if (B == 0) return MPSR_OK;
+    MPSR_REQUIRE(img && w && y, "root_conv: null pointer");
+    MPSR_REQUIRE(((uintptr_t)img & 3) == 0 && ((uintptr_t)w & 15) == 0,
+                 "root_conv: img must be 4-byte aligned, w 16-byte aligned");
+    const int OH = (H + 6 - 7) / 2 + 1, OW = (W + 6 - 7) / 2 + 1;
+    const long long M64 = (long long)B * OH * OW;
+    MPSR_REQUIRE((long long)B * H * W * 3 * 4 < 0x7ff00000LL && (long long)cout * kpad * 4 < 0x7ff00000LL &&
+                     M64 < 0x7fffffffLL,
+                 "root_conv: tensor exceeds the 2 GiB this kernel's offsets address; split the batch");
+    return conv2d_gemm(img, B, OH, OW, kpad, w, bias, nullptr, y, cout, 1, 1, 1, relu, 0, ws, ws_floats, stream, H, W);
+}
+
+}
+
+extern "C" int mpsr_root_conv_fwd(const float *img, int B, int H, int W, const float *w, int kpad, const float *bias,
+                                  int relu, float *y, int cout, mpsr_stream_t stream)
+{
+    return mpsr::root_conv(img, B, H, W, w, kpad, bias, relu, y, cout, nullptr, 0, mpsr::as_stream(stream));
 }
 
 extern "C" void mpsr_debug_set_auto_split_target(int workgroups) { mpsr::g_auto_split_target = workgroups; }
diff --git a/monopsr_amd/csrc/internal.h b/monopsr_amd/csrc/internal.h
--- a/monopsr_amd/csrc/internal.h
+++ b/monopsr_amd/csrc/internal.h
@@ -15,6 +15,8 @@
 int conv2d(const float *x, int B, int H, int W, int C, const float *w, const float *bias, const float *residual,
            float *y, int N, int KH, int KW, int dilation, int relu, int split_k, float *ws, size_t ws_floats,
            hipStream_t stream);
+int root_conv(const float *img, int B, int H, int W, const float *w, int kpad, const float *bias, int relu, float *y,
+              int cout, float *ws, size_t ws_floats, hipStream_t stream);
 size_t conv_scratch_floats(long long M, int N);
 bool conv2d_takes_winograd4(int B, int H, int W, int C, int N, const float *ws, size_t ws_floats);
 bool conv2d_takes_winograd3(int B, int H, int W, int C, int N, int KH, int KW, int dilation, int split_k, const float *ws,
diff --git a/monopsr_amd/csrc/network.hip b/monopsr_amd/csrc/network.hip
--- a/monopsr_amd/csrc/network.hip
+++ b/monopsr_amd/csrc/network.hip
@@ -101,7 +101,7 @@
     if (B <= 0 || H <= 0 || W <= 0) return 0;
     const TrunkDims d = trunk_dims(H, W);
     const size_t Mr = (size_t)B * d.OH * d.OW, Mp = (size_t)B * d.PH * d.PW;
-    return fbytes(Mr * 160) + fbytes(Mr * 64) + fbytes(Mp * 64) + 3 * fbytes(Mp * 1024) + 2 * fbytes(Mp * 256) +
+    return fbytes(Mr * 64) + fbytes(Mp * 64) + 3 * fbytes(Mp * 1024) + 2 * fbytes(Mp * 256) +
            fbytes(mpsr::conv_scratch_floats((long long)(Mr > Mp ? Mr : Mp), 1024));
 }
 
@@ -146,7 +146,6 @@
         if (layers[i].cout > cmax) cmax = layers[i].cout;
     }
     Arena ar(workspace, workspace_bytes);
-    float *cols = ar.floats(Mr * root.cin);
     float *rootout = ar.floats(Mr * root.cout);
     float *pooled = ar.floats(Mp * root.cout);
     float *ping = ar.floats(Mp * cmax), *pong = ar.floats(Mp * cmax), *scut = ar.floats(Mp * cmax);
@@ -167,8 +166,9 @@
         }
     } tail_job_guard;
     FilterCache cache(opts);
-    if ((rc = mpsr_im2col_root(img, B, H, W, cols, root.cin, stream))) return rc;
-    if ((rc = run_layer(blob, root, cols, B, d.OH, d.OW, nullptr, rootout, 0, sk, skn, s))) return rc;
+    if ((rc = mpsr::root_conv(img, B, H, W, blob + root.w_off, root.cin, root.b_off >= 0 ? blob + root.b_off : nullptr,
+                              root.relu, rootout, root.cout, sk, skn, s)))
+        return rc;
     if ((rc = mpsr_max_pool(rootout, B, d.OH, d.OW, root.cout, 3, 2, 1, pooled, stream))) return rc;
 
     const float *cur = pooled;
diff --git a/monopsr_amd/csrc/winograd3.hip b/monopsr_amd/csrc/winograd3.hip
--- a/monopsr_amd/csrc/winograd3.hip
+++ b/monopsr_amd/csrc/winograd3.hip
@@ -10,11 +10,10 @@
 using f32x16 = __attribute__((ext_vector_type(16))) float;
 
 namespace f3 {
-constexpr int MT = 32, NT = 64, KC = 8, NP = 25;
+constexpr int MT = 32, KC = 8, NP = 25;
 constexpr int APOS = MT * KC;
 constexpr int ABUF = NP * APOS;
-constexpr int MEXF = NP * 16 * NT;
-constexpr int LDSF = MEXF > 2 * ABUF ? MEXF : 2 * ABUF;
+constexpr int ldsf(int ntw) { return NP * 16 * ntw > 2 * ABUF ? NP * 16 * ntw : 2 * ABUF; }
 constexpr unsigned OOB = 0x80000000u;
 }
 
@@ -40,14 +39,17 @@
 template <int V>
 using IC3 = std::integral_constant<int, V>;
 
-template <int NPOS, int DG, bool HALO>
+template <int NPOS, int DG, bool HALO, int NTW = 64>
 __device__ __forceinline__ void wino3_body(const Wino3Params &p, const int n0, const int t0, float *lds)
 {
     using namespace f3;
+    static_assert((NTW == 64 && DG < 2) || (NTW == 32 && DG == 2), "eight waves share the K steps, four take them all");
+    constexpr int NT = NTW;
+    constexpr int NSET = DG == 2 ? 2 : 1;
     constexpr int NU = NPOS == 7 ? 3 : 2;
     const int tid = threadIdx.x, lane = tid & 63;
     const int wave = __builtin_amdgcn_readfirstlane(tid >> 6);
-    const int pg = wave >> 1, nh = wave & 1;
+    const int pg = NTW == 64 ? wave >> 1 : wave, nh = NTW == 64 ? wave & 1 : 0;
     const int gpos = 6 * pg;
     const int nsteps = p.cblocks;
     const int d = p.dil;
@@ -70,8 +72,9 @@
 #pragma unroll
             for (int v = 0; v < 3; ++v) voffc[u][v] = (t < p.T && rowc[u] && colc[v]) ? abase : OOB;
     }
-    float pa[25];
-    auto load_patch1 = [&](int step, int L) __attribute__((always_inline)) {
+    float pa_[NSET][25];
+    auto load_patch1 = [&](int step, int L, int set) __attribute__((always_inline)) {
+        float(&pa)[25] = pa_[set];
         const bool live = step < nsteps;
         if constexpr (HALO) {
             const int s_ = L / 5, r_ = L % 5;
@@ -89,7 +92,8 @@
             pa[5 * (i + 1) + (j + 1)] = __builtin_bit_cast(float, __builtin_amdgcn_raw_buffer_load_b32(rr, abase, so, 0));
         }
     };
-    auto vertical = [&](int j) __attribute__((always_inline)) {
+    auto vertical = [&](int j, int set) __attribute__((always_inline)) {
+        float(&pa)[25] = pa_[set];
         float t0_, t1_, t2_, t3_, t4_;
         if constexpr (HALO) {
             bt5(pa[5 + j], pa[10 + j], pa[15 + j], t0_, t1_, t2_, t3_, t4_);
@@ -107,7 +111,8 @@
         pa[15 + j + 1] = t3_;
         pa[20 + j + 1] = t4_;
     };
-    auto horizontal = [&](int r) __attribute__((always_inline)) {
+    auto horizontal = [&](int r, int set) __attribute__((always_inline)) {
+        float(&pa)[25] = pa_[set];
         float t0_, t1_, t2_, t3_, t4_;
         bt5(pa[5 * r + 1], pa[5 * r + 2], pa[5 * r + 3], t0_, t1_, t2_, t3_, t4_);
         if constexpr (HALO) {
@@ -121,8 +126,8 @@
         pa[5 * r + 4] = t4_;
     };
     float *awr = lds + lt * 8 + 4 * ((ch >> 2) ^ ((lt >> 3) & 1)) + (ch & 3);
-    auto store_a = [&](int buf, int pos) __attribute__((always_inline)) {
-        awr[buf * ABUF + pos * APOS] = pa[pos];
+    auto store_a = [&](int buf, int pos, int set) __attribute__((always_inline)) {
+        awr[buf * ABUF + pos * APOS] = pa_[set][pos];
     };
 
     const unsigned bvoff = n0 + 32 * nh + (lane & 31) < p.N
@@ -176,46 +181,46 @@
                 }
         }
     };
-    auto request = [&](int step) __attribute__((always_inline)) {
-        return [&, step](int slot) __attribute__((always_inline)) {
+    auto request = [&](int step, int set = 0) __attribute__((always_inline)) {
+        return [&, step, set](int slot) __attribute__((always_inline)) {
             if constexpr (HALO) {
-                load_patch1(step, slot);
-                if (slot == 23) load_patch1(step, 24);
+                load_patch1(step, slot, set);
+                if (slot == 23) load_patch1(step, 24, set);
             } else {
-                if (slot >= 3 && slot < 12) load_patch1(step, slot - 3);
+                if (slot >= 3 && slot < 12) load_patch1(step, slot - 3, set);
             }
         };
     };
-    auto transform = [&](auto buf_c) __attribute__((always_inline)) {
-        return [&](int slot) __attribute__((always_inline)) {
+    auto transform = [&](auto buf_c, int set = 0) __attribute__((always_inline)) {
+        return [&, set](int slot) __attribute__((always_inline)) {
             constexpr int buf = decltype(buf_c)::value;
             if constexpr (HALO) {
-                if (slot < 5) vertical(slot);
-                else if (slot < 15 && ((slot - 5) & 1) == 0) horizontal((slot - 5) >> 1);
+                if (slot < 5) vertical(slot, set);
+                else if (slot < 15 && ((slot - 5) & 1) == 0) horizontal((slot - 5) >> 1, set);
                 if (slot >= 6 && slot < 16) {
                     const int r = (slot - 6) >> 1;
                     if (((slot - 6) & 1) == 0) {
-                        store_a(buf, 5 * r);
-                        store_a(buf, 5 * r + 1);
-                        store_a(buf, 5 * r + 2);
+                        store_a(buf, 5 * r, set);
+                        store_a(buf, 5 * r + 1, set);
+                        store_a(buf, 5 * r + 2, set);
                     } else {
-                        store_a(buf, 5 * r + 3);
-                        store_a(buf, 5 * r + 4);
+                        store_a(buf, 5 * r + 3, set);
+                        store_a(buf, 5 * r + 4, set);
                     }
                 }
                 return;
             }
-            if (slot < 3) vertical(slot);
-            else if (slot < 13 && ((slot - 3) & 1) == 0) horizontal((slot - 3) >> 1);
+            if (slot < 3) vertical(slot, set);
+            else if (slot < 13 && ((slot - 3) & 1) == 0) horizontal((slot - 3) >> 1, set);
             if (slot >= 4 && slot < 14) {
                 const int r = (slot - 4) >> 1;
                 if (((slot - 4) & 1) == 0) {
-                    store_a(buf, 5 * r);
-                    store_a(buf, 5 * r + 1);
-                    store_a(buf, 5 * r + 2);
+                    store_a(buf, 5 * r, set);
+                    store_a(buf, 5 * r + 1, set);
+                    store_a(buf, 5 * r + 2, set);
                 } else {
-                    store_a(buf, 5 * r + 3);
-                    store_a(buf, 5 * r + 4);
+                    store_a(buf, 5 * r + 3, set);
+                    store_a(buf, 5 * r + 4, set);
                 }
             }
         };
@@ -224,18 +229,37 @@
 #pragma unroll
     for (int j = 0; j < 3; ++j) load_b1(0, j, 0, j);
 #pragma unroll
-    for (int i = 0; i < (HALO ? 25 : 9); ++i) load_patch1(DG, i);
-    if (DG == 0) {
-#pragma unroll
-        for (int j = 0; j < (HALO ? 5 : 3); ++j) vertical(j);
-#pragma unroll
-        for (int r = 0; r < 5; ++r) horizontal(r);
-#pragma unroll
-        for (int i = 0; i < 25; ++i) store_a(0, i);
+    for (int i = 0; i < (HALO ? 25 : 9); ++i) load_patch1(DG == 2 ? 0 : DG, i, 0);
+    if (DG != 1) {
+#pragma unroll
+        for (int j = 0; j < (HALO ? 5 : 3); ++j) vertical(j, 0);
+#pragma unroll
+        for (int r = 0; r < 5; ++r) horizontal(r, 0);
+#pragma unroll
+        for (int i = 0; i < 25; ++i) store_a(0, i, 0);
+    }
+    if constexpr (DG == 2) {
+#pragma unroll
+        for (int i = 0; i < (HALO ? 25 : 9); ++i) load_patch1(1, i, NSET - 1);
     }
     __syncthreads();
 
-    if (DG == 0) {
+    if constexpr (DG == 2) {
+        for (int s = 0; s < nsteps; s += 2) {
+            {
+                auto tr = transform(IC3<1>{}, NSET - 1);
+                auto rq = request(s + 2, 0);
+                kstep(s, IC3<0>{}, [&](int slot) __attribute__((always_inline)) { tr(slot); rq(slot); });
+            }
+            __syncthreads();
+            {
+                auto tr = transform(IC3<0>{}, 0);
+                auto rq = request(s + 3, NSET - 1);
+                kstep(s + 1, IC3<1>{}, [&](int slot) __attribute__((always_inline)) { tr(slot); rq(slot); });
+            }
+            __syncthreads();
+        }
+    } else if (DG == 0) {
         for (int s = 0; s < nsteps; s += 2) {
             kstep(s, IC3<0>{}, request(s + 2));
             __syncthreads();
@@ -261,11 +285,12 @@
 
     const int lane2 = tid2 & 63;
     float *mwr = lds + gpos * (16 * NT) + (4 * (lane2 >> 5)) * NT + 32 * nh + (lane2 & 31);
-    const float *mrd = lds + (tid2 >> 5) * NT + (tid2 & 31);
+    auto ecol = [&](int h) { return (tid2 & 31) + (NTW == 64 ? 32 * h : 0); };
+    auto erow = [&](int h) { return (tid2 >> 5) + (NTW == 64 ? 0 : 8 * h); };
     float bias2[2];
 #pragma unroll
     for (int h = 0; h < 2; ++h) {
-        const int n = n0 + (tid2 & 31) + 32 * h;
+        const int n = n0 + ecol(h);
         bias2[h] = (p.bias && n < p.N) ? p.bias[n] : 0.f;
     }
 #pragma unroll
@@ -278,17 +303,23 @@
                 const int trow = (e8 & 3) + 8 * (e8 >> 2);
                 mwr[q * (16 * NT) + trow * NT] = acc[q][8 * round + e8];
             }
-        const int tt = t0 + 16 * round + (tid2 >> 5);
-        const int img = tt / tpi, rem = tt - img * tpi;
-        const int sub = rem / (th * th), tq = rem - sub * th * th;
-        const int a = sub / d + 3 * d * (tq / th), b = sub % d + 3 * d * (tq % th);
+        int tt[2], img[2], a[2], b[2];
+#pragma unroll
+        for (int h = 0; h < 2; ++h) {
+            tt[h] = t0 + 16 * round + erow(h);
+            img[h] = tt[h] / tpi;
+            const int rem = tt[h] - img[h] * tpi;
+            const int sub = rem / (th * th), tq = rem - sub * th * th;
+            a[h] = sub / d + 3 * d * (tq / th);
+            b[h] = sub % d + 3 * d * (tq % th);
+        }
         float mk[2][9];
         if (p.mask) {
 #pragma unroll
             for (int h = 0; h < 2; ++h) {
-                const int n = n0 + (tid2 & 31) + 32 * h;
-                const bool ok = tt < p.T && n < p.N;
-                const float *mo = p.mask + ((size_t)(img * p.H + a) * p.W + b) * p.N + n;
+                const int n = n0 + ecol(h);
+                const bool ok = tt[h] < p.T && n < p.N;
+                const float *mo = p.mask + ((size_t)(img[h] * p.H + a[h]) * p.W + b[h]) * p.N + n;
 #pragma unroll
                 for (int j = 0; j < 3; ++j)
 #pragma unroll
@@ -298,17 +329,18 @@
         __syncthreads();
 #pragma unroll
         for (int h = 0; h < 2; ++h) {
+            const float *mrd = lds + erow(h) * NT + ecol(h);
             float z[5][3];
 #pragma unroll
             for (int u = 0; u < 5; ++u) {
                 float m[5];
 #pragma unroll
-                for (int v = 0; v < 5; ++v) m[v] = mrd[(5 * u + v) * (16 * NT) + 32 * h];
+                for (int v = 0; v < 5; ++v) m[v] = mrd[(5 * u + v) * (16 * NT)];
                 at3(m[0], m[1], m[2], m[3], m[4], z[u][0], z[u][1], z[u][2]);
             }
-            const int n = n0 + (tid2 & 31) + 32 * h;
-            const bool ok = tt < p.T && n < p.N;
-            float *o = p.y + ((size_t)(img * p.H + a) * p.W + b) * p.N + n;
+            const int n = n0 + ecol(h);
+            const bool ok = tt[h] < p.T && n < p.N;
+            float *o = p.y + ((size_t)(img[h] * p.H + a[h]) * p.W + b[h]) * p.N + n;
 #pragma unroll
             for (int j = 0; j < 3; ++j) {
                 float yv[3];
@@ -325,32 +357,37 @@
     }
 }
 
-__global__ __launch_bounds__(512) __attribute__((amdgpu_waves_per_eu(2, 2))) void wino3_conv_kernel(const Wino3Params p)
-{
-    extern __shared__ __attribute__((aligned(16))) float lds[];
+template <int NTW, bool HALO>
+__device__ __forceinline__ void wino3_workgroup(const Wino3Params &p, float *lds)
+{
     const int xcd = blockIdx.x & 7, l_ = blockIdx.x >> 3;
     const int nb = l_ % p.nblocks;
     const int mb = (l_ / p.nblocks) * 8 + xcd;
     if (mb >= p.mblocks) return;
-    const int n0 = nb * f3::NT, t0 = mb * f3::MT;
+    const int n0 = nb * NTW, t0 = mb * f3::MT;
     const int wave = __builtin_amdgcn_readfirstlane(threadIdx.x >> 6);
-    if (wave < 4) wino3_body<6, 0, false>(p, n0, t0, lds);
-    else if (wave < 6) wino3_body<6, 1, false>(p, n0, t0, lds);
-    else wino3_body<7, 1, false>(p, n0, t0, lds);
-}
-
-__global__ __launch_bounds__(512) __attribute__((amdgpu_waves_per_eu(2, 2))) void wino3h_conv_kernel(const Wino3Params p)
+    if constexpr (NTW == 64) {
+        if (wave < 4) wino3_body<6, 0, HALO>(p, n0, t0, lds);
+        else if (wave < 6) wino3_body<6, 1, HALO>(p, n0, t0, lds);
+        else wino3_body<7, 1, HALO>(p, n0, t0, lds);
+    } else {
+        if (wave < 3) wino3_body<6, 2, HALO, 32>(p, n0, t0, lds);
+        else wino3_body<7, 2, HALO, 32>(p, n0, t0, lds);
+    }
+}
+
+template <int NTW = 64>
+__global__ __launch_bounds__(NTW * 8) __attribute__((amdgpu_waves_per_eu(NTW / 32, NTW / 32))) void wino3_conv_kernel(const Wino3Params p)
 {
     extern __shared__ __attribute__((aligned(16))) float lds[];
-    const int xcd = blockIdx.x & 7, l_ = blockIdx.x >> 3;
-    const int nb = l_ % p.nblocks;
-    const int mb = (l_ / p.nblocks) * 8 + xcd;
-    if (mb >= p.mblocks) return;
-    const int n0 = nb * f3::NT, t0 = mb * f3::MT;
-    const int wave = __builtin_amdgcn_readfirstlane(threadIdx.x >> 6);
-    if (wave < 4) wino3_body<6, 0, true>(p, n0, t0, lds);
-    else if (wave < 6) wino3_body<6, 1, true>(p, n0, t0, lds);
-    else wino3_body<7, 1, true>(p, n0, t0, lds);
+    wino3_workgroup<NTW, false>(p, lds);
+}
+
+template <int NTW = 64>
+__global__ __launch_bounds__(NTW * 8) __attribute__((amdgpu_waves_per_eu(NTW / 32, NTW / 32))) void wino3h_conv_kernel(const Wino3Params p)
+{
+    extern __shared__ __attribute__((aligned(16))) float lds[];
+    wino3_workgroup<NTW, true>(p, lds);
 }
 
 }
@@ -406,8 +443,6 @@
     MPSR_REQUIRE(xbytes < 0x7ff00000LL && winograd3_scratch_floats(C, N) * 4 < 0x7ff00000ULL,
                  "conv3x3_winograd3: tensor exceeds the 2 GiB this kernel's offsets address; split the batch");
     const int th = H / (3 * dilation);
-    const void *kern = th > 1 ? reinterpret_cast<const void *>(wino3h_conv_kernel) : reinterpret_cast<const void *>(wino3_conv_kernel);
-    MPSR_CHECK_HIP(hipFuncSetAttribute(kern, hipFuncAttributeMaxDynamicSharedMemorySize, (int)(LDSF * sizeof(float))));
     const int form = winograd3_form(B, H, W, C, N, dilation);
     const int fform = form == 2 ? FILTER_FORM_WINO3Z : FILTER_FORM_WINO3;
     float *u = ws;
@@ -446,17 +481,33 @@
     p.th = th;
     p.T = (int)winograd3_tiles(B, H, dilation);
     p.cblocks = C / KC;
-    p.nblocks = ceil_div(N, NT);
     p.mblocks = ceil_div(p.T, MT);
+    static std::atomic<int> cu_count[64];
+    int dev = 0;
+    MPSR_CHECK_HIP(hipGetDevice(&dev));
+    int cus = dev >= 0 && dev < 64 ? cu_count[dev].load() : 0;
+    if (cus == 0) {
+        MPSR_CHECK_HIP(hipDeviceGetAttribute(&cus, hipDeviceAttributeMultiprocessorCount, dev));
+        if (cus <= 0) cus = 256;
+        if (dev >= 0 && dev < 64) cu_count[dev] = cus;
+    }
+    const bool narrow = (long long)p.mblocks * ceil_div(N, 64) < cus;
+    p.nblocks = ceil_div(N, narrow ? 32 : 64);
     p.relu = relu;
     p.xbytes = (unsigned)xbytes;
     p.ubytes = (unsigned)(winograd3_scratch_floats(C, N) * 4);
     const long long blocks = 8LL * ceil_div(p.mblocks, 8) * p.nblocks;
     if (blocks > 0x7fffffffLL) return fail(MPSR_ERR_UNSUPPORTED, "conv3x3_winograd3: grid too large");
-    if (th > 1) hipLaunchKernelGGL(wino3h_conv_kernel, dim3((unsigned)blocks), dim3(512), LDSF * sizeof(float), s, p);
-    else hipLaunchKernelGGL(wino3_conv_kernel, dim3((unsigned)blocks), dim3(512), LDSF * sizeof(float), s, p);
-    MPSR_CHECK_LAUNCH("wino3_conv_kernel");
-    return MPSR_OK;
+    auto go = [&](auto kern, int ntw) -> int {
+        const size_t lds_bytes = (size_t)ldsf(ntw) * sizeof(float);
+        MPSR_CHECK_HIP(hipFuncSetAttribute(reinterpret_cast<const void *>(kern), hipFuncAttributeMaxDynamicSharedMemorySize,
+                                           (int)lds_bytes));
+        hipLaunchKernelGGL(kern, dim3((unsigned)blocks), dim3(8 * ntw), lds_bytes, s, p);
+        MPSR_CHECK_LAUNCH("wino3_conv_kernel");
+        return MPSR_OK;
+    };
+    if (th > 1) return narrow ? go(wino3h_conv_kernel<32>, 32) : go(wino3h_conv_kernel<64>, 64);
+    return narrow ? go(wino3_conv_kernel<32>, 32) : go(wino3_conv_kernel<64>, 64);
 }
 
 }
```

Result: no change. 19860 crops/s (-0.1%).
